# jhqxxx/aha

Hardware: AMD Instinct MI355X
Metric: decode tokens/s (greedy, batch 1) -- Qwen3-VL-8B, 1x1024^2 image + 512-token prompt; prefill tok/s alongside (higher is better)
Workload: dtype bf16; 1 GPU; qwen3vl8b; image=1024, kv_len_mid=2024, replicas=1, loop=device-resident greedy loop

## Files before the change

### aha_amd/_lib.py

```python
from __future__ import annotations

import ctypes as C
import os

_HERE = os.path.dirname(os.path.abspath(__file__))
LIB_PATH = os.path.join(_HERE, "csrc", "libaha_hip.so")

AHA_BF16, AHA_F16, AHA_F32, AHA_U32, AHA_U8 = 0, 1, 2, 3, 4
AHA_ARCH_QWEN3, AHA_ARCH_QWEN3VL, AHA_ARCH_QWEN3ASR = 0, 1, 2
ACT_NONE, ACT_GELU_TANH, ACT_GELU_ERF, ACT_SILU, ACT_SILU_MUL_PAIRS = 0, 1, 2, 3, 4


AHA_SAMPLE_HAS_TOP_P, AHA_SAMPLE_HAS_TOP_K = 1, 2
AHA_SAMPLE_NEED_LOGITS = 1
AHA_WQ_NONE, AHA_WQ_MXFP8_E4M3, AHA_WQ_MXFP4_E2M1 = 0, 1, 2
AHA_WQ_LM_HEAD = 1


class SamplingParams(C.Structure):
    _fields_ = [
        ("temperature", C.c_float), ("top_p", C.c_float), ("top_k", C.c_int32), ("repeat_penalty", C.c_float),
        ("repeat_last_n", C.c_int32), ("flags", C.c_uint32), ("seed", C.c_uint64),
    ]

# ... 80 lines not shown
                ("audio_samples", C.POINTER(C.c_float)), ("n_samples", C.c_int64),
                ("image_embeds", C.c_void_p), ("n_image_tokens", C.c_int64),
                ("pixel_values_video", C.c_void_p), ("n_patches_video", C.c_int64),
                ("video_grid_thw", C.POINTER(C.c_uint32)), ("n_videos", C.c_int32)]


_P = C.c_void_p
ALLREDUCE_FN = C.CFUNCTYPE(C.c_int, C.c_void_p, C.c_size_t, C.c_void_p)
REDUCE_SCATTER_FN = C.CFUNCTYPE(C.c_int, C.c_void_p, C.c_size_t, C.c_void_p)
ALL_GATHER_FN = C.CFUNCTYPE(C.c_int, C.c_void_p, C.c_size_t, C.c_void_p)

SIGNATURES = {
    "aha_hip_init": (C.c_int, [C.c_int, C.POINTER(_P)]),
    "aha_hip_shutdown": (None, [_P]),
    "aha_hip_last_error": (C.c_char_p, []),
    "aha_hip_version": (C.c_char_p, []),
    "aha_hip_get_dtype": (C.c_int, [C.c_int32, C.c_char_p, C.POINTER(C.c_int32)]),
    "aha_hip_check_dtype": (C.c_int, [C.c_int32]),
    "aha_hip_model_create": (C.c_int, [_P, C.POINTER(ModelDesc), C.POINTER(TensorView), C.c_size_t, C.POINTER(_P)]),
    "aha_hip_model_destroy": (None, [_P]),
    "aha_hip_forward_initial": (C.c_int, [_P, C.POINTER(C.c_uint32), C.c_size_t, C.c_size_t, C.POINTER(MmInput),
                                          C.POINTER(C.c_float), C.POINTER(C.c_uint32)]),
    "aha_hip_forward_step": (C.c_int, [_P, C.c_uint32, C.c_size_t, C.POINTER(C.c_float), C.POINTER(C.c_uint32)]),
    "aha_hip_clear_cache": (C.c_int, [_P]),
    "aha_hip_stop_token_ids": (C.c_int, [_P, C.POINTER(C.c_uint32), C.c_size_t]),
    "aha_hip_decode_greedy": (C.c_int, [_P, C.c_uint32, C.c_size_t, C.c_size_t, C.POINTER(C.c_uint32)]),
    "aha_hip_sample_candidates": (C.c_int, [_P, C.POINTER(C.c_uint32), C.c_size_t, C.c_float, C.c_float, C.c_int32,
                                            C.POINTER(C.c_float), C.POINTER(C.c_uint32), C.POINTER(C.c_float),
                                            C.POINTER(C.c_float)]),
    "aha_hip_last_logits": (C.c_int, [_P, C.POINTER(C.c_float)]),
    "aha_hip_rng_create": (C.c_int, [C.c_uint64, C.POINTER(_P)]),
    "aha_hip_rng_destroy": (None, [_P]),
    "aha_hip_rng_next_u32": (C.c_uint32, [_P]),
    "aha_hip_rng_weighted_index": (C.c_int, [_P, C.POINTER(C.c_float), C.c_size_t, C.POINTER(C.c_uint32)]),
    "aha_hip_debug_chacha_block": (C.c_int, [C.POINTER(C.c_uint32), C.c_int, C.POINTER(C.c_uint32)]),
    "aha_hip_img_smart_resize": (C.c_int, [C.c_uint32, C.c_uint32, C.c_uint32, C.c_uint32, C.c_uint32, C.POINTER(C.c_uint32),
                                           C.POINTER(C.c_uint32)]),
    "aha_hip_image_resize": (C.c_int, [_P, C.c_int32, C.c_int32, _P, C.c_int32, C.c_int32, _P]),
    "aha_hip_debug_resize_taps": (C.c_int, [C.c_int32, C.c_int32, C.POINTER(C.c_int32), C.POINTER(C.c_int32), C.POINTER(C.c_float),
                                            C.c_int64]),
    "aha_hip_debug_resample_taps": (C.c_int64, [C.c_int32, C.c_int32, C.POINTER(C.c_float), C.c_int64, C.POINTER(C.c_int32),
                                                C.POINTER(C.c_int32)]),
    "aha_hip_audio_resample": (C.c_int64, [_P, C.POINTER(C.c_float), C.c_int64, C.c_int32, C.c_int32, C.c_int32,
                                           C.POINTER(C.c_float), C.c_int64]),
    "aha_hip_cache_len": (C.c_size_t, [_P]),
    "aha_hip_debug_steps_executed": (C.c_int64, [_P]),
    "aha_hip_debug_graph_step": (C.c_int, [_P, C.c_int32, C.POINTER(C.c_double), C.POINTER(C.c_double)]),
    "aha_hip_kv_export": (C.c_int, [_P, _P, C.c_size_t, C.POINTER(C.c_size_t), C.POINTER(C.c_size_t), C.POINTER(C.c_int64)]),
    "aha_hip_kv_import": (C.c_int, [_P, _P, C.c_size_t, C.c_int32, C.c_int32, C.c_int32, C.c_int32, C.c_size_t, C.c_int64]),
    "aha_hip_set_profiling": (C.c_int, [_P, C.c_int]),
    "aha_hip_get_profile": (C.c_int, [_P, C.c_char_p, C.POINTER(C.c_double), C.POINTER(C.c_int64),
                                      C.POINTER(C.c_double), C.POINTER(C.c_double)]),
    "aha_hip_debug_scramble_pages": (C.c_int, [_P, C.c_int]),
    "aha_hip_debug_attn_decode_form": (C.c_int, [_P]),
    "aha_hip_debug_last_hidden": (C.c_int, [_P, C.POINTER(C.c_float), C.c_size_t]),
    "aha_hip_debug_image_embeds": (C.c_int, [_P, C.c_int, C.POINTER(C.c_float), C.c_size_t]),
    "aha_hip_rmsnorm": (C.c_int, [_P, _P, _P, C.c_int64, C.c_int32, C.c_float, _P]),
    "aha_hip_gemv": (C.c_int, [_P, _P, _P, C.c_int32, C.c_int32, _P, C.c_float, _P, _P]),
    "aha_hip_gemv_gate_up": (C.c_int, [_P, _P, _P, _P, C.c_int32, C.c_int32, _P, C.c_float, _P]),
    "aha_hip_gemm": (C.c_int, [_P, _P, _P, C.c_int32, C.c_int32, C.c_int32, C.c_int32, C.c_int32, C.c_int32, _P, _P,
                               C.c_int32, _P]),
    "aha_hip_qknorm_rope": (C.c_int, [_P, _P, _P, _P, _P, _P, _P, _P, C.c_int32, C.c_int32, C.c_int32, C.c_int32,
                                      C.c_float, C.c_float, _P]),
    "aha_hip_attn_decode": (C.c_int, [_P, _P, _P, _P, C.c_int32, C.c_int32, C.c_int32, C.c_int32, C.c_float, _P]),
    "aha_hip_attn_prefill": (C.c_int, [_P, _P, _P, _P, C.c_int32, C.c_int32, C.c_int32, C.c_int32, C.c_int32,
                                       C.c_int32, C.c_int32, C.c_float, _P]),
    "aha_hip_debug_attn_prefill_segs": (C.c_int, [_P, _P, _P, _P, C.c_int32, C.c_int32, _P, C.c_int32, C.c_int32, C.c_float, _P]),
    "aha_hip_debug_prefill_rope": (C.c_int, [_P, _P, _P, _P, _P, _P, _P, C.c_int32, C.c_int32, C.c_int32, C.c_int32, C.c_int32, C.c_float,
                                             C.c_int32, C.c_int32, C.c_int32, _P, _P, C.c_int32, _P, _P, _P]),
    "aha_hip_debug_prefill_attn_qfuse": (C.c_int, [_P, _P, _P, _P, C.c_int32, C.c_int32, C.c_int32, C.c_int32, C.c_int32, C.c_float, C.c_float,
                                                   C.c_int32, C.c_int32, C.c_int32, C.c_int32, C.c_int32, _P, C.c_int32, C.c_int32, _P, _P]),
    "aha_hip_debug_layernorm_rows": (C.c_int, [_P, _P, _P, _P, C.c_int64, C.c_int32, C.c_float, _P]),
    "aha_hip_debug_gemm_layernorm": (C.c_int, [_P, _P, _P] + [C.c_int32] * 6 + [_P, _P, C.c_int32, _P, _P, _P, C.c_float, _P]),
    "aha_hip_debug_vit_pos_embed": (C.c_int, [_P, C.c_int32, C.c_int32, C.c_int32, _P, _P, C.c_int64, C.c_int32, _P, _P, _P]),
    "aha_hip_debug_vit_rope": (C.c_int, [_P, _P, C.c_int32, C.c_int32, _P, _P, C.c_int32, C.c_int64, C.c_int32, C.c_int32, _P, _P, _P, _P, _P, _P]),
    "aha_hip_debug_scatter_rows": (C.c_int, [_P, _P, _P, C.c_int64, C.c_int64, C.c_int32, C.c_int32, _P]),
    "aha_hip_debug_audio_im2col1": (C.c_int, [_P, C.c_int64, _P, C.c_int32, C.c_int32, C.c_int32, _P, _P]),
    "aha_hip_debug_im2col_nhwc": (C.c_int, [_P, _P, C.c_int32, C.c_int32, C.c_int32, C.c_int32, _P]),
    "aha_hip_debug_audio_tokens_gather": (C.c_int, [_P, _P, C.c_int32, C.c_int32, C.c_int32, C.c_int32, _P]),
    "aha_hip_debug_sinus_pe_add": (C.c_int, [_P, C.c_int64, C.c_int32, C.c_int32, _P]),
    "aha_hip_debug_kv_pack_generic": (C.c_int, [_P, C.c_int64, C.c_int32, C.c_int32, _P, C.c_int32, C.c_int32, C.c_int32, C.c_int32, _P, _P]),
    "aha_hip_argmax": (C.c_int, [_P, C.c_int64, _P, _P]),
    "aha_hip_logmel": (C.c_int, [_P, C.c_int64, _P, _P]),
    "aha_hip_logmel_batch": (C.c_int, [_P, _P, C.c_size_t, _P, _P]),
    "aha_hip_debug_poison_lds": (C.c_int, [C.c_uint32, _P]),
    "aha_hip_debug_gemm_plan": (C.c_int, [C.c_int32, C.c_int32]),
    "aha_hip_debug_attn_variant": (C.c_int, [C.c_int32]),
    "aha_hip_debug_attn_form": (C.c_int, [C.c_int32]),
    "aha_hip_debug_gemm_grouped": (C.c_int, [_P, _P, _P] + [C.c_int32] * 10 + [_P]),
    "aha_hip_debug_streamk_plan": (C.c_int, [C.c_int32, C.c_int32, C.c_int32, C.c_int32, C.c_int32, C.c_size_t, _P, C.c_int32, _P, _P]),
    "aha_hip_set_gemm_reserved_cus": (C.c_int, [C.c_int32]),
    "aha_hip_debug_plan_gemm": (C.c_int, [C.c_int32, C.c_int32, C.c_int32, C.c_int32, C.c_int32, C.c_int32, C.c_size_t, _P]),
    "aha_hip_get_rope_index": (C.c_int, [_P, _P, C.c_size_t, _P, C.c_int32, _P, _P]),
    "aha_hip_get_rope_index_mm": (C.c_int, [_P, _P, C.c_size_t, _P, C.c_int32, _P, C.c_int32, _P, _P]),
    "aha_hip_embed": (C.c_int, [_P, _P, C.c_size_t, _P]),
    "aha_hip_embed_batch": (C.c_int, [_P, _P, _P, C.c_size_t, C.c_size_t, _P]),
    "aha_hip_generate_batch": (C.c_int, [_P, _P, _P, C.c_size_t, C.c_size_t, C.c_size_t, _P, _P, _P]),
    "aha_hip_generate_batch_sampled": (C.c_int, [_P, _P, _P, C.c_size_t, C.POINTER(SamplingParams), C.c_size_t, C.c_size_t, _P, _P, _P]),
    "aha_hip_generate_batch_mm": (C.c_int, [_P, _P, _P, C.c_size_t, _P, C.POINTER(SamplingParams), C.c_size_t, C.c_size_t, _P, _P, _P]),
    "aha_hip_generate_batch_spec": (C.c_int, [_P, _P, _P, C.c_size_t, C.c_size_t, C.c_size_t, C.POINTER(SpecConfig), _P, _P, _P, _P, _P, _P, _P,
                                              C.POINTER(SpecStats)]),
    "aha_hip_spec_propose": (C.c_int, [C.POINTER(SpecConfig), _P, C.c_size_t, C.c_size_t, _P, C.c_size_t, _P, C.POINTER(C.c_size_t)]),
    "aha_hip_engine_create": (C.c_int, [_P, C.POINTER(EngineConfig), _P]),
    "aha_hip_engine_destroy": (None, [_P]),
    "aha_hip_engine_submit": (C.c_int, [_P, _P, C.c_size_t, _P, C.POINTER(SamplingParams), C.c_size_t, C.POINTER(C.c_uint64)]),
    "aha_hip_engine_cancel": (C.c_int, [_P, C.c_uint64]),
    "aha_hip_engine_step": (C.c_int, [_P, C.POINTER(EngineEvent), C.c_size_t, C.POINTER(C.c_size_t), _P]),
    "aha_hip_engine_stats": (C.c_int, [_P, C.POINTER(EngineStats)]),
    "aha_hip_engine_debug_ctr_base": (C.c_int, [_P, C.c_uint32]),
    "aha_hip_engine_submit_spec": (C.c_int, [_P, _P, C.c_size_t, _P, C.c_size_t, C.POINTER(SpecConfig), _P, C.c_size_t, C.POINTER(C.c_uint64)]),
    "aha_hip_engine_max_events": (C.c_size_t, [_P]),
    "aha_hip_engine_spec_stats": (C.c_int, [_P, C.POINTER(SpecStats)]),
    "aha_hip_engine_request_spec": (C.c_int, [_P, C.c_uint64, C.POINTER(C.c_size_t), C.POINTER(C.c_size_t)]),
    "aha_hip_generate_batch_logprobs": (C.c_int, [_P, _P, _P, C.c_size_t, _P, C.POINTER(SamplingParams), _P, C.c_size_t, C.c_size_t, _P, _P, _P,
                                                  C.POINTER(TokenLogprobs)]),
    "aha_hip_engine_submit_logprobs": (C.c_int, [_P, _P, C.c_size_t, _P, C.POINTER(SamplingParams), C.c_size_t, C.c_int32,
                                                 C.POINTER(C.c_uint64)]),
    "aha_hip_engine_step_logprobs": (C.c_int, [_P, C.POINTER(EngineEvent), C.c_size_t, C.POINTER(C.c_size_t), _P, C.POINTER(TokenLogprobs)]),
    "aha_hip_generate_batch_adjusted": (C.c_int, [_P, _P, _P, C.c_size_t, _P, C.POINTER(SamplingParams), C.POINTER(LogitAdjust), _P, C.c_size_t,
                                                  C.c_size_t, _P, _P, _P, C.POINTER(TokenLogprobs)]),
    "aha_hip_engine_submit_adjusted": (C.c_int, [_P, _P, C.c_size_t, _P, C.POINTER(SamplingParams), C.POINTER(LogitAdjust), C.c_size_t, C.c_int32,
                                                 C.POINTER(C.c_uint64)]),
    "aha_hip_sample_rows_adjusted": (C.c_int, [_P, C.c_int64, C.c_int32, C.c_int32, _P, _P, _P, _P, _P, _P, _P, _P, _P, _P, _P, _P]),
    "aha_hip_sampler_set_adjust": (C.c_int, [_P, C.POINTER(LogitAdjust)]),
    "aha_hip_sampler_adjust_list": (C.c_int, [_P, C.c_size_t, _P, C.c_size_t, _P, _P, C.c_size_t, C.POINTER(C.c_size_t)]),
    "aha_hip_generate_batch_masked": (C.c_int, [_P, _P, _P, C.c_size_t, _P, C.POINTER(SamplingParams), C.POINTER(LogitAdjust), _P, C.c_size_t,
                                                C.c_size_t, _P, _P, _P, _P, _P, C.POINTER(TokenLogprobs)]),
    "aha_hip_engine_submit_masked": (C.c_int, [_P, _P, C.c_size_t, _P, C.POINTER(SamplingParams), C.POINTER(LogitAdjust), _P, C.c_size_t,
                                               C.c_size_t, C.c_int32, C.POINTER(C.c_uint64)]),
    "aha_hip_engine_set_mask": (C.c_int, [_P, C.c_uint64, _P, C.c_size_t]),
    "aha_hip_sample_rows_masked": (C.c_int, [_P, C.c_int64, C.c_int32, C.c_int32, _P, _P, _P, _P, _P, _P, _P, _P, _P, _P, _P, _P, _P, _P]),
    "aha_hip_sampler_set_mask": (C.c_int, [_P, _P, C.c_size_t]),
    "aha_hip_logprob_rows": (C.c_int, [_P, C.c_int64, C.c_int32, C.c_int32, _P, _P, _P, _P]),
    "aha_hip_sample_rows": (C.c_int, [_P, C.c_int64, C.c_int32, C.c_int32, _P, _P, _P, _P, _P, _P, _P, _P, _P]),
    "aha_hip_sampler_create": (C.c_int, [C.POINTER(SamplingParams), _P]),
    "aha_hip_sampler_destroy": (None, [_P]),
    "aha_hip_sampler_plan": (C.c_int, [_P, C.c_size_t, C.c_size_t, C.POINTER(C.c_int32), C.POINTER(C.c_float), C.POINTER(C.c_float),
                                       C.POINTER(C.c_size_t)]),
    "aha_hip_sampler_pick": (C.c_int, [_P, _P, _P, C.c_int32, C.c_float, C.c_float, _P, C.c_size_t, _P, C.c_size_t, C.POINTER(C.c_uint32)]),
    "aha_hip_sampler_rng_words": (C.c_uint64, [_P]),
    "aha_hip_gemv_rows": (C.c_int, [_P, _P, _P, C.c_int32, C.c_int32, C.c_int32, C.c_int32, _P, _P, _P, _P]),
    "aha_hip_quantize_mxfp8": (C.c_int, [_P, C.c_int32, C.c_int32, _P, _P, _P, _P]),
    "aha_hip_gemv_rows_mxfp8": (C.c_int, [_P, _P, _P, _P, C.c_int32, C.c_int32, C.c_int32, C.c_int32, _P, _P, _P, _P]),
    "aha_hip_quantize_mxfp4": (C.c_int, [_P, C.c_int32, C.c_int32, _P, _P, _P, _P]),
    "aha_hip_gemv_rows_mxfp4": (C.c_int, [_P, _P, _P, _P, C.c_int32, C.c_int32, C.c_int32, C.c_int32, _P, _P, _P, _P]),
    "aha_hip_model_quantize_weights": (C.c_int, [_P, C.c_int32, C.c_uint32]),
    "aha_hip_model_weight_format": (C.c_int, [_P, C.POINTER(C.c_int32), C.POINTER(C.c_uint32)]),
    "aha_hip_debug_fp8_rows": (C.c_int, [_P, C.c_int]),
    "aha_hip_debug_fp8_single": (C.c_int, [_P, C.c_int]),
    "aha_hip_debug_pk13_single": (C.c_int, [_P, C.c_int]),
    "aha_hip_pk13_status": (C.c_int, [_P, C.c_char_p, C.c_size_t]),
    "aha_hip_pack_pk13": (C.c_int, [_P, C.c_int32, C.c_int32, _P, C.POINTER(C.c_int32), C.POINTER(C.c_int64), _P]),
    "aha_hip_gemv_pk13": (C.c_int, [_P, C.c_int32, _P, _P, C.c_int32, C.c_int32, C.c_int32, _P, C.c_float, _P, _P, _P, _P]),
    "aha_hip_debug_plan_gemv_pk13": (C.c_int, [C.c_int32, C.c_int32, C.c_int32, C.c_int32, C.POINTER(C.c_int32), C.POINTER(C.c_int32),
                                              C.POINTER(C.c_int32), C.POINTER(C.c_int32), C.POINTER(C.c_int32)]),
    "aha_hip_gemv_epi": (C.c_int, [_P, _P, _P, C.c_int32, C.c_int32, C.c_int32, _P, C.c_float, _P, _P, _P, _P]),
    "aha_hip_gemv_mxfp8": (C.c_int, [_P, _P, _P, _P, C.c_int32, C.c_int32, C.c_int32, _P, C.c_float, _P, _P, _P, _P]),
    "aha_hip_debug_plan_gemv_mxfp8": (C.c_int, [C.c_int32, C.c_int32, C.c_int32, C.c_int32, C.POINTER(C.c_int32), C.POINTER(C.c_int32),
                                                C.POINTER(C.c_int32), C.POINTER(C.c_int32), C.POINTER(C.c_int32)]),
    "aha_hip_debug_fp4_single": (C.c_int, [_P, C.c_int]),
    "aha_hip_gemv_mxfp4": (C.c_int, [_P, _P, _P, _P, C.c_int32, C.c_int32, C.c_int32, _P, C.c_float, _P, _P, _P, _P]),
    "aha_hip_debug_plan_gemv_mxfp4": (C.c_int, [C.c_int32, C.c_int32, C.c_int32, C.c_int32, C.POINTER(C.c_int32), C.POINTER(C.c_int32),
                                                C.POINTER(C.c_int32), C.POINTER(C.c_int32), C.POINTER(C.c_int32)]),
    "aha_hip_debug_plan_gemv": (C.c_int, [C.c_int32, C.c_int32, C.c_int32, C.c_int32, C.POINTER(C.c_int32), C.POINTER(C.c_int32),
                                          C.POINTER(C.c_int32), C.POINTER(C.c_int32)]),
    "aha_hip_debug_gemv_partial_f32": (C.c_int, [_P, _P, _P, C.c_int32, C.c_int32, _P, C.c_float, _P]),
    "aha_hip_attn_decode_batch": (C.c_int, [_P, _P, _P, _P, _P, _P, _P, C.c_int32, C.c_int32, C.c_int32, C.c_float, C.c_float, _P, _P]),
    "aha_hip_debug_attn_decode_fused": (C.c_int, [_P, _P, _P, _P, _P, C.c_int32, C.c_int32, C.c_int32, C.c_float, C.c_float, _P, _P]),
    "aha_hip_config_parse": (C.c_int, [C.c_char_p, _P]),
    "aha_hip_config_torch_dtype": (C.c_int, [C.c_char_p, C.c_char_p, C.c_size_t]),
    "aha_hip_weights_open": (C.c_int, [C.c_char_p, _P]),
    "aha_hip_weights_count": (C.c_size_t, [_P]),
    "aha_hip_weights_get": (C.c_int, [_P, C.c_size_t, _P]),
    "aha_hip_weights_close": (None, [_P]),
    "aha_hip_model_load": (C.c_int, [_P, C.c_char_p, C.c_size_t, _P]),
    "aha_hip_set_allreduce": (C.c_int, [_P, _P, _P]),
    "aha_hip_set_seq_parallel": (C.c_int, [_P, _P, _P, _P]),
    "aha_hip_tp_unique_id": (C.c_int, [_P]),
    "aha_hip_tp_init_rccl": (C.c_int, [_P, _P]),
    "aha_hip_set_context_parallel": (C.c_int, [_P, C.c_int32, C.c_int32, _P, _P]),
    "aha_hip_cp_init_rccl": (C.c_int, [_P, _P]),
    "aha_hip_debug_cp_plan": (C.c_int, [C.c_int32, C.c_int32, C.c_int32, C.POINTER(C.c_int32)]),
    "aha_hip_debug_allreduce": (C.c_int, [_P, _P, C.c_size_t]),
    "aha_hip_vision_encode": (C.c_int, [_P, C.POINTER(MmInput), _P, C.POINTER(C.c_int64)]),
    "aha_hip_debug_audio_embeds": (C.c_int, [_P, C.POINTER(C.c_float), C.c_size_t]),
    "aha_hip_image_to_patches": (C.c_int, [_P, _P, C.c_int32, C.c_int32, C.c_int32, C.c_int32, C.POINTER(C.c_float),
                                           C.POINTER(C.c_float), _P]),
    "aha_hip_video_smart_resize": (C.c_int, [C.c_uint32] * 8 + [_P, _P]),
    "aha_hip_video_sample_frames": (C.c_int, [C.c_uint32, C.c_float, C.c_uint32, C.c_uint32, C.c_uint32, _P, _P]),
    "aha_hip_video_timestamps": (C.c_int64, [_P, C.c_size_t, C.c_float, C.c_uint32, _P, C.c_size_t]),
    "aha_hip_video_to_patches": (C.c_int, [_P, _P, C.c_int32, C.c_int32, C.c_int32, C.c_int32, C.c_int32, C.POINTER(C.c_float),
                                           C.POINTER(C.c_float), _P]),
}

TOKEN_MASK_FN = C.CFUNCTYPE(C.c_int, C.c_void_p, C.c_size_t, C.POINTER(C.c_uint32), C.c_size_t, C.POINTER(C.c_uint32), C.c_size_t)

_lib = None


class AhaHipError(RuntimeError):
    def __init__(self, code: int, msg: str):
        super().__init__(f"aha_hip error {code}: {msg}")
        self.code = code


def lib() -> C.CDLL:
    global _lib
    if _lib is None:
        if not os.path.exists(LIB_PATH):
            raise ImportError(f"{LIB_PATH} is missing: run `python -m aha_amd.build` (or __graft_entry__.build()) first; "
                              "there is no CPU fallback for the HIP path")
        try:
            import torch
        except ImportError:
            pass
        l = C.CDLL(LIB_PATH)
        for name, (res, args) in SIGNATURES.items():
            fn = getattr(l, name)
            fn.restype = res
            fn.argtypes = args
        _lib = l
    return _lib


def check(rc: int) -> int:
    if rc < 0:
        raise AhaHipError(rc, lib().aha_hip_last_error().decode(errors="replace"))
    return rc
```

### aha_amd/csrc/capi.hip

```cpp
#include <math.h>
#include <string.h>

#include <algorithm>
#include <map>
#include <memory>
#include <mutex>
#include <numeric>
#include <vector>

#include "common.h"
#include "model.h"
#include "sampler.h"
#include "audio.h"
#include "vision.h"

namespace aha {
const char* last_error_cstr();
}
using namespace aha;

#define API_GUARD_BEGIN try {
#define API_GUARD_END                                   \
  }                                                     \
  catch (const std::exception& e) {                     \
// ... 1023 lines not shown
  m->fp8_rows = on != 0;
  return AHA_OK;
}

int aha_hip_debug_fp8_single(aha_model* m, int on) {
  if (!m) {
    set_error("debug_fp8_single: null model");
    return AHA_ERR_INVALID;
  }
  if (on < 0 || on > 2) {
    set_error("debug_fp8_single: on must be 0 (bf16), 1 (by plan) or 2 (every matrix with a copy)");
    return AHA_ERR_INVALID;
  }
  m->fp8_single = on;
  return AHA_OK;
}

int aha_hip_debug_pk13_single(aha_model* m, int on) {
  if (!m) {
    set_error("debug_pk13_single: null model");
    return AHA_ERR_INVALID;
  }
  if (on < 0 || on > 2) {
    set_error("debug_pk13_single: on must be 0 (bf16), 1 (by plan) or 2 (every matrix with a copy)");
    return AHA_ERR_INVALID;
  }
  m->pk13_single = on;
  return AHA_OK;
}

int aha_hip_pk13_status(const aha_model* m, char* buf, size_t cap) {
  if (!m || (!buf && cap)) {
    set_error("pk13_status: null model or buffer");
    return AHA_ERR_INVALID;
  }
  std::string s;
  int n = 0;
  for (const Pk13Entry& e : m->pk13) {
    s += e.name + "\t" + e.status + "\n";
    n += e.slot->p != nullptr;
  }
  if (cap) {
    const size_t k = std::min(s.size(), cap - 1);
    memcpy(buf, s.data(), k);
    buf[k] = 0;
  }
  return n;
}

int aha_hip_debug_fp4_single(aha_model* m, int on) {
  if (!m) {
    set_error("debug_fp4_single: null model");
    return AHA_ERR_INVALID;
  }
  if (on < 0 || on > 2) {
    set_error("debug_fp4_single: on must be 0 (bf16), 1 (by plan) or 2 (every matrix with a copy)");
    return AHA_ERR_INVALID;
  }
  m->fp4_single = on;
  return AHA_OK;
}

static int debug_plan_gemv_mx(int mx, int32_t N, int32_t K, int32_t epi, int32_t has_norm, int32_t* R, int32_t* U, int32_t* grid, int32_t* form,
                              int32_t* by_plan) {
  if (!R || !U || !grid || N < 1 || K < 32 || K % 32 || epi < 0 || epi > 3 || (epi == 2 && N % 32)) {
    set_error(std::string("debug_plan_gemv_mxfp") + (mx == 8 ? "8" : "4") +
              ": bad argument (N >= 1, K a positive multiple of 32, epi 0..3, epi 2 needs N % 32 == 0)");
    return AHA_ERR_INVALID;
  }
  int o[5];
  (mx == 8 ? debug_plan_gemv_mxfp8 : debug_plan_gemv_mxfp4)(epi == 2 ? N / 2 : N, K, (GemvEpi)epi, has_norm != 0, o);
  *R = o[0]; *U = o[1]; *grid = o[2];
  if (form) *form = o[3] ? 1 + o[4] : 0;
  if (by_plan) *by_plan = (mx == 8 ? gemv_mxfp8_by_plan : gemv_mxfp4_by_plan)(N, K, (GemvEpi)epi) ? 1 : 0;
  return AHA_OK;
}

int aha_hip_debug_plan_gemv_mxfp8(int32_t N, int32_t K, int32_t epi, int32_t has_norm, int32_t* R, int32_t* U, int32_t* grid, int32_t* form,
                                  int32_t* by_plan) {
  return debug_plan_gemv_mx(8, N, K, epi, has_norm, R, U, grid, form, by_plan);
}

int aha_hip_debug_plan_gemv_pk13(int32_t N, int32_t K, int32_t epi, int32_t has_norm, int32_t* R, int32_t* U, int32_t* grid, int32_t* form,
                                 int32_t* by_plan) {
  if (!R || !U || !grid || epi < 0 || epi > 3 || (epi == 2 && N % 32) || !gemv_pk13_shape_ok(N, K)) {
    set_error("debug_plan_gemv_pk13: bad argument (N >= 1, K a multiple of 4096 and at most 32768, epi 0..3, epi 2 needs N % 32 == 0)");
    return AHA_ERR_INVALID;
  }
  int o[5];
  debug_plan_gemv_pk13(epi == 2 ? N / 2 : N, K, (GemvEpi)epi, has_norm != 0, o);
  *R = o[0]; *U = o[1]; *grid = o[2];
  if (form) *form = 1 + o[4];
  if (by_plan) *by_plan = gemv_pk13_by_plan(N, K, (GemvEpi)epi) ? 1 : 0;
  return AHA_OK;
}

int aha_hip_debug_plan_gemv_mxfp4(int32_t N, int32_t K, int32_t epi, int32_t has_norm, int32_t* R, int32_t* U, int32_t* grid, int32_t* form,
                                  int32_t* by_plan) {
  return debug_plan_gemv_mx(4, N, K, epi, has_norm, R, U, grid, form, by_plan);
}

int aha_hip_debug_plan_gemv(int32_t N, int32_t K, int32_t epi, int32_t has_norm, int32_t* R, int32_t* U, int32_t* grid, int32_t* form) {
  if (!R || !U || !grid || N < 1 || K < 8 || K % 8 || K > 32768 || epi < 0 || epi > 4 || (epi == 2 && N % 2)) {
    set_error("debug_plan_gemv: bad argument (N >= 1, K a positive multiple of 8 and at most 32768, epi 0..4, epi 2 needs an even N)");
    return AHA_ERR_INVALID;
  }
  int o[5];
  debug_plan_gemv(epi == 2 ? N / 2 : N, K, (GemvEpi)epi, has_norm != 0, o);
  *R = o[0]; *U = o[1]; *grid = o[2];
  if (form) *form = o[3] ? 1 + o[4] : 0;
  return AHA_OK;
}

int aha_hip_debug_gemv_partial_f32(const void* W, const void* x, float* y_f32, int32_t N, int32_t K, const void* norm_w, float eps,
                                   void* stream) {
  API_GUARD_BEGIN
  if (!W || !x || !y_f32 || N < 1 || K < 8 || K % 8 || K > 32768) {
    set_error("debug_gemv_partial_f32: bad argument (W, x, y_f32 not null, N >= 1, K a positive multiple of 8 and at most 32768)");
    return AHA_ERR_INVALID;
  }
  GemvArgs g{};
  g.W = W; g.x = x; g.y_f32 = y_f32; g.N = N; g.K = K; g.norm_w = norm_w; g.eps = eps;
  launch_gemv(g, GEMV_PARTIAL_F32, (hipStream_t)stream);
  AHA_HIP_CHECK(hipGetLastError());
  return AHA_OK;
  API_GUARD_END
}

namespace {
struct GemvPartials {
  void* p[2] = {nullptr, nullptr};
  ~GemvPartials() {
    for (void* q : p)
      if (q) hipFree(q);
  }
};
const char* gemv_epi_args_bad(const void* w, const void* x, const void* y, int N, int K, int kmul, int epi, const void* residual,
                              const float* logits, const uint32_t* argmax_out) {
  if (!w || !x) return "null matrix or x";
  if (N < 1) return "N must be at least 1";
  if (K < kmul || K % kmul) return kmul == 32 ? "K must be a positive multiple of 32 (the MX block)" : "K must be a positive multiple of 8";
  if (K > 32768) return "K must be at most 32768";
  if (epi < 0 || epi > 3) return "epi must be 0..3";
  if (epi != 3 && !y) return "null y";
  if (epi == 1 && !residual) return "epi 1 needs a residual";
  if (epi == 2 && N % 32) return "epi 2 needs N % 32 == 0";
  if (epi == 3 && (!logits || !argmax_out)) return "epi 3 needs logits and argmax_out";
  return nullptr;
}
}

static int gemv_epi_run(const void* W, int mx, const void* q, const uint32_t* scales, const void* x, void* y, int32_t N, int32_t K,
                        int32_t epi, const void* norm_w, float eps, const void* residual, float* logits, uint32_t* argmax_out, void* stream,
                        int pk13_bh = 0) {
  hipStream_t st = (hipStream_t)stream;
  GemvArgs g{};
  g.W = W; g.x = x; g.y = y; g.N = epi == 2 ? N / 2 : N; g.K = K; g.norm_w = norm_w; g.eps = eps; g.residual = epi == 1 ? residual : nullptr;
  g.y_f32 = logits;
  const GemvEpi e = epi == 0 ? GEMV_STORE : epi == 1 ? GEMV_RESIDUAL : epi == 2 ? GEMV_SILU_MUL : GEMV_LOGITS;
  GemvPartials part;
  int tiles = 0;
  if (epi == 3) {
    tiles = !q ? gemv_num_tiles(N, K) : mx == 8 ? gemv_mxfp8_num_tiles(N, K) : mx == 13 ? gemv_pk13_num_tiles(N, K) : gemv_mxfp4_num_tiles(N, K);
    AHA_HIP_CHECK(hipMalloc(&part.p[0], (size_t)tiles * 4));
    AHA_HIP_CHECK(hipMalloc(&part.p[1], (size_t)tiles * 4));
    g.blk_max = (float*)part.p[0];
    g.blk_idx = (uint32_t*)part.p[1];
  }
  if (!q) launch_gemv(g, e, st);
  else if (mx == 8) launch_gemv_mxfp8(g, q, scales, e, st);
  else if (mx == 13) launch_gemv_pk13(g, q, pk13_bh, e, st);
  else launch_gemv_mxfp4(g, q, scales, e, st);
  if (epi == 3) launch_argmax_partials(g.blk_max, g.blk_idx, tiles, argmax_out, st);
  hipError_t err = hipGetLastError();
  if (epi == 3) {
    const hipError_t e2 = hipStreamSynchronize(st);
    if (err == hipSuccess) err = e2;
  }
  AHA_HIP_CHECK(err);
  return AHA_OK;
}

int aha_hip_gemv_epi(const void* W, const void* x, void* y, int32_t N, int32_t K, int32_t epi, const void* norm_w, float eps,
                     const void* residual, float* logits, uint32_t* argmax_out, void* stream) {
  API_GUARD_BEGIN
  if (const char* bad = gemv_epi_args_bad(W, x, y, N, K, 8, epi, residual, logits, argmax_out)) {
    set_error(std::string("gemv_epi: ") + bad);
    return AHA_ERR_INVALID;
  }
  return gemv_epi_run(W, 0, nullptr, nullptr, x, y, N, K, epi, norm_w, eps, residual, logits, argmax_out, stream);
  API_GUARD_END
}

int aha_hip_gemv_mxfp8(const void* q, const uint32_t* scales, const void* x, void* y, int32_t N, int32_t K, int32_t epi, const void* norm_w,
                       float eps, const void* residual, float* logits, uint32_t* argmax_out, void* stream) {
  API_GUARD_BEGIN
  if (!scales) {
    set_error("gemv_mxfp8: null scales");
    return AHA_ERR_INVALID;
  }
  if (const char* bad = gemv_epi_args_bad(q, x, y, N, K, 32, epi, residual, logits, argmax_out)) {
    set_error(std::string("gemv_mxfp8: ") + bad);
    return AHA_ERR_INVALID;
  }
  return gemv_epi_run(nullptr, 8, q, scales, x, y, N, K, epi, norm_w, eps, residual, logits, argmax_out, stream);
  API_GUARD_END
}

int aha_hip_gemv_pk13(const void* packed, int32_t bh, const void* x, void* y, int32_t N, int32_t K, int32_t epi, const void* norm_w,
                      float eps, const void* residual, float* logits, uint32_t* argmax_out, void* stream) {
  API_GUARD_BEGIN
  if (const char* bad = gemv_epi_args_bad(packed, x, y, N, K, 8, epi, residual, logits, argmax_out)) {
    set_error(std::string("gemv_pk13: ") + bad);
    return AHA_ERR_INVALID;
  }
  if (K % 4096) {
    set_error("gemv_pk13: K must be a multiple of 4096 (the unit)");
    return AHA_ERR_INVALID;
  }
  if (bh < 0 || bh > 112) {
    set_error("gemv_pk13: bh must be 0..112");
    return AHA_ERR_INVALID;
  }
  return gemv_epi_run(nullptr, 13, packed, nullptr, x, y, N, K, epi, norm_w, eps, residual, logits, argmax_out, stream, bh);
  API_GUARD_END
}

int aha_hip_pack_pk13(const void* W, int32_t N, int32_t K, void* out, int32_t* bh_out, int64_t* bad_out, void* stream) {
  API_GUARD_BEGIN
  if (!W || !bh_out || !bad_out || N < 1 || K < 4096 || K % 4096) {
    set_error("pack_pk13: bad argument (W, bh_out, bad_out not null, N >= 1, K a positive multiple of 4096)");
    return AHA_ERR_INVALID;
  }
  hipStream_t st = (hipStream_t)stream;
  GemvPartials d;
  AHA_HIP_CHECK(hipMalloc(&d.p[0], sizeof(Pk13Stats)));
  AHA_HIP_CHECK(hipMemsetAsync(d.p[0], 0, sizeof(Pk13Stats), st));
  launch_pk13_stats(W, (int64_t)N * K, (Pk13Stats*)d.p[0], st);
  AHA_HIP_CHECK(hipGetLastError());
  Pk13Stats h{};
  AHA_HIP_CHECK(hipMemcpyAsync(&h, d.p[0], sizeof(h), hipMemcpyDeviceToHost, st));
  AHA_HIP_CHECK(hipStreamSynchronize(st));
  *bh_out = pk13_base(h.max_e2);
  *bad_out = (int64_t)h.bad;
  if (out && !h.bad) {
    launch_pk13_pack(W, N, K, *bh_out, out, st);
    AHA_HIP_CHECK(hipGetLastError());
    AHA_HIP_CHECK(hipStreamSynchronize(st));
  }
  return AHA_OK;
  API_GUARD_END
}

int aha_hip_gemv_mxfp4(const void* q, const uint32_t* scales, const void* x, void* y, int32_t N, int32_t K, int32_t epi, const void* norm_w,
                       float eps, const void* residual, float* logits, uint32_t* argmax_out, void* stream) {
  API_GUARD_BEGIN
  if (!scales) {
    set_error("gemv_mxfp4: null scales");
    return AHA_ERR_INVALID;
  }
  if (const char* bad = gemv_epi_args_bad(q, x, y, N, K, 32, epi, residual, logits, argmax_out)) {
    set_error(std::string("gemv_mxfp4: ") + bad);
    return AHA_ERR_INVALID;
  }
  return gemv_epi_run(nullptr, 4, q, scales, x, y, N, K, epi, norm_w, eps, residual, logits, argmax_out, stream);
  API_GUARD_END
}

namespace {
struct DevFree {
  void* p[2] = {nullptr, nullptr};
  ~DevFree() {
    for (void* q : p)
      if (q) hipFree(q);
  }
};
}

static int sample_rows_impl(const float* logits, int64_t ld, int32_t R, int32_t V, const int32_t* k, const float* temperature,
                            const float* repeat_penalty, const uint32_t* context, const size_t* context_offsets, const uint32_t* adj_ids,
                            const float* adj_vals, const size_t* adj_offsets, float* vals_out, uint32_t* idx_out, float* ms_out, void* stream,
                            const uint32_t* masks, const int32_t* mask_rows) {
  if (!logits || R < 1 || V < 1 || ld < V || !k || !temperature || !repeat_penalty || !context_offsets || !vals_out || !idx_out || !ms_out) {
    set_error("sample_rows: bad arguments (R >= 1, ld >= V >= 1, per-row k / temperature / repeat_penalty / context_offsets, outputs)");
    return AHA_ERR_INVALID;
  }
  for (int r = 0; r < R; ++r)
    if (!sample_shape_ok(V, k[r]) || !(repeat_penalty[r] > 0.f) || context_offsets[r + 1] < context_offsets[r] ||
        (context_offsets[r + 1] > context_offsets[r] && !context)) {
      set_error("sample_rows: row " + std::to_string(r) + " needs 1 <= k <= 64, repeat_penalty > 0 and ordered context offsets");
      return AHA_ERR_INVALID;
    }
  hipStream_t st = (hipStream_t)stream;
  std::vector<int32_t> tab((size_t)R * SAMPLE_ROW_WORDS, 0);
  std::vector<uint32_t> ctx;
  for (int r = 0; r < R; ++r) {
    int32_t* t = tab.data() + (size_t)r * SAMPLE_ROW_WORDS;
    const size_t c0 = ctx.size();
    if (repeat_penalty[r] != 1.0f) {
      for (size_t i = context_offsets[r]; i < context_offsets[r + 1]; ++i)
        if (context[i] < (uint32_t)V) ctx.push_back(context[i]);
      std::sort(ctx.begin() + c0, ctx.end());
      ctx.erase(std::unique(ctx.begin() + c0, ctx.end()), ctx.end());
    }
    const float inv_t = temperature[r] > 0.f ? (float)(1.0 / (double)temperature[r]) : 1.0f;
    t[SAMPLE_ROW_LROW] = r;
    t[SAMPLE_ROW_K] = k[r];
    memcpy(&t[SAMPLE_ROW_INVT], &inv_t, 4);
    memcpy(&t[SAMPLE_ROW_PEN], &repeat_penalty[r], 4);
    t[SAMPLE_ROW_CTX0] = (int32_t)c0;
    t[SAMPLE_ROW_NCTX] = (int32_t)(ctx.size() - c0);
    t[SAMPLE_ROW_MASK] = mask_rows && mask_rows[r] >= 0 ? mask_rows[r] : -1;
    if (t[SAMPLE_ROW_MASK] >= 0 && (!masks || (int64_t)t[SAMPLE_ROW_MASK] * ((V + 31) / 32) > (int64_t)INT32_MAX)) {
      set_error("sample_rows_masked: row " + std::to_string(r) + " names a mask but masks is null, or the mask index is out of range");
      return AHA_ERR_INVALID;
    }
  }
  std::vector<uint32_t> aid;
  std::vector<float> aval;
  for (int r = 0; adj_offsets && r < R; ++r) {
    const size_t a0 = adj_offsets[r], a1 = adj_offsets[r + 1];
    if (a1 < a0 || (a1 > a0 && (!adj_ids || !adj_vals)) || a1 - a0 > (size_t)V) {
      set_error("sample_rows_adjusted: row " + std::to_string(r) + " needs ordered adj_offsets, adj_ids / adj_vals and at most V entries");
      return AHA_ERR_INVALID;
    }
    std::vector<size_t> o(a1 - a0);
    std::iota(o.begin(), o.end(), a0);
    std::sort(o.begin(), o.end(), [&](size_t x, size_t y) { return adj_ids[x] < adj_ids[y]; });
    int32_t* t = tab.data() + (size_t)r * SAMPLE_ROW_WORDS;
    t[SAMPLE_ROW_ADJ0] = (int32_t)aid.size();
    t[SAMPLE_ROW_NADJ] = (int32_t)o.size();
    for (size_t i = 0; i < o.size(); ++i) {
      const uint32_t id = adj_ids[o[i]];
      const float a = adj_vals[o[i]];
      if (id >= (uint32_t)V || (i && id == aid.back()) || isnan(a) || a == INFINITY) {
        set_error("sample_rows_adjusted: row " + std::to_string(r) + " needs distinct ids < V and addends that are finite or -inf");
        return AHA_ERR_INVALID;
      }
      aid.push_back(id);
      aval.push_back(a);
    }
  }
  if (aid.size() > (size_t)INT32_MAX) {
    set_error("sample_rows_adjusted: too many addends");
    return AHA_ERR_INVALID;
  }
  const int nw = sample_stage1_waves(V);
  const size_t cand = (size_t)R * (nw + 16) * 64;
  DevFree adj_free;
  uint32_t* d_aid = nullptr;
  float* d_aval = nullptr;
  if (!aid.empty()) {
    AHA_HIP_CHECK(hipMalloc((void**)&d_aid, aid.size() * 4));
    adj_free.p[0] = d_aid;
    AHA_HIP_CHECK(hipMalloc((void**)&d_aval, aid.size() * 4));
    adj_free.p[1] = d_aval;
    AHA_HIP_CHECK(hipMemcpyAsync(d_aid, aid.data(), aid.size() * 4, hipMemcpyHostToDevice, st));
    AHA_HIP_CHECK(hipMemcpyAsync(d_aval, aval.data(), aid.size() * 4, hipMemcpyHostToDevice, st));
  }
  int32_t* d_tab = nullptr;
  uint32_t *d_ctx = nullptr, *d_cidx = nullptr;
  float *d_cval = nullptr, *d_part = nullptr, *d_out = nullptr;
  AHA_HIP_CHECK(hipMalloc((void**)&d_tab, tab.size() * 4));
  AHA_HIP_CHECK(hipMalloc((void**)&d_ctx, std::max<size_t>(ctx.size(), 1) * 4));
  AHA_HIP_CHECK(hipMalloc((void**)&d_cval, cand * 4));
  AHA_HIP_CHECK(hipMalloc((void**)&d_cidx, cand * 4));
  AHA_HIP_CHECK(hipMalloc((void**)&d_part, 2 * (size_t)R * nw * 4));
  AHA_HIP_CHECK(hipMalloc((void**)&d_out, (size_t)R * SAMPLE_OUT_WORDS * 4));
  AHA_HIP_CHECK(hipMemcpyAsync(d_tab, tab.data(), tab.size() * 4, hipMemcpyHostToDevice, st));
  if (!ctx.empty()) AHA_HIP_CHECK(hipMemcpyAsync(d_ctx, ctx.data(), ctx.size() * 4, hipMemcpyHostToDevice, st));
  for (int stage = 0; stage < 3; ++stage)
    launch_topk_rows(logits, ld, V, R, d_tab, d_ctx, d_cval, d_cidx, d_part, d_part + (size_t)R * nw, d_out, stage, st, d_aid, d_aval, masks);
  hipError_t err = hipGetLastError();
  if (err == hipSuccess) err = hipMemcpy2DAsync(vals_out, 64 * 4, d_out, SAMPLE_OUT_WORDS * 4, 64 * 4, R, hipMemcpyDeviceToDevice, st);
  if (err == hipSuccess) err = hipMemcpy2DAsync(ms_out, 2 * 4, d_out + 64, SAMPLE_OUT_WORDS * 4, 2 * 4, R, hipMemcpyDeviceToDevice, st);
  if (err == hipSuccess) err = hipMemcpy2DAsync(idx_out, 64 * 4, d_out + 66, SAMPLE_OUT_WORDS * 4, 64 * 4, R, hipMemcpyDeviceToDevice, st);
  hipStreamSynchronize(st);
  hipFree(d_tab);
  hipFree(d_ctx);
  hipFree(d_cval);
  hipFree(d_cidx);
  hipFree(d_part);
  hipFree(d_out);
  AHA_HIP_CHECK(err);
  return AHA_OK;
}

int aha_hip_sample_rows(const float* logits, int64_t ld, int32_t R, int32_t V, const int32_t* k, const float* temperature,
                        const float* repeat_penalty, const uint32_t* context, const size_t* context_offsets, float* vals_out,
                        uint32_t* idx_out, float* ms_out, void* stream) {
  API_GUARD_BEGIN
  return sample_rows_impl(logits, ld, R, V, k, temperature, repeat_penalty, context, context_offsets, nullptr, nullptr, nullptr, vals_out, idx_out,
                          ms_out, stream, nullptr, nullptr);
  API_GUARD_END
}

int aha_hip_sample_rows_adjusted(const float* logits, int64_t ld, int32_t R, int32_t V, const int32_t* k, const float* temperature,
                                 const float* repeat_penalty, const uint32_t* context, const size_t* context_offsets,
                                 const uint32_t* adj_ids, const float* adj_vals, const size_t* adj_offsets, float* vals_out,
                                 uint32_t* idx_out, float* ms_out, void* stream) {
  API_GUARD_BEGIN
  if (!adj_offsets) {
    set_error("sample_rows_adjusted: null adj_offsets");
// ... 868 lines not shown
```

### aha_amd/csrc/gemv_pk13_body.h

```cpp
#pragma once
#include "gemv_body.h"

namespace aha {

typedef __attribute__((ext_vector_type(2))) uint32_t pk13_u32x2_t;
typedef __attribute__((ext_vector_type(2))) uint16_t pk13_u16x2_t;

constexpr int PK13_UNIT_K = 4096;
constexpr int PK13_UNIT_BYTES = 6656;
constexpr int PK13_OFF_H = 4096, PK13_OFF_S = 6144;

__device__ __forceinline__ pk13_u32x2_t pk13_ld_nt8(const void* p) { return __builtin_nontemporal_load(reinterpret_cast<const pk13_u32x2_t*>(p)); }

struct Pk13Unit {
  u32x4_t a[4];
  u32x4_t h[2];
  pk13_u32x2_t s;
};

__device__ __forceinline__ uint32_t pk13_high4(uint32_t x, uint32_t sd, pk13_u16x2_t bh2, int g) {
  const uint32_t nz = ((x + 0x0f0f0f0fu) >> 4) & 0x01010101u;
  const pk13_u16x2_t r = __builtin_bit_cast(pk13_u16x2_t, nz) * bh2 + __builtin_bit_cast(pk13_u16x2_t, x);
  return __builtin_bit_cast(uint32_t, r) | ((sd << (7 - g)) & 0x80808080u);
}

template <int E>
__device__ __forceinline__ float pk13_f32(uint32_t hb, uint32_t lo) {
  return __uint_as_float(__builtin_amdgcn_perm(hb, lo, 0x04000c0cu + 0x01010000u * E));
}

struct GemvPk13Args {
  const void* p;
  const void* x;
  const void* norm_w;
  const void* residual;
  void* y;
  float* y_f32;
  float* blk_max;
  uint32_t* blk_idx;
  void* h_out;
  int N, K;
  int bh;
  float eps;
};

template <int R, int EPI, int PRO>
__device__ __forceinline__ void gemv_pk13_body(const GemvPk13Args& a, float* xs, const int bid, const int nblk) {
  const int tid = threadIdx.x, lane = tid & 63;
  const int wave = __builtin_amdgcn_readfirstlane(tid >> 6);
  const int K = a.K, N = a.N;
  const int nchunks = K >> 9;
  float* red = xs + (nchunks << 9);

  constexpr int ROWS_PER_TILE = GEMV_WAVES * R;
  constexpr int NW = (EPI == GEMV_SILU_MUL) ? 2 : 1;
  const int n_out = N;
  const int ntiles = (n_out + ROWS_PER_TILE - 1) / ROWS_PER_TILE;
  const int gpt = K >> 12;
  const int my_tiles = (ntiles - bid + nblk - 1) / nblk;
  const int ngroups = my_tiles * gpt;
  const uint8_t* P = (const uint8_t*)a.p;
  const size_t prow = (size_t)gpt * PK13_UNIT_BYTES;
  const pk13_u16x2_t bh2 = {(uint16_t)a.bh, (uint16_t)a.bh};

  auto issue = [&](int gi, Pk13Unit (&buf)[NW][R], bf16_t (&resv)[R]) {
    const int tile = bid + (gi / gpt) * nblk;
    const int unit = gi % gpt;
    const int row0 = tile * ROWS_PER_TILE + wave * R;
    if (EPI == GEMV_RESIDUAL) {
#pragma unroll
      for (int r = 0; r < R; ++r) resv[r] = ((const bf16_t*)a.residual)[min(row0 + r, n_out - 1)];
    }
#pragma unroll
    for (int r = 0; r < R; ++r) {
      const int row = min(row0 + r, n_out - 1);
      const size_t fr = NW == 2 ? (size_t)(row >> 4) * 32 + (row & 15) : (size_t)row;
#pragma unroll
      for (int m = 0; m < NW; ++m) {
        const uint8_t* up = P + (fr + 16 * m) * prow + (size_t)unit * PK13_UNIT_BYTES;
        Pk13Unit& b = buf[m][r];
        b.s = pk13_ld_nt8(up + PK13_OFF_S + lane * 8);
        b.h[0] = ld_nt16(up + PK13_OFF_H + lane * 16);
        b.a[0] = ld_nt16(up + lane * 16);
        b.a[1] = ld_nt16(up + 1024 + lane * 16);
        b.h[1] = ld_nt16(up + PK13_OFF_H + 1024 + lane * 16);
        b.a[2] = ld_nt16(up + 2048 + lane * 16);
        b.a[3] = ld_nt16(up + 3072 + lane * 16);
      }
    }
  };

  constexpr int XPRE = 8;
  constexpr bool SL = PRO != 0, SL_NORM = PRO == 2;
  constexpr int XSL = SL_NORM ? 4 : XPRE;
  const bool pre = SL || (nchunks << 6) <= XPRE * GEMV_THREADS;
  u32x4_t xpre[XPRE], npre[XPRE];
  Pk13Unit bufA[NW][R], bufB[NW][R];
  bf16_t resA[R], resB[R];
  if (SL) {
    const int vlast = (K >> 3) - 1;
#pragma unroll
    for (int j = 0; j < XSL; ++j) {
      const int v = min(tid + j * GEMV_THREADS, vlast);
      xpre[j] = ld16((const bf16_t*)a.x + v * 8);
      if (SL_NORM) npre[j] = ld16((const bf16_t*)a.norm_w + v * 8);
    }
    __builtin_amdgcn_sched_barrier(0);
    issue(0, bufA, resA);
    __builtin_amdgcn_sched_barrier(0);
  } else {
    if (pre) {
#pragma unroll
      for (int j = 0; j < XPRE; ++j) {
        const int v = tid + j * GEMV_THREADS;
        xpre[j] = u32x4_t{0u, 0u, 0u, 0u};
        npre[j] = u32x4_t{0u, 0u, 0u, 0u};
        if (v * 8 < K) {
          xpre[j] = ld16((const bf16_t*)a.x + v * 8);
          if (a.norm_w != nullptr) npre[j] = ld16((const bf16_t*)a.norm_w + v * 8);
        }
      }
    }
    issue(0, bufA, resA);
  }

  {
    const bf16_t* x = (const bf16_t*)a.x;
    const bf16_t* nw = (const bf16_t*)a.norm_w;
    float ss = 0.f;
    auto stage = [&](int v, u32x4_t xv) {
      float f[8];
#pragma unroll
      for (int j = 0; j < 4; ++j) { f[2 * j] = lo_bf(xv[j]); f[2 * j + 1] = hi_bf(xv[j]); }
#pragma unroll
      for (int j = 0; j < 8; ++j) ss += f[j] * f[j];
      const int base = xs_index(v * 8);
      *reinterpret_cast<float4*>(xs + base) = make_float4(f[0], f[1], f[2], f[3]);
      *reinterpret_cast<float4*>(xs + base + 256) = make_float4(f[4], f[5], f[6], f[7]);
    };
    if (pre) {
#pragma unroll
      for (int it = 0; it < (SL ? XSL : XPRE); ++it) {
        const int v = tid + it * GEMV_THREADS;
        if (v < (nchunks << 6)) stage(v, xpre[it]);
      }
    } else {
      for (int v = tid; v < (nchunks << 6); v += GEMV_THREADS) stage(v, ld16(x + v * 8));
    }
    if (SL ? SL_NORM : nw != nullptr) {
      ss = wave_sum(ss);
      if (lane == 0) red[wave] = ss;
      __syncthreads();
      const float tot = red[0] + red[1] + red[2] + red[3];
      const float rinv = 1.0f / sqrtf(tot / (float)K + a.eps);
      auto norm = [&](int v, u32x4_t wv) {
        const int base = xs_index(v * 8);
        float4 lo = *reinterpret_cast<float4*>(xs + base), hi = *reinterpret_cast<float4*>(xs + base + 256);
        lo.x = rbf(lo.x * rinv * lo_bf(wv[0])); lo.y = rbf(lo.y * rinv * hi_bf(wv[0]));
        lo.z = rbf(lo.z * rinv * lo_bf(wv[1])); lo.w = rbf(lo.w * rinv * hi_bf(wv[1]));
        hi.x = rbf(hi.x * rinv * lo_bf(wv[2])); hi.y = rbf(hi.y * rinv * hi_bf(wv[2]));
        hi.z = rbf(hi.z * rinv * lo_bf(wv[3])); hi.w = rbf(hi.w * rinv * hi_bf(wv[3]));
        *reinterpret_cast<float4*>(xs + base) = lo;
        *reinterpret_cast<float4*>(xs + base + 256) = hi;
        if (a.h_out != nullptr && bid == 0) {
          u32x4_t o;
          o[0] = pack_bf(lo.x, lo.y); o[1] = pack_bf(lo.z, lo.w); o[2] = pack_bf(hi.x, hi.y); o[3] = pack_bf(hi.z, hi.w);
          *reinterpret_cast<u32x4_t*>((bf16_t*)a.h_out + v * 8) = o;
        }
      };
      if (pre) {
#pragma unroll
        for (int it = 0; it < (SL ? XSL : XPRE); ++it) {
          const int v = tid + it * GEMV_THREADS;
          if (v < (K >> 3)) norm(v, npre[it]);
        }
      } else {
        for (int v = tid; v < (K >> 3); v += GEMV_THREADS) norm(v, ld16(nw + v * 8));
      }
    }
    __syncthreads();
  }
  __builtin_amdgcn_sched_barrier(0);

  float tile_best = -INFINITY;
  uint32_t tile_best_i = 0xffffffffu;
  float acc[NW][R];
#pragma unroll
  for (int m = 0; m < NW; ++m)
#pragma unroll
    for (int r = 0; r < R; ++r) acc[m][r] = 0.f;

  auto consume = [&](int gi, Pk13Unit (&buf)[NW][R], bf16_t (&resv)[R]) {
    const int c0 = (gi % gpt) * 8;
#pragma unroll
    for (int c = 0; c < 8; ++c) {
      const float4 xlo = *reinterpret_cast<const float4*>(xs + ((c0 + c) << 9) + (lane << 2));
      const float4 xhi = *reinterpret_cast<const float4*>(xs + ((c0 + c) << 9) + 256 + (lane << 2));
#pragma unroll
      for (int m = 0; m < NW; ++m)
#pragma unroll
        for (int r = 0; r < R; ++r) {
          const Pk13Unit& b = buf[m][r];
          const uint32_t hd = b.h[c >> 2][c & 3], sd = b.s[c >> 2];
          const uint32_t lo0 = b.a[c >> 1][(c & 1) * 2], lo1 = b.a[c >> 1][(c & 1) * 2 + 1];
          const uint32_t h0 = pk13_high4(hd & 0x0f0f0f0fu, sd, bh2, (c & 3) * 2);
          const uint32_t h1 = pk13_high4((hd >> 4) & 0x0f0f0f0fu, sd, bh2, (c & 3) * 2 + 1);
          float s = acc[m][r];
          s = fmaf(xlo.x, pk13_f32<0>(h0, lo0), s); s = fmaf(xlo.y, pk13_f32<1>(h0, lo0), s);
          s = fmaf(xlo.z, pk13_f32<2>(h0, lo0), s); s = fmaf(xlo.w, pk13_f32<3>(h0, lo0), s);
          s = fmaf(xhi.x, pk13_f32<0>(h1, lo1), s); s = fmaf(xhi.y, pk13_f32<1>(h1, lo1), s);
          s = fmaf(xhi.z, pk13_f32<2>(h1, lo1), s); s = fmaf(xhi.w, pk13_f32<3>(h1, lo1), s);
          acc[m][r] = s;
        }
    }
    if (gi % gpt != gpt - 1) return;
    const int tile = bid + (gi / gpt) * nblk;
    const int row0 = tile * ROWS_PER_TILE + wave * R;
#pragma unroll
    for (int m = 0; m < NW; ++m)
#pragma unroll
      for (int r = 0; r < R; ++r) acc[m][r] = wave_sum(acc[m][r]);
    if (lane == 0) {
#pragma unroll
      for (int r = 0; r < R; ++r) {
        const int row = row0 + r;
        if (row < n_out) {
          const float lin = rbf(acc[0][r]);
          if (EPI == GEMV_STORE) {
            ((bf16_t*)a.y)[row] = f2bf(lin);
          } else if (EPI == GEMV_RESIDUAL) {
            ((bf16_t*)a.y)[row] = f2bf(bf2f(resv[r]) + lin);
          } else if (EPI == GEMV_SILU_MUL) {
            const float g = rbf(silu_f(lin));
            const float up = rbf(acc[NW - 1][r]);
            ((bf16_t*)a.y)[row] = f2bf(g * up);
          } else {
            a.y_f32[row] = lin;
            if (lin > tile_best || (lin == tile_best && (uint32_t)row < tile_best_i)) { tile_best = lin; tile_best_i = row; }
          }
        }
      }
    }
#pragma unroll
    for (int m = 0; m < NW; ++m)
#pragma unroll
      for (int r = 0; r < R; ++r) acc[m][r] = 0.f;
  };

  int g = 0;
  for (; g + 2 < ngroups; g += 2) {
    __builtin_amdgcn_sched_barrier(0);
    issue(g + 1, bufB, resB);
    __builtin_amdgcn_sched_barrier(0);
    consume(g, bufA, resA);
    __builtin_amdgcn_sched_barrier(0);
    issue(g + 2, bufA, resA);
    __builtin_amdgcn_sched_barrier(0);
    consume(g + 1, bufB, resB);
  }
  if (g + 1 < ngroups) {
    __builtin_amdgcn_sched_barrier(0);
    issue(g + 1, bufB, resB);
    __builtin_amdgcn_sched_barrier(0);
    consume(g, bufA, resA);
    consume(g + 1, bufB, resB);
  } else if (g < ngroups) {
    consume(g, bufA, resA);
  }
  if (EPI == GEMV_LOGITS) {
    __syncthreads();
    if (lane == 0) { red[wave] = tile_best; reinterpret_cast<uint32_t*>(red)[4 + wave] = tile_best_i; }
    __syncthreads();
    if (tid == 0) {
      float bv = red[0];
      uint32_t bi = reinterpret_cast<uint32_t*>(red)[4];
      for (int w = 1; w < 4; ++w) {
        const float v = red[w];
        const uint32_t i = reinterpret_cast<uint32_t*>(red)[4 + w];
        if (v > bv || (v == bv && i < bi)) { bv = v; bi = i; }
      }
      a.blk_max[bid] = bv;
      a.blk_idx[bid] = bi;
    }
  }
}

}
```

### aha_amd/csrc/kernels.h

```cpp
#pragma once
#include <hip/hip_runtime.h>
#include <stdint.h>

#include <algorithm>
#include <utility>
#include <vector>

namespace aha {

struct KvLayer {
  const uint64_t* page_ptrs;
  uint64_t layer_off;
  int kvh, d;
};

enum GemvEpi { GEMV_STORE = 0, GEMV_RESIDUAL = 1, GEMV_SILU_MUL = 2, GEMV_LOGITS = 3, GEMV_PARTIAL_F32 = 4 };

struct GemvArgs {
  const void* W;
  const void* W2;
  const void* x;
  const void* norm_w;
  const void* residual;
  void* y;
// ... 91 lines not shown
  const float* rope;
  KvLayer kv;
  uint64_t lin_page0 = 0;
  int64_t lin_step = 0;
  int kv_start_v;
  int kv_len_v;
  float* part_o;
  float* part_ml;
  void* o;
  unsigned* head_ctr;
  unsigned ctr_target;
  unsigned long long* trace;
  int nh, kvh, nsplit;
  float eps, scale;
};
void launch_attn_decode_fused(const AttnDecodeFusedArgs& a, hipStream_t st);

struct AttnPrefillArgs {
  const void* q;
  KvLayer kv;
  void* o;
  int S, nh, kvh, d;
  int kv_offset;
  int kv_total;
  int causal;
  float scale;
  int64_t q_ld;
  int nqb;
  int S2 = 0, kv_offset2 = 0, kv_total2 = 0;
  int epi_rows = 0;
  int v_ones_row = 0;
  int rows_hint = 0;
  const void* q_norm_w = nullptr;
  const void* q_rope_tab = nullptr;
  float q_eps = 0.f;
  const int32_t* seg_tab = nullptr;
  const int32_t* seg_items = nullptr;
  int n_items = 0;
  const int32_t* seg_kv0 = nullptr;
};
inline std::vector<int32_t> seg_items_of(const std::vector<int32_t>& seg_tab, bool causal, const std::vector<int32_t>* kv0 = nullptr) {
  constexpr int QB = 64;
  std::vector<std::pair<int32_t, int32_t>> items;
  for (size_t j = 0; 3 * j < seg_tab.size(); ++j)
    for (int32_t b = 0; b * QB < seg_tab[3 * j + 1]; ++b) items.emplace_back((int32_t)j, b);
  auto cost = [&](const std::pair<int32_t, int32_t>& it) {
    const int32_t len = seg_tab[3 * (size_t)it.first + 1];
    return causal ? (kv0 ? (*kv0)[(size_t)it.first] : 0) + std::min(len, (it.second + 1) * QB) : len;
  };
  std::stable_sort(items.begin(), items.end(), [&](const auto& x, const auto& y) { return cost(x) > cost(y); });
  std::vector<int32_t> out;
  out.reserve(2 * items.size());
  for (const auto& it : items) out.push_back(it.first), out.push_back(it.second);
  return out;
}
void launch_attn_prefill(const AttnPrefillArgs& a, hipStream_t st);
bool attn_prefill_takes_qfuse(const AttnPrefillArgs& a);
int attn_prefill_form_of(const AttnPrefillArgs& a);
bool launch_attn_prefill64(const AttnPrefillArgs& a, hipStream_t st, int pipe);
void set_attn_form_override(int form);
void set_attn_variant_override(int smx);

enum GemmAct { ACT_NONE = 0, ACT_GELU_TANH = 1, ACT_GELU_ERF = 2, ACT_SILU = 3, ACT_SILU_MUL_PAIRS = 4, ACT_PARTIAL_F32 = 5 };
struct GemmArgs {
  const void* A;
  const void* W;
  void* C;
  const void* bias;
  const void* residual;
  int M, N, K;
  int64_t lda, ldw, ldc;
  int act;
  const void* norm_w = nullptr;
  void* norm_out = nullptr;
  float norm_eps = 0.f;
  const void* norm_b = nullptr;
  void* workspace = nullptr;
  size_t workspace_bytes = 0;
  void* sk_counters = nullptr;
  int tile_group = 8;
  int partial_rows = 1;
  int groups = 1, a_gstride = 0, c_gstride = 0, c_row0 = 0, m_total = 0;
};
void launch_gemm(const GemmArgs& a, hipStream_t st);
void launch_gemm_grouped(const GemmArgs& a, hipStream_t st);
void set_gemm_workspace(void* ws, size_t bytes, void* sk_counters = nullptr);
constexpr int SK_MAX_COUNTERS = 4096;
bool streamk_has_kernel(int act, bool has_bias, bool has_res, bool n192);
double streamk_estimate(const GemmArgs& a, int tile_n, int* n_chunks, int* n_split);
bool launch_gemm_streamk(const GemmArgs& a, int tile_n, hipStream_t st);
void set_streamk_forced_cut(int code);
int gemm_streamk_workers();
int gemm_streamk_cus();
int get_gemm_reserved_cus();
void set_gemm_reserved_cus(int n);
bool acquire_gemm_cu_reservation(int cus);
void release_gemm_cu_reservation();
int debug_streamk_plan(int M, int N, int K, int tile_n, int workers, int group, size_t ws_bytes, int* out, int cap, int* off_out, int* info);
void debug_plan_gemm(int M, int N, int K, int act, bool has_bias, bool has_res, size_t ws_bytes, int* out, bool has_norm = false);
void set_gemm_plan_override(int tile, int splitk);
void get_gemm_workspace(void** ws, size_t* bytes, void** sk_counters);
struct GemmWorkspaceScope {
  GemmWorkspaceScope(void* ws, size_t bytes, void* sk_counters = nullptr) {
    get_gemm_workspace(&prev_ws, &prev_bytes, &prev_ctrs);
    set_gemm_workspace(ws, bytes, sk_counters);
  }
  ~GemmWorkspaceScope() { set_gemm_workspace(prev_ws, prev_bytes, prev_ctrs); }
  GemmWorkspaceScope(const GemmWorkspaceScope&) = delete;
  GemmWorkspaceScope& operator=(const GemmWorkspaceScope&) = delete;
  void* prev_ws = nullptr;
  size_t prev_bytes = 0;
  void* prev_ctrs = nullptr;
};
void launch_residual_add_f32(void* x, const float* sum, int64_t n, hipStream_t st);
void launch_poison_lds(uint32_t seed, hipStream_t st);
void launch_residual_add_f32_cols(void* x, int64_t ldx, const float* sum, int64_t lds, int64_t rows, int cols, hipStream_t st);
void launch_row_to_f32(const void* x_bf16_or_null, float* out, int n, hipStream_t st);
void launch_f32_to_row(const float* x, void* out_bf16, int n, hipStream_t st);

struct GemvRowsArgs {
  const void* W;
  const void* x;
  const void* residual;
  void* y;
  float* y_f32;
  float* blk_max;
  uint32_t* blk_idx;
  float* ws;
  int R, N, K;
  int64_t ldx, ldy, ldf;
  int64_t ldws = 0;
};
void launch_gemv_rows(const GemvRowsArgs& a, GemvEpi epi, hipStream_t st);
void launch_gemv_rows_merge(const GemvRowsArgs& a, GemvEpi epi, int nks, hipStream_t st);
struct WQuant {
  void* q = nullptr;
  uint32_t* scales = nullptr;
};
size_t mxfp8_scale_words(int N, int K);
void launch_gemv_rows_mxfp8(const GemvRowsArgs& a, const void* q, const uint32_t* scales, GemvEpi epi, hipStream_t st);
void launch_mxfp8_quantize(const void* w, int N, int K, void* q_out, uint32_t* scales_out, void* w_roundtrip_out, hipStream_t st);
void launch_mxfp8_check(const void* w, int64_t n_elems, int* flag, hipStream_t st);
void launch_gemv_mxfp8(const GemvArgs& g, const void* q, const uint32_t* scales, GemvEpi epi, hipStream_t st);
int gemv_mxfp8_num_tiles(int N, int K);
bool gemv_mxfp8_by_plan(int N, int K, GemvEpi epi);
void debug_plan_gemv_mxfp8(int N, int K, GemvEpi epi, bool has_norm, int* out5);
void launch_gemv_rows_mxfp4(const GemvRowsArgs& a, const void* q, const uint32_t* scales, GemvEpi epi, hipStream_t st);
void launch_mxfp4_quantize(const void* w, int N, int K, void* q_out, uint32_t* scales_out, void* w_roundtrip_out, hipStream_t st);
void launch_mxfp4_check(const void* w, int64_t n_elems, int* flag, hipStream_t st);
void launch_gemv_mxfp4(const GemvArgs& g, const void* q, const uint32_t* scales, GemvEpi epi, hipStream_t st);
int gemv_mxfp4_num_tiles(int N, int K);
bool gemv_mxfp4_by_plan(int N, int K, GemvEpi epi);
void debug_plan_gemv_mxfp4(int N, int K, GemvEpi epi, bool has_norm, int* out5);
struct Pk13Stats {
  int max_e2;
  int pad;
  unsigned long long bad;
};
__host__ __device__ inline int pk13_base(int max_e2) { return max_e2 > 15 ? max_e2 - 15 : 0; }
size_t pk13_bytes(int N, int K);
void launch_pk13_stats(const void* w, int64_t n_elems, Pk13Stats* stats, hipStream_t st);
void launch_pk13_pack(const void* w, int N, int K, int bh, void* out, hipStream_t st);
bool gemv_pk13_shape_ok(int N, int K);
void launch_gemv_pk13(const GemvArgs& g, const void* packed, int bh, GemvEpi epi, hipStream_t st);
int gemv_pk13_num_tiles(int N, int K);
bool gemv_pk13_by_plan(int N, int K, GemvEpi epi);
void debug_plan_gemv_pk13(int N, int K, GemvEpi epi, bool has_norm, int* out5);
void gemv_rows_plan(int N, int K, int* chunks_per_wave, int* k_splits);
int gemv_rows_num_tiles(int N);
size_t gemv_rows_ws_floats(int R, int N, int K);
void launch_argmax_rows(const float* blk_max, const uint32_t* blk_idx, int ntiles, int rows, uint32_t* out, hipStream_t st);

constexpr int GEN_ROW_WORDS = 8;
constexpr int GEN_ROW_PAGE0 = 0;
constexpr int GEN_ROW_KVLEN = 1;
constexpr int GEN_ROW_NSPLIT = 2;
constexpr int GEN_ROW_CTR = 3;
constexpr int GEN_ROW_POS = 4;
constexpr int GEN_ROW_SRC = 5;
constexpr int GEN_ROW_CTRROW = 6;
constexpr int GEN_ROW_TOK = 7;
void launch_gen_embed(const void* table, const uint32_t* tok_in, const int32_t* row_tab, int rows, void* x, int H, const float* inv_freq,
                      const int32_t* axis_map, float* rope, hipStream_t st);

struct AttnDecodeBatchArgs {
  const void* qkv;
  const void* q_norm_w;
  const void* k_norm_w;
  const float* rope;
  const uint64_t* page_ptrs;
  uint64_t layer_off;
  const int32_t* row_tab;
  float* part_o;
  float* part_ml;
  void* o;
  unsigned* head_ctr;
  int ctr_step;
  int nh, kvh, max_nsplit;
  float eps, scale;
};
void launch_attn_decode_batch(const AttnDecodeBatchArgs& a, int rows, int max_nsplit_rows, hipStream_t st, bool append = true);
void launch_kv_append_rows(const AttnDecodeBatchArgs& a, int rows, hipStream_t st);
constexpr int SPEC_MAX_DRAFT = 15;
constexpr int SPEC_SEQ_WORDS = 2, SPEC_SEQ_ROW0 = 0, SPEC_SEQ_NDRAFT = 1;
constexpr int SPEC_OUT_WORDS = 2 + SPEC_MAX_DRAFT + 1, SPEC_OUT_COUNT = 0, SPEC_OUT_LAST_ROW = 1, SPEC_OUT_TOKENS = 2;
void launch_spec_accept_rows(const uint32_t* argmax, const int32_t* row_tab, const int32_t* seq_tab, int n_seqs, uint32_t* out, hipStream_t st);
constexpr int ENG_SEQ_WORDS = 3, ENG_SEQ_ROW = 0, ENG_SEQ_DRAFT0 = 1, ENG_SEQ_NDRAFT = 2;
void launch_spec_accept_split(const uint32_t* argmax, const int32_t* row_tab, const int32_t* seq_tab, int n_seqs, uint32_t* out, hipStream_t st);
int attn_decode_nsplit(int kv_len_after, int g, int max_nsplit);

struct StepState;
constexpr size_t DECODE_SYNC_BYTES = 32768;
constexpr int DECODE_HEAD_CTR_WORD = 6144;

}

namespace aha {
constexpr int VIT_DQK = 96;
constexpr int VIT_DV = 80;
void launch_layernorm_rows(const void* x, const void* w, const void* b, void* y, int64_t rows, int dim, float eps,
                           hipStream_t st);
void launch_pos_embed_add(void* x, const void* table, const int32_t* idx, const float* wt, int64_t N, int D,
                          hipStream_t st);
struct VitRopeArgs {
  const void* qkv;
  const int32_t* rowcol;
  const float* inv_freq;
  const int32_t* page_of;
  const int32_t* slot_of;
  void* q_out;
  KvLayer kv;
  int N, nh, hd;
  const float* cs_tab = nullptr;
  const int32_t* page_first = nullptr;
  const int32_t* page_cnt = nullptr;
  int n_pages = 0;
};
void launch_vit_rope_pack(const VitRopeArgs& a, hipStream_t st);
void launch_vit_rope_table(const int32_t* rowcol, const float* inv_freq, int N, int hd, float* tab, hipStream_t st);
void launch_scatter_rows(void* dst, const void* src, const int32_t* rows, int64_t n, int D, int add, hipStream_t st);
int img_smart_resize(uint32_t h, uint32_t w, uint32_t factor, uint32_t min_pixels, uint32_t max_pixels, uint32_t* h_out, uint32_t* w_out);
int video_smart_resize(uint32_t num_frames, uint32_t h, uint32_t w, uint32_t temporal_factor, uint32_t factor, uint32_t min_pixels,
                       uint32_t max_pixels, uint32_t video_ratio, uint32_t* h_out, uint32_t* w_out);
int video_sample_frames(uint32_t total_frames, float rate, uint32_t fps, uint32_t min_frames, uint32_t max_frames, uint32_t* nframes,
                        uint32_t* interval);
int64_t video_timestamps(const uint32_t* frame_indices, size_t n, float fps, uint32_t t_merge, float* out, size_t cap);
int image_resize(const uint8_t* src, int H, int W, uint8_t* dst, int new_h, int new_w, hipStream_t st);
int debug_resize_taps(int n_in, int n_out, int32_t* left, int32_t* count, float* weights, int64_t weights_cap);
void launch_video_to_patches(const uint8_t* frames, void* out, int T, int H, int W, int patch, int merge, const float* mean,
                             const float* stdv, hipStream_t st);
void launch_image_to_patches(const uint8_t* img, void* out, int H, int W, int patch, int merge, const float* mean,
                             const float* stdv, hipStream_t st);
}

namespace aha {
constexpr int LOGMEL_CLIP_WORDS = 5;
void launch_logmel(const float* x, const int64_t* d_clips, int n_clips, int64_t n_groups, int64_t ld, const float* window, const float* twid,
                   const float* melfb, float* out, float* frame_max, hipStream_t st);
void launch_audio_im2col1(const float* feat, const int32_t* d_chunks, void* out, int64_t ld, int C, int Hin, int Win, hipStream_t st);
void launch_im2col_nhwc(const void* in, void* out, int B, int Hin, int Win, int Cin, hipStream_t st);
void launch_audio_tokens_gather(const void* in, void* out, int B, int Fq, int T, int Cc, hipStream_t st);
void launch_sinus_pe_add(void* x, int64_t rows, int d, int T, hipStream_t st);
void launch_kv_pack_generic(const void* src, int64_t ld, int k_off, int v_off, KvLayer kv, int N, int nh, int hd, hipStream_t st,
                            const int32_t* slot_of = nullptr);
}
```

### aha_amd/csrc/kernels_gemv_pk13.hip

```cpp
#include <algorithm>

#include "gemv_pk13_body.h"
#include "kernels.h"

namespace aha {

namespace {

struct GemvPk13TailArgs {
  float* y_f32;
  float* blk_max;
  uint32_t* blk_idx;
  void* h_out;
  float eps;
  int nblk;
};

template <int R, int EPI, int PRO>
__global__ __launch_bounds__(GEMV_THREADS) void gemv_kernel_pk13(const void* p, const void* x, const void* norm_w, void* y, const void* residual,
                                                                 int N, int K, int bh, GemvPk13TailArgs t) {
  extern __shared__ __attribute__((aligned(16))) float xs[];
  GemvPk13Args a;
  a.p = p; a.x = x; a.norm_w = norm_w; a.residual = residual; a.y = y;
  a.y_f32 = t.y_f32; a.blk_max = t.blk_max; a.blk_idx = t.blk_idx; a.h_out = t.h_out; a.N = N; a.K = K; a.bh = bh; a.eps = t.eps;
  gemv_pk13_body<R, EPI, PRO>(a, xs, (int)blockIdx.x, t.nblk);
}

struct GemvPk13Plan { int R, grid; };

GemvPk13Plan plan_gemv_pk13(int N, GemvEpi epi) {
  const int R = epi == GEMV_LOGITS ? 2 : 1;
  const int gmax = 768;
  const int ntiles = (N + 4 * R - 1) / (4 * R);
  int grid = std::min(ntiles, gmax);
  if (ntiles > gmax) {
    for (int g = gmax; g >= gmax / 2; g -= 8)
      if (ntiles % g == 0) {
        grid = g;
        break;
      }
  }
  return {R, std::max(grid, 1)};
}

int pro_of(int K, bool has_norm) { return K <= (has_norm ? 4 : 8) * 8 * GEMV_THREADS ? (has_norm ? 2 : 1) : 0; }

template <int R, int EPI>
void launch_pk13_epi(const GemvPk13Args& a, const GemvPk13Plan& p, hipStream_t st) {
  const size_t lds = (size_t)a.K * 4 + 64;
  dim3 grid(p.grid), block(GEMV_THREADS);
  const GemvPk13TailArgs t{a.y_f32, a.blk_max, a.blk_idx, a.h_out, a.eps, p.grid};
  const int pro = pro_of(a.K, a.norm_w != nullptr);
#define GV_(PP) hipLaunchKernelGGL((gemv_kernel_pk13<R, EPI, PP>), grid, block, lds, st, a.p, a.x, a.norm_w, a.y, a.residual, a.N, a.K, a.bh, t)
  if (pro == 2) GV_(2); else if (pro == 1) GV_(1); else GV_(0);
#undef GV_
}

__device__ __forceinline__ int pk13_e2(uint32_t bits16) { return (bits16 >> 8) & 0x7f; }

__global__ __launch_bounds__(256) void pk13_max_kernel(const u32x4_t* w, int64_t nvec, Pk13Stats* out) {
  int mx = 0;
  unsigned long long bad = 0;
  for (int64_t i = (int64_t)blockIdx.x * 256 + threadIdx.x; i < nvec; i += (int64_t)gridDim.x * 256) {
    const u32x4_t v = ld_nt16(w + i);
#pragma unroll
    for (int j = 0; j < 8; ++j) {
      const uint32_t b = (v[j >> 1] >> ((j & 1) * 16)) & 0xffffu;
      if ((b & 0x7f80u) == 0x7f80u) ++bad;
      else mx = max(mx, pk13_e2(b));
    }
  }
  for (int o = 32; o > 0; o >>= 1) {
    mx = max(mx, __shfl_xor(mx, o));
    bad += __shfl_xor(bad, o);
  }
  if ((threadIdx.x & 63) == 0) {
    atomicMax(&out->max_e2, mx);
    if (bad) atomicAdd(&out->bad, bad);
  }
}

__global__ __launch_bounds__(256) void pk13_window_kernel(const u32x4_t* w, int64_t nvec, Pk13Stats* out) {
  const int bh = pk13_base(out->max_e2);
  unsigned long long bad = 0;
  for (int64_t i = (int64_t)blockIdx.x * 256 + threadIdx.x; i < nvec; i += (int64_t)gridDim.x * 256) {
    const u32x4_t v = ld_nt16(w + i);
#pragma unroll
    for (int j = 0; j < 8; ++j) {
      const uint32_t b = (v[j >> 1] >> ((j & 1) * 16)) & 0xffffu;
      const int e2 = pk13_e2(b);
      if ((b & 0x7f80u) != 0x7f80u && e2 != 0 && e2 <= bh) ++bad;
    }
  }
  for (int o = 32; o > 0; o >>= 1) bad += __shfl_xor(bad, o);
  if ((threadIdx.x & 63) == 0 && bad) atomicAdd(&out->bad, bad);
}

__global__ __launch_bounds__(256) void pk13_pack_kernel(const bf16_t* w, int64_t nunits, int bh, uint8_t* out) {
  const int lane = threadIdx.x & 63;
  const int64_t unit = (int64_t)blockIdx.x * 4 + (threadIdx.x >> 6);
  if (unit >= nunits) return;
  const bf16_t* src = w + unit * PK13_UNIT_K + lane * 8;
  uint8_t* dst = out + unit * PK13_UNIT_BYTES;
  u32x4_t a[4], h[2];
  uint32_t s[2] = {0u, 0u};
#pragma unroll
  for (int c = 0; c < 8; ++c) {
    const u32x4_t v = ld16(src + c * 512);
    uint32_t lo[2] = {0u, 0u}, hd = 0u;
#pragma unroll
    for (int e = 0; e < 8; ++e) {
      const uint32_t b = (v[e >> 1] >> ((e & 1) * 16)) & 0xffffu;
      const int e2 = pk13_e2(b);
      const uint32_t code = e2 == 0 ? 0u : (uint32_t)(e2 - bh) & 15u;
      lo[e >> 2] |= (b & 0xffu) << (8 * (e & 3));
      hd |= code << (8 * (e & 3) + 4 * (e >> 2));
      s[c >> 2] |= (b >> 15) << ((c & 3) * 2 + (e >> 2) + 8 * (e & 3));
    }
    a[c >> 1][(c & 1) * 2] = lo[0];
    a[c >> 1][(c & 1) * 2 + 1] = lo[1];
    h[c >> 2][c & 3] = hd;
  }
#pragma unroll
  for (int p = 0; p < 4; ++p) *reinterpret_cast<u32x4_t*>(dst + p * 1024 + lane * 16) = a[p];
#pragma unroll
  for (int q = 0; q < 2; ++q) *reinterpret_cast<u32x4_t*>(dst + PK13_OFF_H + q * 1024 + lane * 16) = h[q];
  *reinterpret_cast<pk13_u32x2_t*>(dst + PK13_OFF_S + lane * 8) = pk13_u32x2_t{s[0], s[1]};
}

}

size_t pk13_bytes(int N, int K) { return (size_t)N * (K / PK13_UNIT_K) * PK13_UNIT_BYTES; }

void launch_pk13_stats(const void* w, int64_t n_elems, Pk13Stats* stats, hipStream_t st) {
  const int64_t nvec = n_elems / 8;
  const int grid = (int)std::min<int64_t>((nvec + 255) / 256, 4096);
  hipLaunchKernelGGL(pk13_max_kernel, dim3(grid), dim3(256), 0, st, (const u32x4_t*)w, nvec, stats);
  hipLaunchKernelGGL(pk13_window_kernel, dim3(grid), dim3(256), 0, st, (const u32x4_t*)w, nvec, stats);
}

void launch_pk13_pack(const void* w, int N, int K, int bh, void* out, hipStream_t st) {
  const int64_t nunits = (int64_t)N * (K / PK13_UNIT_K);
  hipLaunchKernelGGL(pk13_pack_kernel, dim3((unsigned)((nunits + 3) / 4)), dim3(256), 0, st, (const bf16_t*)w, nunits, bh, (uint8_t*)out);
}

bool gemv_pk13_shape_ok(int N, int K) { return N >= 1 && K >= PK13_UNIT_K && K % PK13_UNIT_K == 0 && K <= 32768; }

bool gemv_pk13_by_plan(int N, int K, GemvEpi epi) {
  (void)epi;
  return gemv_pk13_shape_ok(N, K) && (int64_t)N * K >= ((int64_t)1 << 25);
}

int gemv_pk13_num_tiles(int N, int K) { (void)K; return plan_gemv_pk13(N, GEMV_LOGITS).grid; }

void debug_plan_gemv_pk13(int N, int K, GemvEpi epi, bool has_norm, int* out5) {
  const GemvPk13Plan p = plan_gemv_pk13(N, epi);
  out5[0] = p.R; out5[1] = 8; out5[2] = p.grid; out5[3] = 1; out5[4] = pro_of(K, has_norm);
}

void launch_gemv_pk13(const GemvArgs& g, const void* packed, int bh, GemvEpi epi, hipStream_t st) {
  if (!gemv_pk13_shape_ok(g.N, g.K)) abort();
  GemvPk13Args a{};
  a.p = packed; a.x = g.x; a.norm_w = g.norm_w; a.residual = g.residual; a.y = g.y; a.y_f32 = g.y_f32;
  a.blk_max = g.blk_max; a.blk_idx = g.blk_idx; a.h_out = g.h_out; a.N = g.N; a.K = g.K; a.bh = bh; a.eps = g.eps;
  const GemvPk13Plan p = plan_gemv_pk13(g.N, epi);
  switch (epi) {
    case GEMV_STORE: launch_pk13_epi<1, GEMV_STORE>(a, p, st); break;
    case GEMV_RESIDUAL: launch_pk13_epi<1, GEMV_RESIDUAL>(a, p, st); break;
    case GEMV_SILU_MUL: launch_pk13_epi<1, GEMV_SILU_MUL>(a, p, st); break;
    case GEMV_LOGITS: launch_pk13_epi<2, GEMV_LOGITS>(a, p, st); break;
    default: abort();
  }
}

}
```

### aha_amd/csrc/model.h

```cpp
#pragma once
#include <hip/hip_runtime.h>

#include <map>
#include <string>
#include <vector>

#include "../../include/aha_hip.h"
#include "kernels.h"

struct aha_ctx {
  int device = 0;
  hipStream_t stream = nullptr;
};

namespace aha {

void set_error(const std::string& msg);
#define AHA_HIP_CHECK(expr)                                                                          \
  do {                                                                                               \
    hipError_t _e = (expr);                                                                          \
    if (_e != hipSuccess) {                                                                          \
      ::aha::set_error(std::string(#expr) + " failed: " + hipGetErrorString(_e));                    \
      return AHA_ERR_HIP;                                                                            \
    }                                                                                                \
  } while (0)

struct Pk13Copy {
  void* p = nullptr;
  int bh = 0;
};
struct Pk13Entry { std::string name; Pk13Copy* slot; std::string status; };

struct LayerWeights {
  void* wqkv = nullptr;
  void* wo = nullptr;
  void* wgu = nullptr;
  void* wdown = nullptr;
  void* in_norm = nullptr;
  void* post_norm = nullptr;
  void* q_norm = nullptr;
  void* k_norm = nullptr;
  WQuant q_wqkv, q_wo, q_wgu, q_wdown;
  Pk13Copy p_wqkv, p_wo, p_wgu, p_wdown;
};

constexpr uint32_t RING_CAP = 256;

struct StepState {
  uint32_t token;
  int32_t pos[3];
  int32_t kv_start;
  int32_t kv_len;
  uint32_t next_token;
  int32_t step;
};

struct ProfRec { int cls; hipEvent_t e0, e1; double bytes, flops; };

struct VisionModel;
struct AudioModel;

}

struct aha_weights {
  struct Mapping { void* base; size_t len; };
  std::vector<Mapping> maps;
  std::vector<std::string> names;
  std::vector<aha_tensor_view> views;
  ~aha_weights();
};

struct aha_model {
  aha_ctx* ctx = nullptr;
  aha_model_desc desc{};
  hipStream_t stream = nullptr;
  void* embed = nullptr;
  void* lm_head = nullptr;
  void* final_norm = nullptr;
  std::vector<aha::LayerWeights> layers;
  std::vector<void*> owned;
  int32_t wq_format = 0;
  uint32_t wq_flags = 0;
  aha::WQuant q_lm_head;
  bool fp8_rows = true;
  int fp8_single = 1;
  aha::Pk13Copy p_lm_head;
  std::vector<aha::Pk13Entry> pk13;
  int pk13_single = 1;
  int fp4_single = 1;
  float* d_inv_freq = nullptr;
  int32_t* d_axis_map = nullptr;
  float* d_rope = nullptr;
  float attn_scale = 0.f;
  std::vector<void*> slabs;
  std::vector<uint64_t> h_page_ptrs;
  uint64_t* d_page_ptrs = nullptr;
  size_t page_table_cap = 0;
  size_t pages_per_slab = 0;
  uint64_t page_bytes = 0;
  uint64_t layer_stride = 0;
  size_t n_pages = 0;
  size_t lin_pages = 0;
  uint64_t lin_p0 = 0;
  int64_t lin_step = 0;
  int last_attn_form = -1;
  size_t cache_len = 0;
  bool scramble_pages = false;
  std::vector<uint64_t> free_pages;
  aha::StepState* d_state = nullptr;
  aha::StepState* h_state = nullptr;
  uint32_t* d_token_log = nullptr;
  size_t token_log_cap = 0;
  uint32_t* h_ring = nullptr;
  uint32_t* h_ring_dev = nullptr;
  uint32_t* h_done = nullptr;
  uint32_t* h_done_dev = nullptr;
  int64_t steps_executed = 0;
  bool rope_delta_valid = false;
  int64_t rope_delta = 0;
  void *d_x = nullptr, *d_qkv = nullptr, *d_q = nullptr, *d_attn = nullptr, *d_act = nullptr, *d_hlast = nullptr;
  float* d_logits = nullptr;
  float* d_blk_max = nullptr;
  uint32_t* d_blk_idx = nullptr;
  float* d_part_o = nullptr;
  float* d_part_ml = nullptr;
  int max_nsplit = 64;
  int tp_rank = 0, tp_size = 1;
  aha_allreduce_fn allreduce_cb = nullptr;
  void* allreduce_user = nullptr;
  aha_reduce_scatter_fn reduce_scatter_cb = nullptr;
  aha_all_gather_fn all_gather_cb = nullptr;
  void* sp_user = nullptr;
  void* rccl_comm = nullptr;
  void* rccl_comm_side = nullptr;
  hipStream_t comm_stream = nullptr;
  bool reserved_cus_set = false;
  hipEvent_t ev_gemm[8] = {};
  hipEvent_t ev_ag[8] = {};
  hipEvent_t ev_comm = nullptr;
  int async_rc = 0;
  int lm_rows = 0, lm_row0 = 0;
  float* d_partial = nullptr;
  float* p_partial = nullptr;
  int cp_rank = 0, cp_size = 1;
  int comm_rank = 0;
  aha_all_gather_fn cp_all_gather_cb = nullptr;
  void* cp_user = nullptr;
  void* p_cp_stage = nullptr;
  std::vector<int32_t> cp_row_map;
  size_t cp_stage_bytes = 0;
  void* p_hstage = nullptr;
  unsigned head_ctr_base = 0;
  unsigned* d_bar = nullptr;
  unsigned long long* d_gemv_trace = nullptr;
  unsigned long long* d_attn_trace = nullptr;
  bool decode_fused = true;
  float* h_logits = nullptr;
  bool have_logits = false;
  bool logits_assembled = false;
  float* d_samp_work = nullptr;
  float* d_samp_f = nullptr;
  unsigned* d_samp_u = nullptr;
  uint32_t* d_samp_ctx = nullptr;
  uint32_t* h_samp = nullptr;
  size_t samp_ctx_cap = 0;
  size_t pf_cap = 0;
  uint32_t* p_ids = nullptr;
  int32_t* p_pos = nullptr;
  void *p_x = nullptr, *p_h = nullptr, *p_qkv = nullptr, *p_q = nullptr, *p_attn = nullptr, *p_act = nullptr;
  void* p_rope = nullptr;
  void* p_gemm_ws = nullptr;
  size_t gemm_ws_bytes = 0;
  void* d_sk_ctrs = nullptr;
  std::vector<void*> pf_owned;
  int32_t* p_pass_tab = nullptr;
  size_t p_pass_tab_cap = 0;
  int32_t* h_pass_stage = nullptr;
  size_t h_pass_stage_cap = 0;
  float* p_pool = nullptr;
  size_t p_pool_cap = 0;
  aha_engine* engine = nullptr;
  aha::VisionModel* vision = nullptr;
// ... 103 lines not shown
```

### aha_amd/csrc/model.hip

```cpp
#include "model.h"
#include "mxfp8.h"

#include <math.h>
#include <stdlib.h>
#include <string.h>

#include <algorithm>
#include <chrono>
#include <deque>

#include "common.h"
#include "audio.h"
#include "sampler.h"
#include "vision.h"

namespace aha {

static thread_local std::string g_last_error;
void set_error(const std::string& msg) { g_last_error = msg; }
const char* last_error_cstr() { return g_last_error.c_str(); }

ProfScope::ProfScope(aha_model* m_, const char* cls, double bytes, double flops) : m(m_) {
  if (!m->profiling) return;
  auto it = m->prof_cls.find(cls);
// ... 372 lines not shown
    set_error("kv_import: the destination model is tensor-parallel (tp_size " + std::to_string(m->tp_size) + "); import into an un-sharded model");
    return AHA_ERR_UNSUPPORTED;
  }
  if (!in_dev || n_heads <= 0 || src_head0 < 0 || dst_head0 < 0 || src_head0 + n_heads > src_heads || dst_head0 + n_heads > c.num_key_value_heads) {
    set_error("kv_import: head ranges out of bounds (buffer holds " + std::to_string(src_heads) + " heads, the model " +
              std::to_string(c.num_key_value_heads) + ")");
    return AHA_ERR_INVALID;
  }
  if (n_tokens == 0) return AHA_OK;
  const size_t pages = (n_tokens + KV_PAGE_TOKENS - 1) / KV_PAGE_TOKENS;
  const size_t need_bytes = (size_t)c.num_hidden_layers * pages * (size_t)src_heads * 2 * KV_BLOCK_BYTES;
  if (in_bytes < need_bytes) {
    set_error("kv_import: the buffer holds " + std::to_string(in_bytes) + " bytes, " + std::to_string(need_bytes) + " are needed for " +
              std::to_string(n_tokens) + " tokens of " + std::to_string(src_heads) + " heads");
    return AHA_ERR_INVALID;
  }
  AHA_HIP_CHECK(hipSetDevice(m->ctx->device));
  int rc = model_ensure_pages(m, n_tokens);
  if (rc) return rc;
  hipLaunchKernelGGL(kv_pack_kernel, dim3((unsigned)pages, (unsigned)c.num_hidden_layers, (unsigned)n_heads * 2), dim3(256), 0, m->stream,
                     m->d_page_ptrs, m->layer_stride, c.num_key_value_heads, (char*)in_dev, src_heads, src_head0, dst_head0, (int)pages, 1);
  AHA_HIP_CHECK(hipGetLastError());
  AHA_HIP_CHECK(hipStreamSynchronize(m->stream));
  m->cache_len = n_tokens;
  m->rope_delta = rope_delta;
  m->rope_delta_valid = true;
  m->have_logits = false;
  m->logits_assembled = false;
  return AHA_OK;
}

static int assemble_logits(aha_model* m);

int model_sample_candidates(aha_model* m, const uint32_t* ctx, size_t n_ctx, float repeat_penalty, float temperature, int k,
                            float* vals_out, uint32_t* idx_out, float* max_out, float* sumexp_out) {
  const int V = m->desc.vocab_size;
  if (!m->have_logits) {
    set_error("sample_candidates: no forward call has produced logits yet");
    return AHA_ERR_STATE;
  }
  if (!sample_shape_ok(V, k)) {
    set_error("sample_candidates: k must be in [1, 64] (and vocab * k within the stage-2 capacity)");
    return AHA_ERR_UNSUPPORTED;
  }
  if (!(repeat_penalty > 0.f) || (n_ctx && !ctx) || !vals_out || !idx_out) {
    set_error("sample_candidates: bad argument");
    return AHA_ERR_INVALID;
  }
  const int nw = sample_stage1_waves(V);
  constexpr size_t OUT_WORDS = 64 + 2 + 64;
  if (!m->d_samp_f) {
    const size_t nc = ((size_t)nw + 16) * 64;
    const size_t nf = nc + 2 * (size_t)nw + OUT_WORDS, nu = nc;
    void *pw = nullptr, *pf = nullptr, *pu = nullptr;
    if (int rc = dev_alloc(m, (size_t)V * 4, &pw, false)) return rc;
    if (int rc = dev_alloc(m, nf * 4, &pf, false)) return rc;
    if (int rc = dev_alloc(m, nu * 4, &pu, false)) return rc;
    m->d_samp_work = (float*)pw;
    m->d_samp_f = (float*)pf;
    m->d_samp_u = (unsigned*)pu;
  }
  if (!m->h_samp || n_ctx > m->samp_ctx_cap) {
    const size_t cap = std::max<size_t>(1024, n_ctx * 2);
    void* pd = nullptr;
    if (int rc = dev_alloc(m, cap * 4, &pd, false)) return rc;
    uint32_t* ph = nullptr;
    AHA_HIP_CHECK(hipHostMalloc((void**)&ph, (cap + OUT_WORDS) * 4));
    if (m->h_samp) hipHostFree(m->h_samp);
    m->h_samp = ph;
    m->d_samp_ctx = (uint32_t*)pd;
    m->samp_ctx_cap = cap;
  }
  if (int rc = assemble_logits(m)) return rc;
  const float* src = m->d_logits;
  if (repeat_penalty != 1.0f && n_ctx > 0) {
    memcpy(m->h_samp, ctx, n_ctx * 4);
    AHA_HIP_CHECK(hipMemcpyAsync(m->d_samp_ctx, m->h_samp, n_ctx * 4, hipMemcpyHostToDevice, m->stream));
    AHA_HIP_CHECK(hipMemcpyAsync(m->d_samp_work, m->d_logits, (size_t)V * 4, hipMemcpyDeviceToDevice, m->stream));
    launch_repeat_penalty(m->d_logits, m->d_samp_work, m->d_samp_ctx, (int)n_ctx, repeat_penalty, V, m->stream);
    src = m->d_samp_work;
  }
  const float inv_temp = temperature > 0.f ? (float)(1.0 / (double)temperature) : 1.0f;
  float* cand_val = m->d_samp_f;
  float* part_m = cand_val + ((size_t)nw + 16) * 64;
  float* part_s = part_m + nw;
  float* out_val = part_s + nw;
  float* out_ms = out_val + 64;
  unsigned* out_idx = reinterpret_cast<unsigned*>(out_ms + 2);
  unsigned* cand_idx = m->d_samp_u;
  launch_topk_candidates(src, V, k, inv_temp, cand_val, cand_idx, part_m, part_s, out_val, out_idx, out_ms, m->stream);
  AHA_HIP_CHECK(hipGetLastError());
  uint32_t* h_out = m->h_samp + m->samp_ctx_cap;
  AHA_HIP_CHECK(hipMemcpyAsync(h_out, out_val, OUT_WORDS * 4, hipMemcpyDeviceToHost, m->stream));
  AHA_HIP_CHECK(hipStreamSynchronize(m->stream));
  memcpy(vals_out, h_out, (size_t)k * 4);
  memcpy(idx_out, h_out + 66, (size_t)k * 4);
  if (max_out) memcpy(max_out, h_out + 64, 4);
  if (sumexp_out) memcpy(sumexp_out, h_out + 65, 4);
  return AHA_OK;
}

int model_last_logits(aha_model* m, float* logits_out) {
  if (!m->have_logits) {
    set_error("last_logits: no forward call has produced logits yet");
    return AHA_ERR_STATE;
  }
  if (int rc = assemble_logits(m)) return rc;
  AHA_HIP_CHECK(hipMemcpyAsync(m->h_logits, m->d_logits, (size_t)m->desc.vocab_size * 4, hipMemcpyDeviceToHost, m->stream));
  AHA_HIP_CHECK(hipStreamSynchronize(m->stream));
  memcpy(logits_out, m->h_logits, (size_t)m->desc.vocab_size * 4);
  return AHA_OK;
}

int model_clear_cache(aha_model* m) {
  for (size_t i = m->n_pages; i > 0; --i) m->free_pages.push_back(m->h_page_ptrs[i - 1]);
  m->n_pages = 0;
  m->lin_pages = 0;
  m->cache_len = 0;
  m->rope_delta = 0;
  m->rope_delta_valid = false;
  return AHA_OK;
}

static void model_free_packed(aha_model* m, const char* why) {
  for (Pk13Entry& e : m->pk13) {
    if (e.slot->p) {
      hipFree(e.slot->p);
      e.status = why;
    }
    *e.slot = Pk13Copy{};
  }
}

static int model_pack_weights(aha_model* m) {
  const aha_model_desc& c = m->desc;
  struct Mat { const void* w; int N, K; };
  std::vector<Mat> mats;
  const int H = c.hidden_size, I = c.intermediate_size, nq = c.num_attention_heads * c.head_dim, nkv = c.num_key_value_heads * c.head_dim;
  for (int li = 0; li < c.num_hidden_layers; ++li) {
    LayerWeights& L = m->layers[li];
    const std::string p = "layers." + std::to_string(li) + ".";
    m->pk13.push_back({p + "self_attn.q_proj/k_proj/v_proj.weight", &L.p_wqkv, ""});
    mats.push_back({L.wqkv, nq + 2 * nkv, H});
    m->pk13.push_back({p + "self_attn.o_proj.weight", &L.p_wo, ""});
    mats.push_back({L.wo, H, nq});
    m->pk13.push_back({p + "mlp.gate_proj/up_proj.weight", &L.p_wgu, ""});
    mats.push_back({L.wgu, 2 * I, H});
    m->pk13.push_back({p + "mlp.down_proj.weight", &L.p_wdown, ""});
    mats.push_back({L.wdown, H, I});
  }
  m->pk13.push_back({c.tie_word_embeddings ? "embed_tokens.weight (tied lm_head)" : "lm_head.weight", &m->p_lm_head, ""});
  mats.push_back({m->lm_head, m->lm_rows, H});
  auto all = [&](const char* why) {
    for (Pk13Entry& e : m->pk13)
      if (e.status.empty()) e.status = why;
    return AHA_OK;
  };
  const char* env = getenv("AHA_WPACK");
  if (env && atoi(env) == 0) return all("off (AHA_WPACK=0)");
  if (m->tp_size > 1 || m->cp_size > 1) return all("sharded model");
  std::vector<size_t> cand;
  for (size_t i = 0; i < mats.size(); ++i) {
    if (!gemv_pk13_shape_ok(mats[i].N, mats[i].K)) m->pk13[i].status = "K is not a multiple of 4096 (or above 32768)";
    else if ((int64_t)mats[i].N * mats[i].K < ((int64_t)1 << 24)) m->pk13[i].status = "fewer than 2^24 elements";
    else cand.push_back(i);
  }
  if (cand.empty()) return AHA_OK;
  hipStream_t st = m->stream;
  std::vector<Pk13Stats> h(cand.size());
  {
    Pk13Stats* d = nullptr;
    if (hipMalloc((void**)&d, cand.size() * sizeof(Pk13Stats)) != hipSuccess) {
      (void)hipGetLastError();
      return all("not enough device memory");
    }
    hipError_t e = hipMemsetAsync(d, 0, cand.size() * sizeof(Pk13Stats), st);
    for (size_t k = 0; k < cand.size() && e == hipSuccess; ++k) launch_pk13_stats(mats[cand[k]].w, (int64_t)mats[cand[k]].N * mats[cand[k]].K, d + k, st);
    if (e == hipSuccess) e = hipGetLastError();
    if (e == hipSuccess) e = hipMemcpyAsync(h.data(), d, cand.size() * sizeof(Pk13Stats), hipMemcpyDeviceToHost, st);
    if (e == hipSuccess) e = hipStreamSynchronize(st);
    hipFree(d);
    AHA_HIP_CHECK(e);
  }
  std::vector<size_t> take;
  size_t bytes = 0;
  for (size_t k = 0; k < cand.size(); ++k) {
    if (h[k].bad) {
      m->pk13[cand[k]].status = std::to_string(h[k].bad) + " weights outside the window (Inf, NaN, or more than 30 binades below the matrix maximum)";
      continue;
    }
    m->pk13[cand[k]].slot->bh = pk13_base(h[k].max_e2);
    take.push_back(cand[k]);
    bytes += pk13_bytes(mats[cand[k]].N, mats[cand[k]].K);
  }
  size_t free_b = 0, total_b = 0;
  if (hipMemGetInfo(&free_b, &total_b) != hipSuccess) {
    (void)hipGetLastError();
    free_b = 0;
  }
  if (take.empty()) return AHA_OK;
  if ((double)free_b < 1.1 * (double)bytes) return all("not enough device memory");
  for (size_t i : take) {
    if (hipMalloc(&m->pk13[i].slot->p, pk13_bytes(mats[i].N, mats[i].K)) != hipSuccess) {
      (void)hipGetLastError();
      m->pk13[i].slot->p = nullptr;
      model_free_packed(m, "not enough device memory");
      return all("not enough device memory");
    }
    launch_pk13_pack(mats[i].w, mats[i].N, mats[i].K, m->pk13[i].slot->bh, m->pk13[i].slot->p, st);
    m->pk13[i].status = "packed";
  }
  hipError_t e = hipGetLastError();
  if (e == hipSuccess) e = hipStreamSynchronize(st);
  AHA_HIP_CHECK(e);
  return AHA_OK;
}

int model_quantize_weights(aha_model* m, int32_t format, uint32_t flags) {
  const aha_model_desc& c = m->desc;
  if (format != AHA_WQ_MXFP8_E4M3 && format != AHA_WQ_MXFP4_E2M1) {
    set_error("quantize_weights: unknown format " + std::to_string(format) + " (AHA_WQ_MXFP8_E4M3 = 1, AHA_WQ_MXFP4_E2M1 = 2)");
    return AHA_ERR_INVALID;
  }
  if (flags & ~(uint32_t)AHA_WQ_LM_HEAD) {
    set_error("quantize_weights: unknown flag bits " + std::to_string(flags & ~(uint32_t)AHA_WQ_LM_HEAD) + " (AHA_WQ_LM_HEAD = 1)");
    return AHA_ERR_INVALID;
  }
  if (m->engine) {
    set_error("quantize_weights: the model has an engine (aha_hip_engine_destroy first)");
    return AHA_ERR_STATE;
  }
  if (m->wq_format != AHA_WQ_NONE) {
    if (m->wq_format == format && m->wq_flags == flags) return AHA_OK;
    set_error("quantize_weights: the model is already quantised with format " + std::to_string(m->wq_format) + ", flags " +
              std::to_string(m->wq_flags));
    return AHA_ERR_STATE;
  }
  if (m->cache_len != 0) {
    set_error("quantize_weights: the cache holds " + std::to_string(m->cache_len) + " tokens (aha_hip_clear_cache first)");
    return AHA_ERR_STATE;
  }
  if (m->tp_size > 1 || m->cp_size > 1) {
    set_error("quantize_weights: tensor- and context-parallel models are not supported");
    return AHA_ERR_UNSUPPORTED;
  }
  if ((c.arch != AHA_ARCH_QWEN3 && c.arch != AHA_ARCH_QWEN3VL && c.arch != AHA_ARCH_QWEN3ASR) || c.head_dim != 128) {
    set_error("quantize_weights: Qwen3, Qwen3-VL and Qwen3-ASR with head_dim 128 only (the models of generate_batch)");
    return AHA_ERR_UNSUPPORTED;
  }
  struct Mat { std::string name; void* w; int N, K; WQuant* slot; };
  std::vector<Mat> mats;
  const int H = c.hidden_size, I = c.intermediate_size, nq = c.num_attention_heads * 128, nkv = c.num_key_value_heads * 128;
  for (int li = 0; li < c.num_hidden_layers; ++li) {
    LayerWeights& L = m->layers[li];
    const std::string p = "layers." + std::to_string(li) + ".";
    mats.push_back({p + "self_attn.q_proj/k_proj/v_proj.weight", L.wqkv, nq + 2 * nkv, H, &L.q_wqkv});
    mats.push_back({p + "self_attn.o_proj.weight", L.wo, H, nq, &L.q_wo});
    mats.push_back({p + "mlp.gate_proj/up_proj.weight", L.wgu, 2 * I, H, &L.q_wgu});
    mats.push_back({p + "mlp.down_proj.weight", L.wdown, H, I, &L.q_wdown});
  }
  if (flags & AHA_WQ_LM_HEAD)
    mats.push_back({c.tie_word_embeddings ? "embed_tokens.weight (tied lm_head)" : "lm_head.weight", m->lm_head, c.vocab_size, H, &m->q_lm_head});
  for (const Mat& t : mats)
    if (t.K % MX_BLOCK) {
      set_error("quantize_weights: " + t.name + " has K = " + std::to_string(t.K) + ", not a multiple of 32 (the MX block)");
      return AHA_ERR_UNSUPPORTED;
    }
  AHA_HIP_CHECK(hipSetDevice(m->ctx->device));
  hipStream_t st = m->stream;
  const bool fp4 = format == AHA_WQ_MXFP4_E2M1;
  {
    int* d_flag = nullptr;
    std::vector<int> h_flag(mats.size(), 0);
    AHA_HIP_CHECK(hipMalloc((void**)&d_flag, mats.size() * sizeof(int)));
    hipError_t e = hipMemsetAsync(d_flag, 0, mats.size() * sizeof(int), st);
    for (size_t i = 0; i < mats.size() && e == hipSuccess; ++i) {
      if (fp4) launch_mxfp4_check(mats[i].w, (int64_t)mats[i].N * mats[i].K, d_flag + i, st);
      else launch_mxfp8_check(mats[i].w, (int64_t)mats[i].N * mats[i].K, d_flag + i, st);
    }
    if (e == hipSuccess) e = hipGetLastError();
    if (e == hipSuccess) e = hipMemcpyAsync(h_flag.data(), d_flag, mats.size() * sizeof(int), hipMemcpyDeviceToHost, st);
    if (e == hipSuccess) e = hipStreamSynchronize(st);
    hipFree(d_flag);
    AHA_HIP_CHECK(e);
    for (size_t i = 0; i < mats.size(); ++i)
      if (h_flag[i]) {
        set_error("quantize_weights: " + mats[i].name + " holds a weight that is not finite (or is " +
                  (fp4 ? "above 1.5 * 2^127" : "1.9375 * 2^127 or more") + " in magnitude); no matrix was modified");
        return AHA_ERR_INVALID;
      }
  }
  std::vector<void*> got;
  std::vector<WQuant> wq(mats.size());
  for (size_t i = 0; i < mats.size(); ++i) {
    const size_t bytes[2] = {(size_t)mats[i].N * mats[i].K / (fp4 ? 2 : 1), mxfp8_scale_words(mats[i].N, mats[i].K) * 4};
    for (int k = 0; k < 2; ++k) {
      void* p = nullptr;
      const hipError_t e = hipMalloc(&p, bytes[k]);
      if (e != hipSuccess) {
        (void)hipGetLastError();
        for (void* q : got) hipFree(q);
        set_error("quantize_weights: hipMalloc of " + std::to_string(bytes[k]) + " bytes for the copy of " + mats[i].name + " failed: " +
                  hipGetErrorString(e) + "; the model is unchanged");
        return e == hipErrorOutOfMemory ? AHA_ERR_OOM : AHA_ERR_HIP;
      }
      got.push_back(p);
      if (k == 0) wq[i].q = p;
      else wq[i].scales = (uint32_t*)p;
    }
  }
  if (const hipError_t es = hipStreamSynchronize(st); es != hipSuccess) {
    for (void* q : got) hipFree(q);
    AHA_HIP_CHECK(es);
  }
  model_free_packed(m, "freed by quantize_weights");
  for (size_t i = 0; i < mats.size(); ++i) {
    if (fp4) launch_mxfp4_quantize(mats[i].w, mats[i].N, mats[i].K, wq[i].q, wq[i].scales, mats[i].w, st);
    else launch_mxfp8_quantize(mats[i].w, mats[i].N, mats[i].K, wq[i].q, wq[i].scales, mats[i].w, st);
  }
  hipError_t e = hipGetLastError();
  if (e == hipSuccess) e = hipStreamSynchronize(st);
  for (void* p : got) m->owned.push_back(p);
  AHA_HIP_CHECK(e);
  for (size_t i = 0; i < mats.size(); ++i) *mats[i].slot = wq[i];
  m->wq_format = format;
  m->wq_flags = flags;
  m->have_logits = false;
  return AHA_OK;
}

int model_create(aha_ctx* ctx, const aha_model_desc* desc, const aha_tensor_view* w, size_t nw, aha_model** out) {
  if (!ctx || !desc || !out || (!w && nw)) {
    set_error("model_create: null argument");
    return AHA_ERR_INVALID;
  }
  const aha_model_desc& cd = *desc;
  if (cd.head_dim != 128) {
    set_error("only head_dim == 128 is supported by the decoder kernels (Qwen3 family)");
    return AHA_ERR_UNSUPPORTED;
  }
  if (cd.hidden_size <= 0 || cd.intermediate_size <= 0 || cd.num_hidden_layers <= 0 || cd.num_attention_heads <= 0 ||
      cd.num_key_value_heads <= 0 || cd.vocab_size <= 0 || cd.n_stop_tokens < 0 || cd.n_stop_tokens > 8 ||
      (cd.arch == AHA_ARCH_QWEN3VL && (cd.vis_spatial_merge_size <= 0 || cd.vis_patch_size <= 0 || cd.vis_num_heads <= 0))) {
    set_error("model_create: sizes must be positive (and at most 8 stop tokens)");
    return AHA_ERR_INVALID;
  }
  if (cd.num_attention_heads % cd.num_key_value_heads || cd.num_attention_heads / cd.num_key_value_heads > 16) {
    set_error("unsupported GQA group size");
    return AHA_ERR_UNSUPPORTED;
  }
  if (cd.hidden_size % 8 || cd.intermediate_size % 16) {
    set_error("hidden_size must be a multiple of 8 and intermediate_size of 16");
    return AHA_ERR_UNSUPPORTED;
  }
  auto ln_covers = [](int64_t dim) { return dim > 0 && dim % 8 == 0 && dim <= 8192; };
  if (cd.arch == AHA_ARCH_QWEN3VL && find_tensor(w, nw, "model.visual.patch_embed.proj.weight")) {
    const int64_t m4 = (int64_t)cd.vis_hidden_size * cd.vis_spatial_merge_size * cd.vis_spatial_merge_size;
    if (!ln_covers(cd.vis_hidden_size) || !ln_covers(m4)) {
      set_error("vision tower: hidden_size " + std::to_string(cd.vis_hidden_size) + " and hidden_size * spatial_merge_size^2 = " + std::to_string(m4) +
                " must be multiples of 8 and at most 8192 (the LayerNorm kernel's row)");
      return AHA_ERR_UNSUPPORTED;
    }
  }
// ... 131 lines not shown
    set_error("model_create: pinned host allocation failed");
    return fail(AHA_ERR_HIP);
  }
  if (hipHostMalloc((void**)&m->h_ring, (RING_CAP + 16) * 4, hipHostMallocMapped | hipHostMallocCoherent) != hipSuccess ||
      hipHostGetDevicePointer((void**)&m->h_ring_dev, m->h_ring, 0) != hipSuccess) {
    set_error("hipHostMalloc (decode token ring) failed");
    return fail(AHA_ERR_OOM);
  }
  memset(m->h_ring, 0, (RING_CAP + 16) * 4);
  m->h_done = m->h_ring + RING_CAP;
  m->h_done_dev = m->h_ring_dev + RING_CAP;
  m->token_log_cap = 1 << 16;
  if ((rc = dev_alloc(m, m->token_log_cap * 4, &p))) return fail(rc);
  m->d_token_log = (uint32_t*)p;
  if ((rc = dev_alloc(m, (size_t)H * 2, &m->d_x))) return fail(rc);
  if ((rc = dev_alloc(m, (size_t)(nq + 2 * nkv) * 2, &m->d_qkv))) return fail(rc);
  if ((rc = dev_alloc(m, (size_t)nq * 2, &m->d_q))) return fail(rc);
  if ((rc = dev_alloc(m, (size_t)nq * 2, &m->d_attn))) return fail(rc);
  if ((rc = dev_alloc(m, (size_t)I * 2, &m->d_act))) return fail(rc);
  if ((rc = dev_alloc(m, (size_t)H * 2, &m->d_hlast, true))) return fail(rc);
  if ((rc = dev_alloc(m, (size_t)H * 4, &p))) return fail(rc);
  m->d_partial = (float*)p;
  if ((rc = dev_alloc(m, (size_t)c.vocab_size * 4, &p))) return fail(rc);
  m->d_logits = (float*)p;
  const int nt = std::max(std::max(std::max(gemv_num_tiles(c.vocab_size, H), gemv_mxfp8_num_tiles(c.vocab_size, H)), gemv_mxfp4_num_tiles(c.vocab_size, H)), std::max(gemv_pk13_num_tiles(c.vocab_size, H), 512));
  if ((rc = dev_alloc(m, (size_t)nt * 4, &p))) return fail(rc);
  m->d_blk_max = (float*)p;
  if ((rc = dev_alloc(m, (size_t)nt * 4, &p))) return fail(rc);
  m->d_blk_idx = (uint32_t*)p;
  if ((rc = dev_alloc(m, (size_t)m->max_nsplit * 4 * c.num_attention_heads * d * 4, &p))) return fail(rc);
  m->d_part_o = (float*)p;
  if ((rc = dev_alloc(m, (size_t)m->max_nsplit * 4 * c.num_attention_heads * 2 * 4, &p))) return fail(rc);
  m->d_part_ml = (float*)p;
  if ((rc = dev_alloc(m, 128 * 4, &p, true))) return fail(rc);
  m->d_rope = (float*)p;

  if ((rc = dev_alloc(m, DECODE_SYNC_BYTES, &p, true))) return fail(rc);
  m->d_bar = (unsigned*)p;
  if ((rc = dev_alloc(m, SK_MAX_COUNTERS * 4, &m->d_sk_ctrs, true))) return fail(rc);

  if (c.arch == AHA_ARCH_QWEN3VL) {
    if ((rc = vision_create(m, w, nw))) return fail(rc);
  }
  if (c.arch == AHA_ARCH_QWEN3ASR) {
    if ((rc = audio_create(m, w, nw))) return fail(rc);
  }
  if ((rc = model_pack_weights(m))) return fail(rc);
  if (hipStreamSynchronize(m->stream) != hipSuccess) {
    set_error(std::string("model_create: ") + hipGetErrorString(hipGetLastError()));
    return fail(AHA_ERR_HIP);
  }
  *out = m;
  return AHA_OK;
}

void model_destroy(aha_model* m) {
  if (!m) return;
  if (m->engine) engine_destroy(m->engine);
  hipStreamSynchronize(m->stream);
  for (auto& r : m->prof) { hipEventDestroy(r.e0); hipEventDestroy(r.e1); }
  vision_destroy(m);
  audio_destroy(m);
  tp_destroy(m);
  model_free_packed(m, "freed");
  for (void* p : m->owned) hipFree(p);
  for (void* p : m->pf_owned) hipFree(p);
  if (m->p_pass_tab) hipFree(m->p_pass_tab);
  if (m->p_pool) hipFree(m->p_pool);
  if (m->h_pass_stage) hipHostFree(m->h_pass_stage);
  for (void* p : m->slabs) hipFree(p);
  if (m->d_page_ptrs) hipFree(m->d_page_ptrs);
  if (m->h_state) hipHostFree(m->h_state);
  if (m->h_ring) hipHostFree(m->h_ring);
  if (m->h_logits) hipHostFree(m->h_logits);
  if (m->h_samp) hipHostFree(m->h_samp);
  delete m;
}

static int ensure_prefill_scratch(aha_model* m, size_t S) {
  if (S <= m->pf_cap) return AHA_OK;
  AHA_HIP_CHECK(hipStreamSynchronize(m->stream));
  for (void* p : m->pf_owned) hipFree(p);
  m->pf_owned.clear();
  m->pf_cap = 0;
  const aha_model_desc& c = m->desc;
  const size_t cap = (S + 255) / 256 * 256;
  const size_t H = c.hidden_size, I = c.intermediate_size, nq = (size_t)c.num_attention_heads * c.head_dim,
               nkv = (size_t)c.num_key_value_heads * c.head_dim;
  auto al = [&](size_t bytes, void** out) -> int {
    void* p = nullptr;
    hipError_t e = hipMalloc(&p, bytes);
    if (e != hipSuccess) {
      set_error(std::string("prefill scratch hipMalloc failed: ") + hipGetErrorString(e));
      return e == hipErrorOutOfMemory ? AHA_ERR_OOM : AHA_ERR_HIP;
    }
    m->pf_owned.push_back(p);
    *out = p;
    return AHA_OK;
  };
  int rc;
  if ((rc = al(cap * 4, (void**)&m->p_ids))) return rc;
  if ((rc = al(cap * 3 * 4, (void**)&m->p_pos))) return rc;
  if ((rc = al(cap * 128 * 2, &m->p_rope))) return rc;
  if ((rc = al(cap * H * 2, &m->p_x))) return rc;
  if ((rc = al((cap + 64) * H * 2, &m->p_h))) return rc;
  if ((rc = al(cap * (nq + 2 * nkv) * 2, &m->p_qkv))) return rc;
  if ((rc = al(cap * nq * 2, &m->p_q))) return rc;
  if ((rc = al(cap * nq * 2, &m->p_attn))) return rc;
  if ((rc = al(cap * I * 2, &m->p_act))) return rc;
  if (m->tp_size > 1 && (rc = al((cap + 64) * H * 4, (void**)&m->p_partial))) return rc;
  if (m->tp_size > 1 && (rc = al((cap + 64) * H * 2, &m->p_hstage))) return rc;
  if (m->cp_size > 1) {
    const size_t pages = cap / KV_PAGE_TOKENS + 1, pmax = pages / m->cp_size + 4;
    m->cp_stage_bytes = std::max((size_t)m->cp_size * pmax * nkv / 128 * 2 * KV_BLOCK_BYTES, (size_t)m->cp_size * H * 2);
    if ((rc = al(m->cp_stage_bytes, &m->p_cp_stage))) return rc;
  }
  m->gemm_ws_bytes = std::min((size_t)12 * cap * H * 4, (size_t)1 << 30);
  if ((rc = al(m->gemm_ws_bytes, &m->p_gemm_ws))) return rc;
  m->pf_cap = cap;
  return AHA_OK;
}

static int push_state(aha_model* m, uint32_t token, const int64_t pos[3], size_t kv_start, size_t kv_len) {
  StepState* s = m->h_state;
  s->token = token;
  for (int i = 0; i < 3; ++i) s->pos[i] = (int32_t)pos[i];
  s->kv_start = (int32_t)kv_start;
  s->kv_len = (int32_t)kv_len;
  s->next_token = 0;
  s->step = 0;
  AHA_HIP_CHECK(hipMemcpyAsync(m->d_state, s, sizeof(StepState), hipMemcpyHostToDevice, m->stream));
  return AHA_OK;
}

static void gemv_row_parallel(aha_model* m, GemvArgs g);

static bool fp8_single(const aha_model* m, const WQuant& wq, int rows, int K, GemvEpi epi) {
  return wq.q != nullptr && m->wq_format == AHA_WQ_MXFP8_E4M3 && m->tp_size <= 1 && (m->fp8_single == 2 || (m->fp8_single == 1 && gemv_mxfp8_by_plan(rows, K, epi)));
}
static bool fp4_single(const aha_model* m, const WQuant& wq, int rows, int K, GemvEpi epi) {
  return wq.q != nullptr && m->wq_format == AHA_WQ_MXFP4_E2M1 && m->tp_size <= 1 && (m->fp4_single == 2 || (m->fp4_single == 1 && gemv_mxfp4_by_plan(rows, K, epi)));
}
static bool pk13_single(const aha_model* m, const Pk13Copy& pk, int rows, int K, GemvEpi epi) {
  return pk.p != nullptr && m->wq_format == AHA_WQ_NONE && m->tp_size <= 1 && gemv_pk13_shape_ok(rows, K) &&
         (m->pk13_single == 2 || (m->pk13_single == 1 && gemv_pk13_by_plan(rows, K, epi)));
}
static void decode_gemv(aha_model* m, const GemvArgs& g, GemvEpi epi, const WQuant& wq, const Pk13Copy& pk, double act_bytes) {
  const double weights = (epi == GEMV_SILU_MUL ? 2.0 : 1.0) * g.N * g.K;
  const int rows = (epi == GEMV_SILU_MUL ? 2 : 1) * g.N;
  const bool fp8 = fp8_single(m, wq, rows, g.K, epi), fp4 = fp4_single(m, wq, rows, g.K, epi), p13 = pk13_single(m, pk, rows, g.K, epi);
  ProfScope ps(m, fp8 ? "gemv_fp8" : fp4 ? "gemv_fp4" : "gemv", weights * (fp8 ? 1.03125 : fp4 ? 0.53125 : p13 ? 1.625 : 2.0) + act_bytes, 2.0 * weights);
  if (fp8) launch_gemv_mxfp8(g, wq.q, wq.scales, epi, m->stream);
  else if (fp4) launch_gemv_mxfp4(g, wq.q, wq.scales, epi, m->stream);
  else if (p13) launch_gemv_pk13(g, pk.p, pk.bh, epi, m->stream);
  else if (epi == GEMV_RESIDUAL) gemv_row_parallel(m, g);
  else launch_gemv(g, epi, m->stream);
}
static int lm_head_partials(const aha_model* m) {
  const int N = m->lm_rows, K = m->desc.hidden_size;
  if (fp8_single(m, m->q_lm_head, N, K, GEMV_LOGITS)) return gemv_mxfp8_num_tiles(N, K);
  if (fp4_single(m, m->q_lm_head, N, K, GEMV_LOGITS)) return gemv_mxfp4_num_tiles(N, K);
  if (pk13_single(m, m->p_lm_head, N, K, GEMV_LOGITS)) return gemv_pk13_num_tiles(N, K);
  return gemv_num_tiles(N, K);
}

static void enqueue_lm_head(aha_model* m, const void* x_last, bool argmax = true) {
  const aha_model_desc& c = m->desc;
  GemvArgs g{};
  g.W = m->lm_head;
  g.x = x_last;
  g.norm_w = m->final_norm;
  g.eps = c.rms_norm_eps;
  g.N = m->lm_rows;
  g.K = c.hidden_size;
  g.y_f32 = m->d_logits + m->lm_row0;
  g.blk_max = m->d_blk_max;
  g.blk_idx = m->d_blk_idx;
  g.h_out = m->d_hlast;
  decode_gemv(m, g, GEMV_LOGITS, m->q_lm_head, m->p_lm_head, c.hidden_size * 2 + m->lm_rows * 4.0);
  if (!argmax) return;
  ProfScope ps(m, "argmax", 0, 0);
  const int ntiles = lm_head_partials(m);
  if (m->lm_rows == c.vocab_size) {
    launch_argmax_partials(m->d_blk_max, m->d_blk_idx, ntiles, &m->d_state->next_token, m->stream);
    return;
  }
  launch_argmax_pair(m->d_blk_max, m->d_blk_idx, ntiles, m->lm_row0, m->d_partial, m->tp_rank, m->tp_size, m->stream);
  const int rc = model_allreduce(m, m->d_partial, (size_t)2 * m->tp_size);
  if (rc && !m->async_rc) m->async_rc = rc;
  launch_argmax_pick(m->d_partial, m->tp_size, &m->d_state->next_token, m->stream);
}

static void gemv_trace_dump(aha_model* m);

static int assemble_logits(aha_model* m) {
  const aha_model_desc& c = m->desc;
  if (m->lm_rows == c.vocab_size || m->logits_assembled) return AHA_OK;
  if (m->lm_row0 > 0) AHA_HIP_CHECK(hipMemsetAsync(m->d_logits, 0, (size_t)m->lm_row0 * 4, m->stream));
  const int tail0 = m->lm_row0 + m->lm_rows;
  if (tail0 < c.vocab_size) AHA_HIP_CHECK(hipMemsetAsync(m->d_logits + tail0, 0, (size_t)(c.vocab_size - tail0) * 4, m->stream));
  const int rc = model_allreduce(m, m->d_logits, (size_t)c.vocab_size);
  if (rc) return rc;
  m->logits_assembled = true;
  return AHA_OK;
}

static int fetch_outputs(aha_model* m, float* logits_out, uint32_t* argmax_out) {
  const aha_model_desc& c = m->desc;
  m->have_logits = true;
  m->logits_assembled = false;
  if (logits_out) {
    const int rc = assemble_logits(m);
    if (rc) return rc;
  }
  if (logits_out) AHA_HIP_CHECK(hipMemcpyAsync(m->h_logits, m->d_logits, (size_t)c.vocab_size * 4, hipMemcpyDeviceToHost, m->stream));
  AHA_HIP_CHECK(hipMemcpyAsync(&m->h_state->next_token, &m->d_state->next_token, 4, hipMemcpyDeviceToHost, m->stream));
  AHA_HIP_CHECK(hipStreamSynchronize(m->stream));
  if (m->d_gemv_trace) gemv_trace_dump(m);
  if (m->d_attn_trace) {
    const int L = m->desc.num_hidden_layers;
    std::vector<unsigned long long> t((size_t)L * 12);
    if (hipMemcpy(t.data(), m->d_attn_trace, t.size() * 8, hipMemcpyDeviceToHost) == hipSuccess) {
      for (int b = 0; b < 2; ++b) {
        double v[5] = {};
        int n = 0;
        for (int li = 1; li < L; ++li) {
          const unsigned long long* p = t.data() + (size_t)li * 12 + b * 6;
          if (p[0] == 0 || p[4] == 0) continue;
          for (int k = 0; k < 5; ++k) v[k] += (p[k + 1] > p[k] ? (double)(p[k + 1] - p[k]) : 0.0) * 0.01;
          ++n;
        }
        if (n) fprintf(stderr, "[attn trace] block %d: prologue %.2f | pages %.2f | merge+publish %.2f | arrive %.2f | final merge %.2f us\n", b, v[0] / n, v[1] / n, v[2] / n, v[3] / n, v[4] / n);
      }
      double dstart = 0.0, arr[2] = {};
      int n = 0;
      for (int li = 1; li < L; ++li) {
        const unsigned long long* p = t.data() + (size_t)li * 12;
        if (p[0] == 0 || p[4] == 0 || p[6] == 0 || p[10] == 0) continue;
        const unsigned long long t0 = std::min(p[0], p[6]);
        dstart += ((double)p[6] - (double)p[0]) * 0.01;
        arr[0] += (double)(p[4] - t0) * 0.01;
        arr[1] += (double)(p[10] - t0) * 0.01;
        ++n;
      }
      if (n) fprintf(stderr, "[attn trace] start of block 1 - start of block 0 %+.2f | arrival after the earlier start: block 0 %.2f | block 1 %.2f us\n", dstart / n, arr[0] / n, arr[1] / n);
    }
  }
  if (logits_out) memcpy(logits_out, m->h_logits, (size_t)c.vocab_size * 4);
  if (argmax_out) *argmax_out = m->h_state->next_token;
  return AHA_OK;
}


int model_allreduce(aha_model* m, float* buf, size_t count) {
  if (m->tp_size <= 1) return AHA_OK;
  ProfScope ps(m, "allreduce", (double)count * 4, 0);
  if (m->rccl_comm) return rccl_allreduce(m, buf, count);
  if (!m->allreduce_cb) {
    set_error("tp_size > 1 but no all-reduce was installed (aha_hip_set_allreduce / aha_hip_tp_init_rccl)");
    return AHA_ERR_STATE;
  }
  AHA_HIP_CHECK(hipStreamSynchronize(m->stream));
  if (m->allreduce_cb(buf, count, m->allreduce_user) != 0) {
    set_error("all-reduce callback failed");
    return AHA_ERR_STATE;
  }
  return AHA_OK;
}
static bool seq_parallel_on(const aha_model* m) {
  static const bool env_on = [] { const char* e = getenv("AHA_TP_SP"); return e ? atoi(e) != 0 : true; }();
  return env_on && m->tp_size > 1 && (m->rccl_comm || (m->reduce_scatter_cb && m->all_gather_cb));
}
static int model_reduce_scatter(aha_model* m, float* buf, size_t count_per_rank) {
  ProfScope ps(m, "reduce_scatter", (double)count_per_rank * m->tp_size * 4, 0);
  if (m->rccl_comm) return rccl_reduce_scatter(m, buf, count_per_rank);
  AHA_HIP_CHECK(hipStreamSynchronize(m->stream));
  if (m->reduce_scatter_cb(buf, count_per_rank, m->sp_user) != 0) {
    set_error("reduce-scatter callback failed");
    return AHA_ERR_STATE;
  }
  return AHA_OK;
}
static int model_all_gather(aha_model* m, void* buf, size_t bytes_per_rank) {
  ProfScope ps(m, "all_gather", (double)bytes_per_rank * m->tp_size, 0);
  if (m->rccl_comm) return rccl_all_gather(m, buf, bytes_per_rank);
  AHA_HIP_CHECK(hipStreamSynchronize(m->stream));
  if (m->all_gather_cb(buf, bytes_per_rank, m->sp_user) != 0) {
    set_error("all-gather callback failed");
    return AHA_ERR_STATE;
  }
  return AHA_OK;
}
static void gemv_row_parallel(aha_model* m, GemvArgs g) {
  if (m->tp_size <= 1) {
    launch_gemv(g, GEMV_RESIDUAL, m->stream);
    return;
  }
  g.y_f32 = m->d_partial;
  launch_gemv(g, GEMV_PARTIAL_F32, m->stream);
  const int rc = model_allreduce(m, m->d_partial, (size_t)g.N);
  if (rc && !m->async_rc) m->async_rc = rc;
  launch_residual_add_f32(g.y, m->d_partial, g.N, m->stream);
}
static int tp_overlap_chunks(const aha_model* m, const GemmArgs& g) {
  const char* e = getenv("AHA_TP_OVERLAP_CHUNKS");
  const char* er = getenv("AHA_TP_OVERLAP_MIN_ROWS");
  int nch = e ? atoi(e) : 4;
// ... 2609 lines not shown
```

### aha_amd/ops.py

```python
from __future__ import annotations

import ctypes as C
import math
from typing import Optional

import numpy as np
import torch

from . import _lib
from ._lib import check, lib


def _ptr(t: Optional[torch.Tensor]):
    return None if t is None else t.data_ptr()


def _stream():
    return torch.cuda.current_stream().cuda_stream


def _chk(*ts):
    for t in ts:
        if t is None:
            continue
# ... 300 lines not shown
    out = torch.empty(128, samples.numel() // 160, dtype=torch.float32, device=samples.device)
    check(lib().aha_hip_logmel(_ptr(samples), samples.numel(), _ptr(out), _stream()))
    return out


def logmel_batch(clips) -> torch.Tensor:
    assert len(clips) > 0
    for c in clips:
        _chk(c)
        assert c.dtype == torch.float32 and c.dim() == 1
    flat = torch.cat([c.reshape(-1) for c in clips]).contiguous()
    n = np.ascontiguousarray([c.numel() for c in clips], dtype=np.int64)
    out = torch.empty(128, int((n // 160).sum()), dtype=torch.float32, device=flat.device)
    check(lib().aha_hip_logmel_batch(_ptr(flat), n.ctypes.data, len(clips), _ptr(out), _stream()))
    return out


GEMV_ROWS_STORE, GEMV_ROWS_RESIDUAL, GEMV_ROWS_SILU_MUL, GEMV_ROWS_LOGITS = 0, 1, 2, 3


def gemv_rows(W: torch.Tensor, x: torch.Tensor, epi: int = GEMV_ROWS_STORE, residual: Optional[torch.Tensor] = None):
    _chk(W, x, residual)
    N, K = W.shape
    R = x.shape[0]
    y = logits = am = None
    if epi == GEMV_ROWS_LOGITS:
        logits = torch.empty(R, N, dtype=torch.float32, device=x.device)
        am = torch.empty(R, dtype=torch.int32, device=x.device)
    else:
        y = torch.empty(R, N // 2 if epi == GEMV_ROWS_SILU_MUL else N, dtype=torch.bfloat16, device=x.device)
    check(lib().aha_hip_gemv_rows(_ptr(W), _ptr(x), _ptr(y), R, N, K, epi, _ptr(residual), _ptr(logits), _ptr(am), _stream()))
    return (logits, am.long()) if epi == GEMV_ROWS_LOGITS else y


def _quantize_mx(entry, W: torch.Tensor, k_per_byte: int):
    from . import quant
    _chk(W)
    N, K = W.shape
    q = torch.empty(N, K // k_per_byte, dtype=torch.uint8, device=W.device)
    words = torch.empty(N, (K + 127) // 128, dtype=torch.int32, device=W.device)
    wr = torch.empty_like(W)
    check(entry(_ptr(W), N, K, _ptr(q), _ptr(words), _ptr(wr), _stream()))
    return q, quant.scales_from_kernel(words, K).to(W.device), wr


def _gemv_rows_mx(entry, q: torch.Tensor, K: int, scales: torch.Tensor, x: torch.Tensor, epi: int, residual: Optional[torch.Tensor]):
    from . import quant
    _chk(q, x, residual)
    N, R = q.shape[0], x.shape[0]
    words = quant.scales_to_kernel(scales).to(x.device)
    y = logits = am = None
    if epi == GEMV_ROWS_LOGITS:
        logits = torch.empty(R, N, dtype=torch.float32, device=x.device)
        am = torch.empty(R, dtype=torch.int32, device=x.device)
    else:
        y = torch.empty(R, N // 2 if epi == GEMV_ROWS_SILU_MUL else N, dtype=torch.bfloat16, device=x.device)
    check(entry(_ptr(q), _ptr(words), _ptr(x), _ptr(y), R, N, K, epi, _ptr(residual), _ptr(logits), _ptr(am), _stream()))
    return (logits, am.long()) if epi == GEMV_ROWS_LOGITS else y


def quantize_mxfp8(W: torch.Tensor):
    return _quantize_mx(lib().aha_hip_quantize_mxfp8, W, 1)


def gemv_rows_mxfp8(q: torch.Tensor, scales: torch.Tensor, x: torch.Tensor, epi: int = GEMV_ROWS_STORE, residual: Optional[torch.Tensor] = None):
    return _gemv_rows_mx(lib().aha_hip_gemv_rows_mxfp8, q, q.shape[1], scales, x, epi, residual)


def quantize_mxfp4(W: torch.Tensor):
    return _quantize_mx(lib().aha_hip_quantize_mxfp4, W, 2)


def gemv_rows_mxfp4(q: torch.Tensor, scales: torch.Tensor, x: torch.Tensor, epi: int = GEMV_ROWS_STORE, residual: Optional[torch.Tensor] = None):
    _chk(q, x, residual)
    N, K = q.shape[0], q.shape[1] * 2
    if scales.shape != (N, K // 32) or x.shape[1] != K:
        raise ValueError(f"gemv_rows_mxfp4: q {tuple(q.shape)} wants scales ({N}, {K // 32}) and x (R, {K})")
    return _gemv_rows_mx(lib().aha_hip_gemv_rows_mxfp4, q, K, scales, x, epi, residual)


def _gemv_epi_outputs(N: int, epi: int, device, out: Optional[torch.Tensor]):
    y = logits = am = None
    if epi == GEMV_ROWS_LOGITS:
        logits = torch.empty(N, dtype=torch.float32, device=device)
        am = torch.empty(1, dtype=torch.int32, device=device)
    else:
        y = out if out is not None else torch.empty(N // 2 if epi == GEMV_ROWS_SILU_MUL else N, dtype=torch.bfloat16, device=device)
    return y, logits, am


def gemv_epi(W: torch.Tensor, x: torch.Tensor, epi: int = GEMV_ROWS_STORE, norm_w: Optional[torch.Tensor] = None, eps: float = 1e-6,
             residual: Optional[torch.Tensor] = None, out: Optional[torch.Tensor] = None):
    _chk(W, x, norm_w, residual, out)
    N, K = W.shape
    y, logits, am = _gemv_epi_outputs(N, epi, x.device, out)
    check(lib().aha_hip_gemv_epi(_ptr(W), _ptr(x), _ptr(y), N, K, epi, _ptr(norm_w), eps, _ptr(residual), _ptr(logits), _ptr(am), _stream()))
    return (logits, int(am.item())) if epi == GEMV_ROWS_LOGITS else y


def plan_gemv(N: int, K: int, epi: int = GEMV_ROWS_STORE, has_norm: bool = False):
    r, u, g, f = C.c_int32(), C.c_int32(), C.c_int32(), C.c_int32()
    check(lib().aha_hip_debug_plan_gemv(N, K, epi, int(has_norm), C.byref(r), C.byref(u), C.byref(g), C.byref(f)))
    return r.value, u.value, g.value, f.value


def gemv_partial_f32(W: torch.Tensor, x: torch.Tensor, norm_w: Optional[torch.Tensor] = None, eps: float = 1e-6) -> torch.Tensor:
    _chk(W, x, norm_w)
    N, K = W.shape
    y = torch.empty(N, dtype=torch.float32, device=x.device)
    check(lib().aha_hip_debug_gemv_partial_f32(_ptr(W), _ptr(x), _ptr(y), N, K, _ptr(norm_w), eps, _stream()))
    return y


def gemv_mxfp8(q: torch.Tensor, scales: torch.Tensor, x: torch.Tensor, epi: int = GEMV_ROWS_STORE, norm_w: Optional[torch.Tensor] = None,
               eps: float = 1e-6, residual: Optional[torch.Tensor] = None, out: Optional[torch.Tensor] = None):
    from . import quant
    _chk(q, x, norm_w, residual, out)
    N, K = q.shape
    words = quant.scales_to_kernel(scales).to(x.device)
    y, logits, am = _gemv_epi_outputs(N, epi, x.device, out)
    check(lib().aha_hip_gemv_mxfp8(_ptr(q), _ptr(words), _ptr(x), _ptr(y), N, K, epi, _ptr(norm_w), eps, _ptr(residual), _ptr(logits), _ptr(am),
                                   _stream()))
    return (logits, int(am.item())) if epi == GEMV_ROWS_LOGITS else y


def plan_gemv_mxfp8(N: int, K: int, epi: int = GEMV_ROWS_STORE, has_norm: bool = False):
    r, u, g, f = C.c_int32(), C.c_int32(), C.c_int32(), C.c_int32()
    check(lib().aha_hip_debug_plan_gemv_mxfp8(N, K, epi, int(has_norm), C.byref(r), C.byref(u), C.byref(g), C.byref(f), None))
    return r.value, u.value, g.value, f.value


def gemv_mxfp8_by_plan(N: int, K: int, epi: int = GEMV_ROWS_STORE) -> bool:
    r, b = C.c_int32(), C.c_int32()
    check(lib().aha_hip_debug_plan_gemv_mxfp8(N, K, epi, 0, C.byref(r), C.byref(r), C.byref(r), None, C.byref(b)))
    return bool(b.value)


def pack_pk13(W: torch.Tensor, check_only: bool = False):
    _chk(W)
    N, K = W.shape
    bh, bad = C.c_int32(), C.c_int64()
    out = None if check_only else torch.zeros(N, K // 4096, 6656, dtype=torch.uint8, device=W.device)
    check(lib().aha_hip_pack_pk13(_ptr(W), N, K, _ptr(out), C.byref(bh), C.byref(bad), _stream()))
    return (out if bad.value == 0 else None), bh.value, bad.value


def gemv_pk13(packed: torch.Tensor, bh: int, x: torch.Tensor, epi: int = GEMV_ROWS_STORE, norm_w: Optional[torch.Tensor] = None,
              eps: float = 1e-6, residual: Optional[torch.Tensor] = None, out: Optional[torch.Tensor] = None):
    _chk(packed, x, norm_w, residual, out)
    N, K = packed.shape[0], packed.shape[1] * 4096
    y, logits, am = _gemv_epi_outputs(N, epi, x.device, out)
    check(lib().aha_hip_gemv_pk13(_ptr(packed), bh, _ptr(x), _ptr(y), N, K, epi, _ptr(norm_w), eps, _ptr(residual), _ptr(logits), _ptr(am),
                                  _stream()))
    return (logits, int(am.item())) if epi == GEMV_ROWS_LOGITS else y


def plan_gemv_pk13(N: int, K: int, epi: int = GEMV_ROWS_STORE, has_norm: bool = False):
    r, u, g, f = C.c_int32(), C.c_int32(), C.c_int32(), C.c_int32()
    check(lib().aha_hip_debug_plan_gemv_pk13(N, K, epi, int(has_norm), C.byref(r), C.byref(u), C.byref(g), C.byref(f), None))
    return r.value, u.value, g.value, f.value


def gemv_pk13_by_plan(N: int, K: int, epi: int = GEMV_ROWS_STORE) -> bool:
    if N < 1 or K < 4096 or K % 4096 or K > 32768:
        return False
    r, b = C.c_int32(), C.c_int32()
    check(lib().aha_hip_debug_plan_gemv_pk13(N, K, epi, 0, C.byref(r), C.byref(r), C.byref(r), None, C.byref(b)))
    return bool(b.value)


def gemv_mxfp4(q: torch.Tensor, scales: torch.Tensor, x: torch.Tensor, epi: int = GEMV_ROWS_STORE, norm_w: Optional[torch.Tensor] = None,
               eps: float = 1e-6, residual: Optional[torch.Tensor] = None, out: Optional[torch.Tensor] = None):
    from . import quant
    _chk(q, x, norm_w, residual, out)
    N, K = q.shape[0], q.shape[1] * 2
    if scales.shape != (N, K // 32) or x.shape[0] != K:
        raise ValueError(f"gemv_mxfp4: q {tuple(q.shape)} wants scales ({N}, {K // 32}) and x ({K})")
    words = quant.scales_to_kernel(scales).to(x.device)
    y, logits, am = _gemv_epi_outputs(N, epi, x.device, out)
    check(lib().aha_hip_gemv_mxfp4(_ptr(q), _ptr(words), _ptr(x), _ptr(y), N, K, epi, _ptr(norm_w), eps, _ptr(residual), _ptr(logits), _ptr(am),
                                   _stream()))
    return (logits, int(am.item())) if epi == GEMV_ROWS_LOGITS else y


def plan_gemv_mxfp4(N: int, K: int, epi: int = GEMV_ROWS_STORE, has_norm: bool = False):
    r, u, g, f = C.c_int32(), C.c_int32(), C.c_int32(), C.c_int32()
    check(lib().aha_hip_debug_plan_gemv_mxfp4(N, K, epi, int(has_norm), C.byref(r), C.byref(u), C.byref(g), C.byref(f), None))
    return r.value, u.value, g.value, f.value


def gemv_mxfp4_by_plan(N: int, K: int, epi: int = GEMV_ROWS_STORE) -> bool:
    r, b = C.c_int32(), C.c_int32()
    check(lib().aha_hip_debug_plan_gemv_mxfp4(N, K, epi, 0, C.byref(r), C.byref(r), C.byref(r), None, C.byref(b)))
    return bool(b.value)


def attn_decode_batch(qkv: torch.Tensor, q_norm_w: torch.Tensor, k_norm_w: torch.Tensor, rope: torch.Tensor, page_ptrs: torch.Tensor,
                      page0, kv_len, nh: int, kvh: int, eps: float, scale: float) -> torch.Tensor:
    _chk(qkv, q_norm_w, k_norm_w, rope, page_ptrs)
    R = qkv.shape[0]
    p0 = np.ascontiguousarray(np.asarray(page0, dtype=np.int32))
    kl = np.ascontiguousarray(np.asarray(kv_len, dtype=np.int32))
    o = torch.empty(R, nh * 128, dtype=torch.bfloat16, device=qkv.device)
    check(lib().aha_hip_attn_decode_batch(_ptr(qkv), _ptr(q_norm_w), _ptr(k_norm_w), _ptr(rope), _ptr(page_ptrs), p0.ctypes.data,
                                          kl.ctypes.data, R, nh, kvh, eps, scale, _ptr(o), _stream()))
    return o


def debug_attn_decode_fused(qkv_row: torch.Tensor, q_norm_w: torch.Tensor, k_norm_w: torch.Tensor, rope_row: torch.Tensor,
                            page_ptrs: torch.Tensor, kv_len: int, nh: int, kvh: int, eps: float, scale: float) -> torch.Tensor:
    _chk(qkv_row, q_norm_w, k_norm_w, rope_row, page_ptrs)
    o = torch.empty(nh * 128, dtype=torch.bfloat16, device=qkv_row.device)
    check(lib().aha_hip_debug_attn_decode_fused(_ptr(qkv_row), _ptr(q_norm_w), _ptr(k_norm_w), _ptr(rope_row), _ptr(page_ptrs), int(kv_len),
                                                nh, kvh, eps, scale, _ptr(o), _stream()))
    return o


def sample_rows(logits: torch.Tensor, k, temperature, repeat_penalty, contexts):
    _chk(logits)
    assert logits.dtype == torch.float32 and logits.dim() == 2 and logits.stride(1) == 1
    R, V = logits.shape
    kk = np.ascontiguousarray(np.asarray(k, dtype=np.int32).reshape(R))
    tt = np.ascontiguousarray(np.asarray(temperature, dtype=np.float32).reshape(R))
    pp = np.ascontiguousarray(np.asarray(repeat_penalty, dtype=np.float32).reshape(R))
    off = np.ascontiguousarray(np.cumsum([0] + [len(c) for c in contexts]), dtype=np.uint64)
    ctx = np.ascontiguousarray(np.concatenate([np.asarray(c, dtype=np.uint32).reshape(-1) for c in contexts] + [np.zeros(1, np.uint32)]))
    vals = torch.empty(R, 64, dtype=torch.float32, device=logits.device)
    idx = torch.empty(R, 64, dtype=torch.int32, device=logits.device)
    ms = torch.empty(R, 2, dtype=torch.float32, device=logits.device)
    check(lib().aha_hip_sample_rows(_ptr(logits), logits.stride(0), R, V, kk.ctypes.data, tt.ctypes.data, pp.ctypes.data, ctx.ctypes.data,
                                    off.ctypes.data, _ptr(vals), _ptr(idx), _ptr(ms), _stream()))
    return vals, idx, ms


def sample_rows_adjusted(logits: torch.Tensor, k, temperature, repeat_penalty, contexts, adjusts):
    if not logits.is_cuda:
        raise ValueError("op inputs must be GPU tensors")
    assert logits.dtype == torch.float32 and logits.dim() == 2 and logits.stride(1) == 1 and logits.stride(0) >= logits.shape[1]
    R, V = logits.shape
    assert len(adjusts) == R
    kk = np.ascontiguousarray(np.asarray(k, dtype=np.int32).reshape(R))
    tt = np.ascontiguousarray(np.asarray(temperature, dtype=np.float32).reshape(R))
    pp = np.ascontiguousarray(np.asarray(repeat_penalty, dtype=np.float32).reshape(R))
    off = np.ascontiguousarray(np.cumsum([0] + [len(c) for c in contexts]), dtype=np.uint64)
    ctx = np.ascontiguousarray(np.concatenate([np.asarray(c, dtype=np.uint32).reshape(-1) for c in contexts] + [np.zeros(1, np.uint32)]))
    aoff = np.ascontiguousarray(np.cumsum([0] + [len(a[0]) for a in adjusts]), dtype=np.uint64)
    aid = np.ascontiguousarray(np.concatenate([np.asarray(a[0], dtype=np.uint32).reshape(-1) for a in adjusts] + [np.zeros(1, np.uint32)]))
    aval = np.ascontiguousarray(np.concatenate([np.asarray(a[1], dtype=np.float32).reshape(-1) for a in adjusts] + [np.zeros(1, np.float32)]))
    vals = torch.empty(R, 64, dtype=torch.float32, device=logits.device)
    idx = torch.empty(R, 64, dtype=torch.int32, device=logits.device)
    ms = torch.empty(R, 2, dtype=torch.float32, device=logits.device)
    check(lib().aha_hip_sample_rows_adjusted(_ptr(logits), logits.stride(0), R, V, kk.ctypes.data, tt.ctypes.data, pp.ctypes.data,
                                             ctx.ctypes.data, off.ctypes.data, aid.ctypes.data, aval.ctypes.data, aoff.ctypes.data, _ptr(vals),
                                             _ptr(idx), _ptr(ms), _stream()))
    return vals, idx, ms


def logprob_rows(logits: torch.Tensor, tokens, n_top):
    if not logits.is_cuda:
        raise ValueError("op inputs must be GPU tensors")
    assert logits.dtype == torch.float32 and logits.dim() == 2 and logits.stride(1) == 1 and logits.stride(0) >= logits.shape[1]
    R, V = logits.shape
    nn = np.ascontiguousarray(np.broadcast_to(np.asarray(n_top, dtype=np.int32), (R,)))
    tok = torch.as_tensor(np.asarray(tokens, dtype=np.int64).reshape(R), dtype=torch.int64).to(torch.int32).to(logits.device)
    out = torch.empty(R, 42, dtype=torch.int32, device=logits.device)
    check(lib().aha_hip_logprob_rows(_ptr(logits), logits.stride(0), R, V, _ptr(tok), nn.ctypes.data, _ptr(out), _stream()))
    o = out.cpu().numpy()
    return (o[:, 0].copy().view(np.float32), o[:, 1].copy(), o[:, 2:22].copy().view(np.uint32), o[:, 22:42].copy().view(np.float32))


def sample_rows_masked(logits: torch.Tensor, k, temperature, repeat_penalty, contexts, adjusts, masks: torch.Tensor, mask_rows):
    if not logits.is_cuda or not masks.is_cuda:
        raise ValueError("op inputs must be GPU tensors")
    assert logits.dtype == torch.float32 and logits.dim() == 2 and logits.stride(1) == 1 and logits.stride(0) >= logits.shape[1]
    R, V = logits.shape
    W = (V + 31) // 32
    assert masks.dim() == 2 and masks.shape[1] == W and masks.is_contiguous() and masks.element_size() == 4
    mr = np.ascontiguousarray(np.asarray(mask_rows, dtype=np.int32).reshape(R))
    assert ((mr >= -1) & (mr < masks.shape[0])).all(), "mask_rows name masks that do not exist"
    adjusts = [([], [])] * R if adjusts is None else adjusts
    assert len(adjusts) == R
    kk = np.ascontiguousarray(np.asarray(k, dtype=np.int32).reshape(R))
    tt = np.ascontiguousarray(np.asarray(temperature, dtype=np.float32).reshape(R))
    pp = np.ascontiguousarray(np.asarray(repeat_penalty, dtype=np.float32).reshape(R))
    off = np.ascontiguousarray(np.cumsum([0] + [len(c) for c in contexts]), dtype=np.uint64)
    ctx = np.ascontiguousarray(np.concatenate([np.asarray(c, dtype=np.uint32).reshape(-1) for c in contexts] + [np.zeros(1, np.uint32)]))
    aoff = np.ascontiguousarray(np.cumsum([0] + [len(a[0]) for a in adjusts]), dtype=np.uint64)
    aid = np.ascontiguousarray(np.concatenate([np.asarray(a[0], dtype=np.uint32).reshape(-1) for a in adjusts] + [np.zeros(1, np.uint32)]))
    aval = np.ascontiguousarray(np.concatenate([np.asarray(a[1], dtype=np.float32).reshape(-1) for a in adjusts] + [np.zeros(1, np.float32)]))
    vals = torch.empty(R, 64, dtype=torch.float32, device=logits.device)
    idx = torch.empty(R, 64, dtype=torch.int32, device=logits.device)
    ms = torch.empty(R, 2, dtype=torch.float32, device=logits.device)
    check(lib().aha_hip_sample_rows_masked(_ptr(logits), logits.stride(0), R, V, kk.ctypes.data, tt.ctypes.data, pp.ctypes.data, ctx.ctypes.data,
                                           off.ctypes.data, aid.ctypes.data, aval.ctypes.data, aoff.ctypes.data, _ptr(masks), mr.ctypes.data,
                                           _ptr(vals), _ptr(idx), _ptr(ms), _stream()))
    return vals, idx, ms
```

### aha_amd/quant.py

```python
from typing import Tuple

import torch

BLOCK = 32
EXP_MIN, EXP_MAX = -117, 120
E4M3_MAX = 448.0


def _blocks(W: torch.Tensor) -> torch.Tensor:
    if W.dim() != 2 or W.shape[1] % BLOCK:
        raise ValueError(f"quantize_mxfp8 wants a (N, K) matrix with K a multiple of {BLOCK}")
    if W.dtype != torch.bfloat16:
        raise ValueError("quantize_mxfp8 wants bf16 weights")
    return W.detach().cpu().float().reshape(W.shape[0], W.shape[1] // BLOCK, BLOCK)


def block_exponents(W: torch.Tensor) -> torch.Tensor:
    amax = _blocks(W).abs().amax(-1)
    if not bool(torch.isfinite(amax).all()):
        raise ValueError("quantize_mxfp8: non-finite weight")
    f, x = torch.frexp(amax)
    e = x.to(torch.int32) - 9 + (f > 0.875).to(torch.int32)
    e = torch.where(amax == 0, torch.full_like(e, EXP_MIN), e)
    return e.clamp(EXP_MIN, EXP_MAX)


def quantize_mxfp8(W: torch.Tensor) -> Tuple[torch.Tensor, torch.Tensor, torch.Tensor]:
    b = _blocks(W)
    e = block_exponents(W)
    v = b * torch.exp2(-e.float())[..., None]
    q8 = v.to(torch.float8_e4m3fn)
    q = q8.view(torch.uint8).reshape(W.shape)
    wr = (q8.float() * torch.exp2(e.float())[..., None]).reshape(W.shape)
    wb = wr.bfloat16()
    if not bool((wb.float() == wr).all()):
        raise ValueError("quantize_mxfp8: a weight of 1.9375 * 2^127 or more in magnitude does not survive the round trip")
    return q.contiguous(), (e + 127).to(torch.uint8).contiguous(), wb.contiguous()


def dequantize_mxfp8(q: torch.Tensor, scales: torch.Tensor) -> torch.Tensor:
    N, K = q.shape
    v = q.cpu().contiguous().view(torch.float8_e4m3fn).float().reshape(N, K // BLOCK, BLOCK)
    e = scales.cpu().to(torch.int32) - 127
    return (v * torch.exp2(e.float())[..., None]).reshape(N, K).bfloat16()


E2M1_GRID = (0.0, 0.5, 1.0, 1.5, 2.0, 3.0, 4.0, 6.0)
EXP4_MIN, EXP4_MAX = -125, 125
E2M1_MAX = 6.0


def _blocks4(W: torch.Tensor) -> torch.Tensor:
    if W.dim() != 2 or W.shape[1] % BLOCK:
        raise ValueError(f"quantize_mxfp4 wants a (N, K) matrix with K a multiple of {BLOCK}")
    if W.dtype != torch.bfloat16:
        raise ValueError("quantize_mxfp4 wants bf16 weights")
    b = W.detach().cpu().double().reshape(W.shape[0], W.shape[1] // BLOCK, BLOCK)
    if not bool(torch.isfinite(b).all()):
        raise ValueError("quantize_mxfp4: non-finite weight")
    if bool((b.abs() > 1.5 * 2.0 ** 127).any()):
        raise ValueError("quantize_mxfp4: a weight above 1.5 * 2^127 in magnitude would round past 6 * 2^125")
    return b


def block_exponents_mxfp4(W: torch.Tensor) -> torch.Tensor:
    amax = _blocks4(W).abs().amax(-1)
    f, x = torch.frexp(amax)
    e = x.to(torch.int32) - 3 + (f > 0.75).to(torch.int32)
    e = torch.where(amax == 0, torch.full_like(e, EXP4_MIN), e)
    return e.clamp(EXP4_MIN, EXP4_MAX)


def pack_nibbles(codes: torch.Tensor) -> torch.Tensor:
    c = codes.cpu().to(torch.uint8)
    return (c[:, 0::2] | (c[:, 1::2] << 4)).contiguous()


def unpack_nibbles(q: torch.Tensor) -> torch.Tensor:
    q = q.cpu()
    return torch.stack((q & 0xf, q >> 4), dim=-1).reshape(q.shape[0], -1).contiguous()


def quantize_mxfp4(W: torch.Tensor) -> Tuple[torch.Tensor, torch.Tensor, torch.Tensor]:
    b = _blocks4(W)
    e = block_exponents_mxfp4(W)
    s = torch.exp2(e.double())[..., None]
    v = b.abs() / s
    idx = ((v > 0.25).to(torch.uint8) + (v >= 0.75).to(torch.uint8) + (v > 1.25).to(torch.uint8) + (v >= 1.75).to(torch.uint8) +
           (v > 2.5).to(torch.uint8) + (v >= 3.5).to(torch.uint8) + (v > 5.0).to(torch.uint8))
    neg = torch.signbit(b)
    codes = (idx | (neg.to(torch.uint8) << 3)).reshape(W.shape)
    mag = torch.tensor(E2M1_GRID, dtype=torch.float64)[idx.long()] * s
    wr = torch.where(neg, -mag, mag).reshape(W.shape)
    wb = wr.bfloat16()
    assert bool((wb.double() == wr).all())
    return pack_nibbles(codes), (e + 127).to(torch.uint8).contiguous(), wb.contiguous()


def dequantize_mxfp4(q: torch.Tensor, scales: torch.Tensor) -> torch.Tensor:
    codes = unpack_nibbles(q)
    N, K = codes.shape
    mag = torch.tensor(E2M1_GRID, dtype=torch.float64)[(codes & 7).long()].reshape(N, K // BLOCK, BLOCK)
    e = scales.cpu().to(torch.int32) - 127
    w = (mag * torch.exp2(e.double())[..., None]).reshape(N, K)
    return torch.where((codes & 8) != 0, -w, w).bfloat16()


def scales_to_kernel(scales: torch.Tensor) -> torch.Tensor:
    N, nb = scales.shape
    nc = (nb + 3) // 4
    s = torch.full((N, nc * 4), 127, dtype=torch.uint8)
    s[:, :nb] = scales.cpu()
    return s.view(torch.int32).reshape(N, nc).contiguous()


def scales_from_kernel(words: torch.Tensor, K: int) -> torch.Tensor:
    N = words.shape[0]
    return words.cpu().contiguous().view(torch.uint8).reshape(N, -1)[:, :K // BLOCK].contiguous()


PK13_UNIT_K = 4096
PK13_UNIT_BYTES = 6656
PK13_OFF_H, PK13_OFF_S = 4096, 6144


def _bf16_bits(W: torch.Tensor) -> torch.Tensor:
    assert W.dtype == torch.bfloat16 and W.dim() == 2
    return W.contiguous().view(torch.int16).to(torch.int32) & 0xffff


def check_pk13(W: torch.Tensor) -> Tuple[int, int]:
    bits = _bf16_bits(W)
    e2 = (bits >> 8) & 0x7f
    nonfinite = (bits & 0x7f80) == 0x7f80
    finite_e2 = e2[~nonfinite]
    bh = max(int(finite_e2.max()) - 15, 0) if finite_e2.numel() else 0
    bad = int(nonfinite.sum()) + int((~nonfinite & (e2 != 0) & (e2 <= bh)).sum())
    return bh, bad


def pack_pk13(W: torch.Tensor, bh: int) -> torch.Tensor:
    N, K = W.shape
    assert K % PK13_UNIT_K == 0 and 0 <= bh <= 112
    J = K // PK13_UNIT_K
    bits = _bf16_bits(W).reshape(N, J, 8, 64, 8)
    lo, e2, sg = bits & 0xff, (bits >> 8) & 0x7f, bits >> 15
    h = torch.where(e2 == 0, torch.zeros_like(e2), (e2 - bh) & 15)
    a = lo.reshape(N, J, 4, 2, 64, 8).permute(0, 1, 2, 4, 3, 5).reshape(N, J, 4 * 64 * 16)
    nib = h[..., 0:4] | (h[..., 4:8] << 4)
    hp = nib.reshape(N, J, 2, 4, 64, 4).permute(0, 1, 2, 4, 3, 5).reshape(N, J, 2 * 64 * 16)
    s5 = sg.reshape(N, J, 2, 4, 64, 2, 4)
    sb = torch.zeros(N, J, 2, 64, 4, dtype=torch.int32, device=W.device)
    for cc in range(4):
        for half in range(2):
            sb |= s5[:, :, :, cc, :, half, :] << (cc * 2 + half)
    sp = sb.permute(0, 1, 3, 2, 4).reshape(N, J, 64 * 8)
    return torch.cat([a, hp, sp], dim=2).to(torch.uint8)


def unpack_pk13(P: torch.Tensor, bh: int) -> torch.Tensor:
    N, J, B = P.shape
    assert B == PK13_UNIT_BYTES
    P = P.to(torch.int32)
    lo = P[:, :, :PK13_OFF_H].reshape(N, J, 4, 64, 2, 8).permute(0, 1, 2, 4, 3, 5).reshape(N, J, 8, 64, 8)
    nib = P[:, :, PK13_OFF_H:PK13_OFF_S].reshape(N, J, 2, 64, 4, 4).permute(0, 1, 2, 4, 3, 5).reshape(N, J, 8, 64, 4)
    h = torch.cat([nib & 15, nib >> 4], dim=-1)
    sb = P[:, :, PK13_OFF_S:].reshape(N, J, 64, 2, 4).permute(0, 1, 3, 2, 4)
    sg = torch.zeros(N, J, 2, 4, 64, 2, 4, dtype=torch.int32)
    for cc in range(4):
        for half in range(2):
            sg[:, :, :, cc, :, half, :] = (sb >> (cc * 2 + half)) & 1
    sg = sg.reshape(N, J, 8, 64, 8)
    e2 = torch.where(h == 0, torch.zeros_like(h), h + bh)
    bits = (sg << 15) | (e2 << 8) | lo
    return bits.reshape(N, J * PK13_UNIT_K).to(torch.int16).view(torch.bfloat16)
```

### include/aha_hip.h

```cpp
#ifndef AHA_HIP_H
#define AHA_HIP_H

#include <stddef.h>
#include <stdint.h>

#ifdef __cplusplus
extern "C" {
#endif

typedef struct aha_ctx aha_ctx;
typedef struct aha_model aha_model;

enum aha_status {
  AHA_OK = 0,
  AHA_ERR_INVALID = -1,
  AHA_ERR_HIP = -2,
  AHA_ERR_OOM = -3,
  AHA_ERR_SHAPE = -4,
  AHA_ERR_MISSING_WEIGHT = -5,
  AHA_ERR_UNSUPPORTED = -6,
  AHA_ERR_STATE = -7
};

enum aha_dtype { AHA_BF16 = 0, AHA_F16 = 1, AHA_F32 = 2, AHA_U32 = 3, AHA_U8 = 4 };
// ... 177 lines not shown
int aha_hip_sampler_plan(const aha_sampler* s, size_t vocab_size, size_t n_generated, int32_t* k_out, float* temperature_out,
                         float* repeat_penalty_out, size_t* n_context_out);
int aha_hip_sampler_pick(aha_sampler* s, const float* vals, const uint32_t* idx, int32_t k, float max, float sumexp, const float* logits,
                         size_t vocab_size, const uint32_t* generated, size_t n_generated, uint32_t* token_out);
uint64_t aha_hip_sampler_rng_words(const aha_sampler* s);

#define AHA_MAX_LOGIT_BIAS 1024
typedef struct aha_logit_adjust {
  float presence_penalty;
  float frequency_penalty;
  const uint32_t* bias_ids;
  const float* bias_vals;
  size_t n_bias;
} aha_logit_adjust;
int aha_hip_generate_batch_adjusted(aha_model* m, const uint32_t* input_ids, const size_t* seq_lens, size_t n_seqs,
                                    const aha_mm_input* const* mm, const aha_sampling_params* params, const aha_logit_adjust* adjust,
                                    const int32_t* top_logprobs, size_t max_new, size_t max_tokens_per_pass, uint32_t* tokens_out,
                                    size_t* n_out, float* step_logits_out, aha_token_logprobs* logprobs_out);
int aha_hip_engine_submit_adjusted(aha_engine* e, const uint32_t* input_ids, size_t n_ids, const aha_mm_input* mm,
                                   const aha_sampling_params* params, const aha_logit_adjust* adjust, size_t max_new, int32_t top_logprobs,
                                   uint64_t* req_id);
int aha_hip_sampler_set_adjust(aha_sampler* s, const aha_logit_adjust* adjust);
int aha_hip_sampler_adjust_list(aha_sampler* s, size_t vocab_size, const uint32_t* generated, size_t n_generated, uint32_t* ids_out,
                                float* vals_out, size_t cap, size_t* n_out);

typedef int (*aha_token_mask_fn)(void* user, size_t seq, const uint32_t* generated, size_t n_generated, uint32_t* mask_words,
                                 size_t n_words);
int aha_hip_generate_batch_masked(aha_model* m, const uint32_t* input_ids, const size_t* seq_lens, size_t n_seqs,
                                  const aha_mm_input* const* mm, const aha_sampling_params* params, const aha_logit_adjust* adjust,
                                  const int32_t* top_logprobs, size_t max_new, size_t max_tokens_per_pass, aha_token_mask_fn mask_fn,
                                  void* mask_user, uint32_t* tokens_out, size_t* n_out, float* step_logits_out,
                                  aha_token_logprobs* logprobs_out);
int aha_hip_engine_submit_masked(aha_engine* e, const uint32_t* input_ids, size_t n_ids, const aha_mm_input* mm,
                                 const aha_sampling_params* params, const aha_logit_adjust* adjust, const uint32_t* mask_words,
                                 size_t n_mask_words, size_t max_new, int32_t top_logprobs, uint64_t* req_id);
int aha_hip_engine_set_mask(aha_engine* e, uint64_t req_id, const uint32_t* words, size_t n_words);
int aha_hip_sampler_set_mask(aha_sampler* s, const uint32_t* words, size_t n_words);

typedef struct aha_weights aha_weights;
int aha_hip_config_parse(const char* model_dir, aha_model_desc* out);
int aha_hip_config_torch_dtype(const char* model_dir, char* out, size_t cap);
int aha_hip_weights_open(const char* model_dir, aha_weights** out);
size_t aha_hip_weights_count(const aha_weights* w);
int aha_hip_weights_get(const aha_weights* w, size_t index, aha_tensor_view* out);
void aha_hip_weights_close(aha_weights* w);
int aha_hip_model_load(aha_ctx* ctx, const char* model_dir, size_t kv_reserve_tokens, aha_model** out);

int aha_hip_forward_initial(aha_model* m, const uint32_t* input_ids, size_t n_ids, size_t seqlen_offset,
                            const aha_mm_input* mm, float* logits_out, uint32_t* argmax_out);
int aha_hip_forward_step(aha_model* m, uint32_t token, size_t seqlen_offset, float* logits_out, uint32_t* argmax_out);
int aha_hip_clear_cache(aha_model* m);
int aha_hip_stop_token_ids(const aha_model* m, uint32_t* out, size_t cap);

int aha_hip_decode_greedy(aha_model* m, uint32_t first_token, size_t seqlen_offset, size_t max_new, uint32_t* tokens_out);

int aha_hip_sample_candidates(aha_model* m, const uint32_t* context, size_t n_context, float repeat_penalty, float temperature,
                              int32_t k, float* vals_out, uint32_t* idx_out, float* max_out, float* sumexp_out);

int aha_hip_last_logits(aha_model* m, float* logits_out);

typedef struct aha_rng aha_rng;
int aha_hip_rng_create(uint64_t seed, aha_rng** out);
void aha_hip_rng_destroy(aha_rng* rng);
uint32_t aha_hip_rng_next_u32(aha_rng* rng);
int aha_hip_rng_weighted_index(aha_rng* rng, const float* weights, size_t n, uint32_t* index_out);
int aha_hip_debug_chacha_block(const uint32_t* state16, int rounds, uint32_t* out16);

int aha_hip_vision_encode(aha_model* m, const aha_mm_input* mm, void* out_dev, int64_t* n_tokens);

typedef int (*aha_allreduce_fn)(void* buf_f32_dev, size_t count, void* user);
int aha_hip_set_allreduce(aha_model* m, aha_allreduce_fn fn, void* user);
int aha_hip_tp_unique_id(void* out128);
int aha_hip_tp_init_rccl(aha_model* m, const void* unique_id128);
typedef int (*aha_reduce_scatter_fn)(void* buf_f32_dev, size_t count_per_rank, void* user);
typedef int (*aha_all_gather_fn)(void* buf_dev, size_t bytes_per_rank, void* user);
int aha_hip_set_seq_parallel(aha_model* m, aha_reduce_scatter_fn reduce_scatter, aha_all_gather_fn all_gather, void* user);
int aha_hip_set_context_parallel(aha_model* m, int32_t rank, int32_t world, aha_all_gather_fn all_gather, void* user);
int aha_hip_cp_init_rccl(aha_model* m, const void* unique_id128);
int aha_hip_debug_cp_plan(int32_t n_tokens, int32_t world, int32_t rank, int32_t* out5);
int aha_hip_kv_export(aha_model* m, void* out_dev, size_t out_bytes, size_t* bytes_needed, size_t* n_tokens, int64_t* rope_delta);
int aha_hip_kv_import(aha_model* m, const void* in_dev, size_t in_bytes, int32_t src_heads, int32_t src_head0, int32_t dst_head0,
                      int32_t n_heads, size_t n_tokens, int64_t rope_delta);
int aha_hip_debug_allreduce(aha_model* m, void* buf_f32_dev, size_t count);

#define AHA_WQ_NONE 0
#define AHA_WQ_MXFP8_E4M3 1
#define AHA_WQ_MXFP4_E2M1 2
#define AHA_WQ_LM_HEAD 1u
int aha_hip_model_quantize_weights(aha_model* m, int32_t format, uint32_t flags);
int aha_hip_model_weight_format(const aha_model* m, int32_t* format, uint32_t* flags);
int aha_hip_debug_fp8_rows(aha_model* m, int on);
int aha_hip_debug_fp8_single(aha_model* m, int on);
int aha_hip_debug_fp4_single(aha_model* m, int on);
int aha_hip_debug_pk13_single(aha_model* m, int on);
int aha_hip_pk13_status(const aha_model* m, char* buf, size_t cap);

size_t aha_hip_cache_len(const aha_model* m);
int64_t aha_hip_debug_steps_executed(const aha_model* m);
int aha_hip_debug_graph_step(aha_model* m, int32_t replays, double* us_launches, double* us_graph);
int aha_hip_set_profiling(aha_model* m, int enable);
int aha_hip_get_profile(aha_model* m, const char* kernel_class, double* total_ms, int64_t* launches, double* bytes,
                        double* flops);
int aha_hip_debug_scramble_pages(aha_model* m, int enable);
int aha_hip_debug_attn_decode_form(const aha_model* m);
int aha_hip_debug_last_hidden(aha_model* m, float* out, size_t n);
int aha_hip_debug_poison_lds(uint32_t seed, void* stream);
int aha_hip_debug_gemm_grouped(const void* A, const void* W, void* C, int32_t M, int32_t N, int32_t K, int32_t ldc, int32_t act,
                               int32_t groups, int32_t a_gstride, int32_t c_gstride, int32_t c_row0, int32_t m_total, void* stream);
int aha_hip_debug_attn_variant(int32_t smx);
int aha_hip_debug_attn_form(int32_t form);
int aha_hip_debug_gemm_plan(int32_t tile, int32_t splitk);
int aha_hip_debug_plan_gemm(int32_t M, int32_t N, int32_t K, int32_t act, int32_t has_bias, int32_t has_residual, size_t workspace_bytes,
                            int32_t* out3);
int aha_hip_debug_streamk_plan(int32_t M, int32_t N, int32_t K, int32_t tile_n, int32_t workers, size_t workspace_bytes, int32_t* out,
                               int32_t cap, int32_t* off_out, int32_t* info7);
int aha_hip_debug_plan_gemv_mxfp8(int32_t N, int32_t K, int32_t epi, int32_t has_norm, int32_t* R, int32_t* U, int32_t* grid, int32_t* form,
                                  int32_t* by_plan);
int aha_hip_debug_plan_gemv_pk13(int32_t N, int32_t K, int32_t epi, int32_t has_norm, int32_t* R, int32_t* U, int32_t* grid, int32_t* form,
                                 int32_t* by_plan);
int aha_hip_debug_plan_gemv_mxfp4(int32_t N, int32_t K, int32_t epi, int32_t has_norm, int32_t* R, int32_t* U, int32_t* grid, int32_t* form,
                                  int32_t* by_plan);
int aha_hip_debug_plan_gemv(int32_t N, int32_t K, int32_t epi, int32_t has_norm, int32_t* R, int32_t* U, int32_t* grid, int32_t* form);
int aha_hip_debug_gemv_partial_f32(const void* W, const void* x, float* y_f32, int32_t N, int32_t K, const void* norm_w, float eps,
                                   void* stream);
int aha_hip_set_gemm_reserved_cus(int32_t n);
int aha_hip_debug_image_embeds(aha_model* m, int which , float* out, size_t n);

int aha_hip_rmsnorm(const void* x, const void* w, void* y, int64_t rows, int32_t dim, float eps, void* stream);
int aha_hip_gemv(const void* W, const void* x, void* y, int32_t N, int32_t K, const void* norm_w, float eps,
                 const void* residual, void* stream);
int aha_hip_gemv_gate_up(const void* Wg, const void* Wu, const void* x, void* y, int32_t I, int32_t K,
                         const void* norm_w, float eps, void* stream);
int aha_hip_gemm(const void* A, const void* W, void* C, int32_t M, int32_t N, int32_t K, int32_t lda, int32_t ldw,
                 int32_t ldc, const void* bias, const void* residual, int32_t act, void* stream);
int aha_hip_qknorm_rope(const void* qkv, const void* q_norm_w, const void* k_norm_w, const int32_t* pos,
                        const int32_t* axis_map, void* q_out, void* k_out, void* v_out, int32_t S, int32_t nh,
                        int32_t kvh, int32_t d, float eps, float theta, void* stream);
int aha_hip_attn_decode(const void* q, const void* k, const void* v, void* o, int32_t nh, int32_t kvh, int32_t d,
                        int32_t L, float scale, void* stream);
int aha_hip_gemv_rows(const void* W, const void* x, void* y, int32_t R, int32_t N, int32_t K, int32_t epi, const void* residual,
                      float* logits, uint32_t* argmax_out, void* stream);
int aha_hip_quantize_mxfp8(const void* W, int32_t N, int32_t K, void* q_out, uint32_t* scales_out, void* w_roundtrip_out, void* stream);
int aha_hip_gemv_epi(const void* W, const void* x, void* y, int32_t N, int32_t K, int32_t epi, const void* norm_w, float eps,
                     const void* residual, float* logits, uint32_t* argmax_out, void* stream);
int aha_hip_gemv_mxfp8(const void* q, const uint32_t* scales, const void* x, void* y, int32_t N, int32_t K, int32_t epi, const void* norm_w,
                       float eps, const void* residual, float* logits, uint32_t* argmax_out, void* stream);
int aha_hip_gemv_rows_mxfp8(const void* q, const uint32_t* scales, const void* x, void* y, int32_t R, int32_t N, int32_t K, int32_t epi,
                            const void* residual, float* logits, uint32_t* argmax_out, void* stream);
int aha_hip_gemv_mxfp4(const void* q, const uint32_t* scales, const void* x, void* y, int32_t N, int32_t K, int32_t epi, const void* norm_w,
                       float eps, const void* residual, float* logits, uint32_t* argmax_out, void* stream);
int aha_hip_pack_pk13(const void* W, int32_t N, int32_t K, void* out, int32_t* bh_out, int64_t* bad_out, void* stream);
int aha_hip_gemv_pk13(const void* packed, int32_t bh, const void* x, void* y, int32_t N, int32_t K, int32_t epi, const void* norm_w,
                      float eps, const void* residual, float* logits, uint32_t* argmax_out, void* stream);
int aha_hip_quantize_mxfp4(const void* W, int32_t N, int32_t K, void* q_out, uint32_t* scales_out, void* w_roundtrip_out, void* stream);
int aha_hip_gemv_rows_mxfp4(const void* q, const uint32_t* scales, const void* x, void* y, int32_t R, int32_t N, int32_t K, int32_t epi,
                            const void* residual, float* logits, uint32_t* argmax_out, void* stream);
int aha_hip_attn_decode_batch(const void* qkv, const void* q_norm_w, const void* k_norm_w, const float* rope, const uint64_t* page_ptrs,
                              const int32_t* page0, const int32_t* kv_len, int32_t rows, int32_t nh, int32_t kvh, float eps, float scale,
                              void* o, void* stream);
int aha_hip_debug_attn_decode_fused(const void* qkv, const void* q_norm_w, const void* k_norm_w, const float* rope, const uint64_t* page_ptrs,
                                    int32_t kv_len, int32_t nh, int32_t kvh, float eps, float scale, void* o, void* stream);
int aha_hip_sample_rows(const float* logits, int64_t ld, int32_t R, int32_t V, const int32_t* k, const float* temperature,
                        const float* repeat_penalty, const uint32_t* context, const size_t* context_offsets, float* vals_out,
                        uint32_t* idx_out, float* ms_out, void* stream);
int aha_hip_logprob_rows(const float* logits, int64_t ld, int32_t R, int32_t V, const uint32_t* tokens, const int32_t* n_top,
                         aha_token_logprobs* out, void* stream);
int aha_hip_sample_rows_adjusted(const float* logits, int64_t ld, int32_t R, int32_t V, const int32_t* k, const float* temperature,
                                 const float* repeat_penalty, const uint32_t* context, const size_t* context_offsets,
                                 const uint32_t* adj_ids, const float* adj_vals, const size_t* adj_offsets, float* vals_out,
                                 uint32_t* idx_out, float* ms_out, void* stream);
int aha_hip_sample_rows_masked(const float* logits, int64_t ld, int32_t R, int32_t V, const int32_t* k, const float* temperature,
                               const float* repeat_penalty, const uint32_t* context, const size_t* context_offsets, const uint32_t* adj_ids,
                               const float* adj_vals, const size_t* adj_offsets, const uint32_t* masks, const int32_t* mask_rows,
                               float* vals_out, uint32_t* idx_out, float* ms_out, void* stream);
int aha_hip_attn_prefill(const void* q, const void* k, const void* v, void* o, int32_t S, int32_t L, int32_t nh,
                         int32_t kvh, int32_t d, int32_t kv_offset, int32_t causal, float scale, void* stream);
int aha_hip_debug_attn_prefill_segs(const void* q, const void* k, const void* v, void* o, int32_t nh, int32_t kvh, const int32_t* segs,
                                    int32_t n_seg, int32_t with_kv0, float scale, void* stream);
#define AHA_ROPE_FORM_TABLE 0
#define AHA_ROPE_FORM_NO_TABLE 1
#define AHA_ROPE_FORM_DEVICE_START 2
#define AHA_ROPE_FORM_PACKED 3
int aha_hip_debug_prefill_rope(const void* qkv, const void* q_norm_w, const void* k_norm_w, const int32_t* pos, const int32_t* axis_map,
                               const float* inv_freq, const uint64_t* page_ptrs, int32_t n_page_ptrs, int32_t S, int32_t nh, int32_t kvh,
                               int32_t d, float eps, int32_t form, int32_t kv_start, int32_t skip_q, const int32_t* row_slot,
                               const int32_t* page_rows, int32_t n_pages, void* rope_tab, void* q_out, void* stream);
int aha_hip_debug_prefill_attn_qfuse(const void* qkv, const void* q_norm_w, const void* rope_tab, const uint64_t* page_ptrs,
                                     int32_t n_page_ptrs, int32_t S, int32_t nh, int32_t kvh, int32_t d, float eps, float scale,
                                     int32_t kv_offset, int32_t kv_total, int32_t S2, int32_t kv_offset2, int32_t kv_total2,
                                     const int32_t* segs, int32_t n_seg, int32_t with_kv0, void* o, void* stream);
int aha_hip_debug_layernorm_rows(const void* x, const void* w, const void* b, void* y, int64_t rows, int32_t dim, float eps, void* stream);
int aha_hip_debug_gemm_layernorm(const void* A, const void* W, void* C, int32_t M, int32_t N, int32_t K, int32_t lda, int32_t ldw, int32_t ldc,
                                 const void* bias, const void* residual, int32_t act, const void* norm_w, const void* norm_b, void* norm_out,
                                 float eps, void* stream);
int aha_hip_debug_vit_pos_embed(const uint32_t* grid_thw, int32_t n_grids, int32_t G, int32_t merge, const void* table, void* x, int64_t N,
                                int32_t D, int32_t* idx_out, float* wt_out, void* stream);
int aha_hip_debug_vit_rope(const void* qkv, const uint32_t* grid_thw, int32_t n_grids, int32_t merge, const float* inv_freq,
                           const uint64_t* page_ptrs, int32_t n_page_ptrs, int64_t N, int32_t nh, int32_t hd, float* cs_tab, void* q_out,
                           int32_t* rowcol_out, int32_t* page_of_out, int32_t* slot_of_out, void* stream);
int aha_hip_debug_scatter_rows(void* dst, const void* src, const int32_t* rows, int64_t n, int64_t dst_rows, int32_t D, int32_t add, void* stream);
int aha_hip_debug_audio_im2col1(const float* feat, int64_t ld, const int32_t* chunks, int32_t C, int32_t mels, int32_t win, void* out, void* stream);
int aha_hip_debug_im2col_nhwc(const void* in, void* out, int32_t B, int32_t Hin, int32_t Win, int32_t Cin, void* stream);
int aha_hip_debug_audio_tokens_gather(const void* in, void* out, int32_t B, int32_t Fq, int32_t T, int32_t Cc, void* stream);
int aha_hip_debug_sinus_pe_add(void* x, int64_t rows, int32_t d, int32_t T, void* stream);
int aha_hip_debug_kv_pack_generic(const void* src, int64_t ld, int32_t k_off, int32_t v_off, const uint64_t* page_ptrs, int32_t n_page_ptrs,
                                  int32_t N, int32_t nh, int32_t hd, const int32_t* slot_of, void* stream);
int aha_hip_img_smart_resize(uint32_t h, uint32_t w, uint32_t factor, uint32_t min_pixels, uint32_t max_pixels, uint32_t* h_out,
                             uint32_t* w_out);
int aha_hip_video_smart_resize(uint32_t num_frames, uint32_t h, uint32_t w, uint32_t temporal_factor, uint32_t factor, uint32_t min_pixels,
                               uint32_t max_pixels, uint32_t video_ratio, uint32_t* h_out, uint32_t* w_out);
int aha_hip_video_sample_frames(uint32_t total_frames, float rate, uint32_t fps, uint32_t min_frames, uint32_t max_frames,
                                uint32_t* nframes_out, uint32_t* interval_out);
int64_t aha_hip_video_timestamps(const uint32_t* frame_indices, size_t n, float fps, uint32_t t_merge_size, float* out, size_t cap);
int aha_hip_image_resize(const uint8_t* src_hwc, int32_t H, int32_t W, uint8_t* dst_hwc, int32_t new_h, int32_t new_w, void* stream);
int aha_hip_debug_resize_taps(int32_t n_in, int32_t n_out, int32_t* left, int32_t* count, float* weights, int64_t weights_cap);
int64_t aha_hip_debug_resample_taps(int32_t orig, int32_t new_f, float* taps, int64_t cap, int32_t* width, int32_t* klen);
int aha_hip_image_to_patches(const uint8_t* img_hwc, void* out, int32_t H, int32_t W, int32_t patch, int32_t merge,
                             const float mean[3], const float std[3], void* stream);
int aha_hip_video_to_patches(const uint8_t* frames_thwc, void* out, int32_t T, int32_t H, int32_t W, int32_t patch, int32_t merge,
                             const float mean[3], const float std[3], void* stream);
int aha_hip_logmel(const float* samples, int64_t n_samples, float* out, void* stream);
int aha_hip_logmel_batch(const float* samples, const int64_t* n_samples, size_t n_clips, float* out, void* stream);
int64_t aha_hip_audio_resample(aha_ctx* ctx, const float* pcm, int64_t n_frames, int32_t channels, int32_t orig_sr,
                               int32_t target_sr, float* out, int64_t out_cap);
int aha_hip_debug_audio_embeds(aha_model* m, float* out, size_t n);
int aha_hip_argmax(const float* x, int64_t n, uint32_t* out_dev, void* stream);

#ifdef __cplusplus
}
#endif
#endif
```

Baseline: 379.3 tokens/s.

## Allow pk13 packing with a few exception rows read from bf16

```diff
diff --git a/aha_amd/_lib.py b/aha_amd/_lib.py
--- a/aha_amd/_lib.py
+++ b/aha_amd/_lib.py
@@ -256,6 +256,10 @@
     "aha_hip_pk13_status": (C.c_int, [_P, C.c_char_p, C.c_size_t]),
     "aha_hip_pack_pk13": (C.c_int, [_P, C.c_int32, C.c_int32, _P, C.POINTER(C.c_int32), C.POINTER(C.c_int64), _P]),
     "aha_hip_gemv_pk13": (C.c_int, [_P, C.c_int32, _P, _P, C.c_int32, C.c_int32, C.c_int32, _P, C.c_float, _P, _P, _P, _P]),
+    "aha_hip_pack_pk13_rows": (C.c_int, [_P, C.c_int32, C.c_int32, _P, C.POINTER(C.c_int32), C.POINTER(C.c_int32), C.c_int32, C.POINTER(C.c_int32),
+                                         C.POINTER(C.c_int64), C.POINTER(C.c_int64), _P]),
+    "aha_hip_gemv_pk13_rows": (C.c_int, [_P, C.c_int32, _P, C.POINTER(C.c_int32), C.c_int32, _P, _P, C.c_int32, C.c_int32, C.c_int32, _P, C.c_float,
+                                         _P, _P, _P, _P]),
     "aha_hip_debug_plan_gemv_pk13": (C.c_int, [C.c_int32, C.c_int32, C.c_int32, C.c_int32, C.POINTER(C.c_int32), C.POINTER(C.c_int32),
                                               C.POINTER(C.c_int32), C.POINTER(C.c_int32), C.POINTER(C.c_int32)]),
     "aha_hip_gemv_epi": (C.c_int, [_P, _P, _P, C.c_int32, C.c_int32, C.c_int32, _P, C.c_float, _P, _P, _P, _P]),
diff --git a/aha_amd/csrc/capi.hip b/aha_amd/csrc/capi.hip
--- a/aha_amd/csrc/capi.hip
+++ b/aha_amd/csrc/capi.hip
@@ -1199,7 +1199,7 @@
 
 static int gemv_epi_run(const void* W, int mx, const void* q, const uint32_t* scales, const void* x, void* y, int32_t N, int32_t K,
                         int32_t epi, const void* norm_w, float eps, const void* residual, float* logits, uint32_t* argmax_out, void* stream,
-                        int pk13_bh = 0) {
+                        int pk13_bh = 0, const int32_t* pk13_rows = nullptr, int pk13_nrows = 0) {
   hipStream_t st = (hipStream_t)stream;
   GemvArgs g{};
   g.W = W; g.x = x; g.y = y; g.N = epi == 2 ? N / 2 : N; g.K = K; g.norm_w = norm_w; g.eps = eps; g.residual = epi == 1 ? residual : nullptr;
@@ -1216,7 +1216,7 @@
   }
   if (!q) launch_gemv(g, e, st);
   else if (mx == 8) launch_gemv_mxfp8(g, q, scales, e, st);
-  else if (mx == 13) launch_gemv_pk13(g, q, pk13_bh, e, st);
+  else if (mx == 13) launch_gemv_pk13(g, q, pk13_bh, pk13_rows, pk13_nrows, e, st);
   else launch_gemv_mxfp4(g, q, scales, e, st);
   if (epi == 3) launch_argmax_partials(g.blk_max, g.blk_idx, tiles, argmax_out, st);
   hipError_t err = hipGetLastError();
@@ -1283,7 +1283,7 @@
   GemvPartials d;
   AHA_HIP_CHECK(hipMalloc(&d.p[0], sizeof(Pk13Stats)));
   AHA_HIP_CHECK(hipMemsetAsync(d.p[0], 0, sizeof(Pk13Stats), st));
-  launch_pk13_stats(W, (int64_t)N * K, (Pk13Stats*)d.p[0], st);
+  launch_pk13_stats(W, N, K, (Pk13Stats*)d.p[0], st);
   AHA_HIP_CHECK(hipGetLastError());
   Pk13Stats h{};
   AHA_HIP_CHECK(hipMemcpyAsync(&h, d.p[0], sizeof(h), hipMemcpyDeviceToHost, st));
@@ -1296,6 +1296,67 @@
     AHA_HIP_CHECK(hipStreamSynchronize(st));
   }
   return AHA_OK;
+  API_GUARD_END
+}
+
+int aha_hip_pack_pk13_rows(const void* W, int32_t N, int32_t K, void* out, int32_t* bh_out, int32_t* rows_out, int32_t cap, int32_t* nrows_out,
+                           int64_t* below_out, int64_t* nonfinite_out, void* stream) {
+  API_GUARD_BEGIN
+  if (!W || !bh_out || !rows_out || !nrows_out || !below_out || !nonfinite_out || cap < 0 || cap > PK13_MAX_EXC || N < 1 || K < 4096 || K % 4096) {
+    set_error("pack_pk13_rows: bad argument (W and the outputs not null, cap 0..16, N >= 1, K a positive multiple of 4096)");
+    return AHA_ERR_INVALID;
+  }
+  hipStream_t st = (hipStream_t)stream;
+  GemvPartials d;
+  AHA_HIP_CHECK(hipMalloc(&d.p[0], sizeof(Pk13Stats)));
+  AHA_HIP_CHECK(hipMemsetAsync(d.p[0], 0, sizeof(Pk13Stats), st));
+  launch_pk13_stats(W, N, K, (Pk13Stats*)d.p[0], st);
+  AHA_HIP_CHECK(hipGetLastError());
+  Pk13Stats h{};
+  AHA_HIP_CHECK(hipMemcpyAsync(&h, d.p[0], sizeof(h), hipMemcpyDeviceToHost, st));
+  AHA_HIP_CHECK(hipStreamSynchronize(st));
+  int rows[PK13_MAX_EXC];
+  const int n = pk13_exception_rows(h, rows);
+  *bh_out = pk13_base(h.max_e2);
+  *nonfinite_out = (int64_t)h.nonfinite;
+  *below_out = (int64_t)(h.bad - h.nonfinite);
+  *nrows_out = n;
+  for (int i = 0; i < cap && i < n && n <= PK13_MAX_EXC; ++i) rows_out[i] = rows[i];
+  if (out && !h.nonfinite && n <= cap) {
+    launch_pk13_pack(W, N, K, *bh_out, out, st);
+    AHA_HIP_CHECK(hipGetLastError());
+    AHA_HIP_CHECK(hipStreamSynchronize(st));
+  }
+  return AHA_OK;
+  API_GUARD_END
+}
+
+int aha_hip_gemv_pk13_rows(const void* packed, int32_t bh, const void* W, const int32_t* rows, int32_t nrows, const void* x, void* y, int32_t N,
+                           int32_t K, int32_t epi, const void* norm_w, float eps, const void* residual, float* logits, uint32_t* argmax_out,
+                           void* stream) {
+  API_GUARD_BEGIN
+  if (const char* bad = gemv_epi_args_bad(packed, x, y, N, K, 8, epi, residual, logits, argmax_out)) {
+    set_error(std::string("gemv_pk13_rows: ") + bad);
+    return AHA_ERR_INVALID;
+  }
+  if (K % 4096) {
+    set_error("gemv_pk13_rows: K must be a multiple of 4096 (the unit)");
+    return AHA_ERR_INVALID;
+  }
+  if (bh < 0 || bh > 112) {
+    set_error("gemv_pk13_rows: bh must be 0..112");
+    return AHA_ERR_INVALID;
+  }
+  if (nrows < 0 || nrows > PK13_MAX_EXC || (nrows > 0 && (!W || !rows))) {
+    set_error("gemv_pk13_rows: nrows must be 0..16, and rows need W and the list");
+    return AHA_ERR_INVALID;
+  }
+  for (int i = 0; i < nrows; ++i)
+    if (rows[i] < 0 || rows[i] >= N) {
+      set_error("gemv_pk13_rows: row " + std::to_string(rows[i]) + " is not a row of the matrix");
+      return AHA_ERR_INVALID;
+    }
+  return gemv_epi_run(W, 13, packed, nullptr, x, y, N, K, epi, norm_w, eps, residual, logits, argmax_out, stream, bh, rows, nrows);
   API_GUARD_END
 }
 
diff --git a/aha_amd/csrc/gemv_pk13_body.h b/aha_amd/csrc/gemv_pk13_body.h
--- a/aha_amd/csrc/gemv_pk13_body.h
+++ b/aha_amd/csrc/gemv_pk13_body.h
@@ -44,8 +44,14 @@
   float eps;
 };
 
-template <int R, int EPI, int PRO>
-__device__ __forceinline__ void gemv_pk13_body(const GemvPk13Args& a, float* xs, const int bid, const int nblk) {
+struct Pk13ExcRows {
+  const void* W;
+  int n;
+  int row[PK13_MAX_EXC];
+};
+
+template <int R, int EPI, int PRO, bool EXC = false>
+__device__ __forceinline__ void gemv_pk13_body(const GemvPk13Args& a, float* xs, const int bid, const int nblk, const Pk13ExcRows& ex = Pk13ExcRows{}) {
   const int tid = threadIdx.x, lane = tid & 63;
   const int wave = __builtin_amdgcn_readfirstlane(tid >> 6);
   const int K = a.K, N = a.N;
@@ -190,6 +196,41 @@
 #pragma unroll
     for (int r = 0; r < R; ++r) acc[m][r] = 0.f;
 
+  float* exc = red + 16;
+  if (EXC) {
+    for (int i = 0; i < ex.n; ++i) {
+      int wr = -1;
+#pragma unroll
+      for (int j = 0; j < PK13_MAX_EXC; ++j) wr = j == i ? ex.row[j] : wr;
+      const int orow = NW == 2 ? (wr >> 5) * 16 + (wr & 15) : wr;
+      const int otile = orow / ROWS_PER_TILE;
+      if (otile % nblk != bid || (orow % ROWS_PER_TILE) / R != wave) continue;
+      const bf16_t* wp = (const bf16_t*)ex.W + (size_t)wr * K + lane * 8;
+      float s = 0.f;
+#pragma unroll 1
+      for (int u = 0; u < gpt; ++u) {
+        u32x4_t w[8];
+        __builtin_amdgcn_sched_barrier(0);
+#pragma unroll
+        for (int c = 0; c < 8; ++c) w[c] = ld16(wp + ((u * 8 + c) << 9));
+#pragma unroll
+        for (int c = 0; c < 8; ++c) {
+          __builtin_amdgcn_sched_barrier(0);
+          const float4 xlo = *reinterpret_cast<const float4*>(xs + ((u * 8 + c) << 9) + (lane << 2));
+          const float4 xhi = *reinterpret_cast<const float4*>(xs + ((u * 8 + c) << 9) + 256 + (lane << 2));
+          s = fmaf(xlo.x, lo_bf(w[c][0]), s); s = fmaf(xlo.y, hi_bf(w[c][0]), s);
+          s = fmaf(xlo.z, lo_bf(w[c][1]), s); s = fmaf(xlo.w, hi_bf(w[c][1]), s);
+          s = fmaf(xhi.x, lo_bf(w[c][2]), s); s = fmaf(xhi.y, hi_bf(w[c][2]), s);
+          s = fmaf(xhi.z, lo_bf(w[c][3]), s); s = fmaf(xhi.w, hi_bf(w[c][3]), s);
+        }
+        __builtin_amdgcn_sched_barrier(0);
+      }
+      s = wave_sum(s);
+      if (lane == 0) exc[i] = s;
+    }
+    __builtin_amdgcn_sched_barrier(0);
+  }
+
   auto consume = [&](int gi, Pk13Unit (&buf)[NW][R], bf16_t (&resv)[R]) {
     const int c0 = (gi % gpt) * 8;
 #pragma unroll
@@ -220,6 +261,20 @@
     for (int m = 0; m < NW; ++m)
 #pragma unroll
       for (int r = 0; r < R; ++r) acc[m][r] = wave_sum(acc[m][r]);
+    if (EXC) {
+#pragma unroll
+      for (int r = 0; r < R; ++r) {
+        const int row = min(row0 + r, n_out - 1);
+        const int fr = NW == 2 ? (row >> 4) * 32 + (row & 15) : row;
+#pragma unroll
+        for (int m = 0; m < NW; ++m) {
+          int hit = -1;
+#pragma unroll
+          for (int i = 0; i < PK13_MAX_EXC; ++i) hit = ex.row[i] == fr + 16 * m ? i : hit;
+          if (__builtin_expect(hit >= 0, 0)) acc[m][r] = exc[hit];
+        }
+      }
+    }
     if (lane == 0) {
 #pragma unroll
       for (int r = 0; r < R; ++r) {
diff --git a/aha_amd/csrc/kernels.h b/aha_amd/csrc/kernels.h
--- a/aha_amd/csrc/kernels.h
+++ b/aha_amd/csrc/kernels.h
@@ -267,17 +267,22 @@
 int gemv_mxfp4_num_tiles(int N, int K);
 bool gemv_mxfp4_by_plan(int N, int K, GemvEpi epi);
 void debug_plan_gemv_mxfp4(int N, int K, GemvEpi epi, bool has_norm, int* out5);
+constexpr int PK13_MAX_EXC = 16;
 struct Pk13Stats {
   int max_e2;
-  int pad;
+  int over;
   unsigned long long bad;
+  unsigned long long nonfinite;
+  int row1[PK13_MAX_EXC];
 };
 __host__ __device__ inline int pk13_base(int max_e2) { return max_e2 > 15 ? max_e2 - 15 : 0; }
 size_t pk13_bytes(int N, int K);
-void launch_pk13_stats(const void* w, int64_t n_elems, Pk13Stats* stats, hipStream_t st);
+void launch_pk13_stats(const void* w, int N, int K, Pk13Stats* stats, hipStream_t st);
+int pk13_exception_rows(const Pk13Stats& s, int* rows);
 void launch_pk13_pack(const void* w, int N, int K, int bh, void* out, hipStream_t st);
 bool gemv_pk13_shape_ok(int N, int K);
 void launch_gemv_pk13(const GemvArgs& g, const void* packed, int bh, GemvEpi epi, hipStream_t st);
+void launch_gemv_pk13(const GemvArgs& g, const void* packed, int bh, const int* rows, int nrows, GemvEpi epi, hipStream_t st);
 int gemv_pk13_num_tiles(int N, int K);
 bool gemv_pk13_by_plan(int N, int K, GemvEpi epi);
 void debug_plan_gemv_pk13(int N, int K, GemvEpi epi, bool has_norm, int* out5);
diff --git a/aha_amd/csrc/kernels_gemv_pk13.hip b/aha_amd/csrc/kernels_gemv_pk13.hip
--- a/aha_amd/csrc/kernels_gemv_pk13.hip
+++ b/aha_amd/csrc/kernels_gemv_pk13.hip
@@ -24,6 +24,16 @@
   a.p = p; a.x = x; a.norm_w = norm_w; a.residual = residual; a.y = y;
   a.y_f32 = t.y_f32; a.blk_max = t.blk_max; a.blk_idx = t.blk_idx; a.h_out = t.h_out; a.N = N; a.K = K; a.bh = bh; a.eps = t.eps;
   gemv_pk13_body<R, EPI, PRO>(a, xs, (int)blockIdx.x, t.nblk);
+}
+
+template <int R, int EPI, int PRO>
+__global__ __launch_bounds__(GEMV_THREADS) void gemv_kernel_rows_pk13(const void* p, const void* x, const void* norm_w, void* y, const void* residual,
+                                                                      int N, int K, int bh, GemvPk13TailArgs t, Pk13ExcRows ex) {
+  extern __shared__ __attribute__((aligned(16))) float xs[];
+  GemvPk13Args a;
+  a.p = p; a.x = x; a.norm_w = norm_w; a.residual = residual; a.y = y;
+  a.y_f32 = t.y_f32; a.blk_max = t.blk_max; a.blk_idx = t.blk_idx; a.h_out = t.h_out; a.N = N; a.K = K; a.bh = bh; a.eps = t.eps;
+  gemv_pk13_body<R, EPI, PRO, true>(a, xs, (int)blockIdx.x, t.nblk, ex);
 }
 
 struct GemvPk13Plan { int R, grid; };
@@ -46,11 +56,17 @@
 int pro_of(int K, bool has_norm) { return K <= (has_norm ? 4 : 8) * 8 * GEMV_THREADS ? (has_norm ? 2 : 1) : 0; }
 
 template <int R, int EPI>
-void launch_pk13_epi(const GemvPk13Args& a, const GemvPk13Plan& p, hipStream_t st) {
+void launch_pk13_epi(const GemvPk13Args& a, const GemvPk13Plan& p, const Pk13ExcRows& ex, hipStream_t st) {
   const size_t lds = (size_t)a.K * 4 + 64;
   dim3 grid(p.grid), block(GEMV_THREADS);
   const GemvPk13TailArgs t{a.y_f32, a.blk_max, a.blk_idx, a.h_out, a.eps, p.grid};
   const int pro = pro_of(a.K, a.norm_w != nullptr);
+  if (ex.n > 0) {
+#define GV_(PP) hipLaunchKernelGGL((gemv_kernel_rows_pk13<R, EPI, PP>), grid, block, lds + PK13_MAX_EXC * 4, st, a.p, a.x, a.norm_w, a.y, a.residual, a.N, a.K, a.bh, t, ex)
+    if (pro == 2) GV_(2); else if (pro == 1) GV_(1); else GV_(0);
+#undef GV_
+    return;
+  }
 #define GV_(PP) hipLaunchKernelGGL((gemv_kernel_pk13<R, EPI, PP>), grid, block, lds, st, a.p, a.x, a.norm_w, a.y, a.residual, a.N, a.K, a.bh, t)
   if (pro == 2) GV_(2); else if (pro == 1) GV_(1); else GV_(0);
 #undef GV_
@@ -76,20 +92,37 @@
   }
   if ((threadIdx.x & 63) == 0) {
     atomicMax(&out->max_e2, mx);
-    if (bad) atomicAdd(&out->bad, bad);
-  }
-}
-
-__global__ __launch_bounds__(256) void pk13_window_kernel(const u32x4_t* w, int64_t nvec, Pk13Stats* out) {
+    if (bad) {
+      atomicAdd(&out->bad, bad);
+      atomicAdd(&out->nonfinite, bad);
+    }
+  }
+}
+
+__global__ __launch_bounds__(256) void pk13_window_kernel(const u32x4_t* w, int64_t nvec, int K, Pk13Stats* out) {
   const int bh = pk13_base(out->max_e2);
   unsigned long long bad = 0;
   for (int64_t i = (int64_t)blockIdx.x * 256 + threadIdx.x; i < nvec; i += (int64_t)gridDim.x * 256) {
     const u32x4_t v = ld_nt16(w + i);
+    bool below = false;
 #pragma unroll
     for (int j = 0; j < 8; ++j) {
       const uint32_t b = (v[j >> 1] >> ((j & 1) * 16)) & 0xffffu;
       const int e2 = pk13_e2(b);
-      if ((b & 0x7f80u) != 0x7f80u && e2 != 0 && e2 <= bh) ++bad;
+      if ((b & 0x7f80u) != 0x7f80u && e2 != 0 && e2 <= bh) {
+        ++bad;
+        below = true;
+      }
+    }
+    if (below && *(volatile int*)&out->over == 0) {
+      const int key = (int)(i * 8 / K) + 1;
+      int s = 0;
+      for (; s < PK13_MAX_EXC; ++s) {
+        int cur = *(volatile int*)&out->row1[s];
+        if (cur == 0) cur = atomicCAS(&out->row1[s], 0, key);
+        if (cur == 0 || cur == key) break;
+      }
+      if (s == PK13_MAX_EXC) atomicExch(&out->over, 1);
     }
   }
   for (int o = 32; o > 0; o >>= 1) bad += __shfl_xor(bad, o);
@@ -132,11 +165,21 @@
 
 size_t pk13_bytes(int N, int K) { return (size_t)N * (K / PK13_UNIT_K) * PK13_UNIT_BYTES; }
 
-void launch_pk13_stats(const void* w, int64_t n_elems, Pk13Stats* stats, hipStream_t st) {
-  const int64_t nvec = n_elems / 8;
+void launch_pk13_stats(const void* w, int N, int K, Pk13Stats* stats, hipStream_t st) {
+  const int64_t nvec = (int64_t)N * K / 8;
   const int grid = (int)std::min<int64_t>((nvec + 255) / 256, 4096);
   hipLaunchKernelGGL(pk13_max_kernel, dim3(grid), dim3(256), 0, st, (const u32x4_t*)w, nvec, stats);
-  hipLaunchKernelGGL(pk13_window_kernel, dim3(grid), dim3(256), 0, st, (const u32x4_t*)w, nvec, stats);
+  hipLaunchKernelGGL(pk13_window_kernel, dim3(grid), dim3(256), 0, st, (const u32x4_t*)w, nvec, K, stats);
+}
+
+int pk13_exception_rows(const Pk13Stats& s, int* rows) {
+  if (s.over) return PK13_MAX_EXC + 1;
+  int n = 0;
+  for (int i = 0; i < PK13_MAX_EXC; ++i)
+    if (s.row1[i] > 0) rows[n++] = s.row1[i] - 1;
+  std::sort(rows, rows + n);
+  for (int i = n; i < PK13_MAX_EXC; ++i) rows[i] = -1;
+  return n;
 }
 
 void launch_pk13_pack(const void* w, int N, int K, int bh, void* out, hipStream_t st) {
@@ -158,19 +201,32 @@
   out5[0] = p.R; out5[1] = 8; out5[2] = p.grid; out5[3] = 1; out5[4] = pro_of(K, has_norm);
 }
 
-void launch_gemv_pk13(const GemvArgs& g, const void* packed, int bh, GemvEpi epi, hipStream_t st) {
+void launch_gemv_pk13(const GemvArgs& g, const void* packed, int bh, const int* rows, int nrows, GemvEpi epi, hipStream_t st) {
   if (!gemv_pk13_shape_ok(g.N, g.K)) abort();
+  const int mat_rows = (epi == GEMV_SILU_MUL ? 2 : 1) * g.N;
+  if (nrows < 0 || nrows > PK13_MAX_EXC || (nrows > 0 && (g.W == nullptr || rows == nullptr))) abort();
+  Pk13ExcRows ex{};
+  ex.W = g.W;
+  ex.n = nrows;
+  for (int i = 0; i < PK13_MAX_EXC; ++i) {
+    ex.row[i] = i < nrows ? rows[i] : -1;
+    if (i < nrows && (rows[i] < 0 || rows[i] >= mat_rows)) abort();
+  }
   GemvPk13Args a{};
   a.p = packed; a.x = g.x; a.norm_w = g.norm_w; a.residual = g.residual; a.y = g.y; a.y_f32 = g.y_f32;
   a.blk_max = g.blk_max; a.blk_idx = g.blk_idx; a.h_out = g.h_out; a.N = g.N; a.K = g.K; a.bh = bh; a.eps = g.eps;
   const GemvPk13Plan p = plan_gemv_pk13(g.N, epi);
   switch (epi) {
-    case GEMV_STORE: launch_pk13_epi<1, GEMV_STORE>(a, p, st); break;
-    case GEMV_RESIDUAL: launch_pk13_epi<1, GEMV_RESIDUAL>(a, p, st); break;
-    case GEMV_SILU_MUL: launch_pk13_epi<1, GEMV_SILU_MUL>(a, p, st); break;
-    case GEMV_LOGITS: launch_pk13_epi<2, GEMV_LOGITS>(a, p, st); break;
+    case GEMV_STORE: launch_pk13_epi<1, GEMV_STORE>(a, p, ex, st); break;
+    case GEMV_RESIDUAL: launch_pk13_epi<1, GEMV_RESIDUAL>(a, p, ex, st); break;
+    case GEMV_SILU_MUL: launch_pk13_epi<1, GEMV_SILU_MUL>(a, p, ex, st); break;
+    case GEMV_LOGITS: launch_pk13_epi<2, GEMV_LOGITS>(a, p, ex, st); break;
     default: abort();
   }
 }
 
-}
+void launch_gemv_pk13(const GemvArgs& g, const void* packed, int bh, GemvEpi epi, hipStream_t st) {
+  launch_gemv_pk13(g, packed, bh, nullptr, 0, epi, st);
+}
+
+}
diff --git a/aha_amd/csrc/model.h b/aha_amd/csrc/model.h
--- a/aha_amd/csrc/model.h
+++ b/aha_amd/csrc/model.h
@@ -28,6 +28,9 @@
 struct Pk13Copy {
   void* p = nullptr;
   int bh = 0;
+  const void* w = nullptr;
+  int nrows = 0;
+  int rows[PK13_MAX_EXC] = {};
 };
 struct Pk13Entry { std::string name; Pk13Copy* slot; std::string status; };
 
diff --git a/aha_amd/csrc/model.hip b/aha_amd/csrc/model.hip
--- a/aha_amd/csrc/model.hip
+++ b/aha_amd/csrc/model.hip
@@ -548,8 +548,10 @@
   m->pk13.push_back({c.tie_word_embeddings ? "embed_tokens.weight (tied lm_head)" : "lm_head.weight", &m->p_lm_head, ""});
   mats.push_back({m->lm_head, m->lm_rows, H});
   auto all = [&](const char* why) {
-    for (Pk13Entry& e : m->pk13)
+    for (Pk13Entry& e : m->pk13) {
       if (e.status.empty()) e.status = why;
+      if (!e.slot->p) *e.slot = Pk13Copy{};
+    }
     return AHA_OK;
   };
   const char* env = getenv("AHA_WPACK");
@@ -571,7 +573,7 @@
       return all("not enough device memory");
     }
     hipError_t e = hipMemsetAsync(d, 0, cand.size() * sizeof(Pk13Stats), st);
-    for (size_t k = 0; k < cand.size() && e == hipSuccess; ++k) launch_pk13_stats(mats[cand[k]].w, (int64_t)mats[cand[k]].N * mats[cand[k]].K, d + k, st);
+    for (size_t k = 0; k < cand.size() && e == hipSuccess; ++k) launch_pk13_stats(mats[cand[k]].w, mats[cand[k]].N, mats[cand[k]].K, d + k, st);
     if (e == hipSuccess) e = hipGetLastError();
     if (e == hipSuccess) e = hipMemcpyAsync(h.data(), d, cand.size() * sizeof(Pk13Stats), hipMemcpyDeviceToHost, st);
     if (e == hipSuccess) e = hipStreamSynchronize(st);
@@ -579,13 +581,24 @@
     AHA_HIP_CHECK(e);
   }
   std::vector<size_t> take;
+  std::vector<std::string> row_note(mats.size());
   size_t bytes = 0;
   for (size_t k = 0; k < cand.size(); ++k) {
+    Pk13Copy& pk = *m->pk13[cand[k]].slot;
+    pk.nrows = h[k].bad ? pk13_exception_rows(h[k], pk.rows) : 0;
+    if (h[k].nonfinite || pk.nrows > PK13_MAX_EXC) {
+      m->pk13[cand[k]].status = std::to_string(h[k].bad) + " weights outside the window (Inf, NaN, or more than 30 binades below the matrix maximum)";
+      pk = Pk13Copy{};
+      continue;
+    }
     if (h[k].bad) {
-      m->pk13[cand[k]].status = std::to_string(h[k].bad) + " weights outside the window (Inf, NaN, or more than 30 binades below the matrix maximum)";
-      continue;
-    }
-    m->pk13[cand[k]].slot->bh = pk13_base(h[k].max_e2);
+      std::string& why = row_note[cand[k]];
+      why = std::to_string(h[k].bad) + " weights outside the window: packed, rows";
+      for (int i = 0; i < pk.nrows; ++i) why += (i ? ", " : " ") + std::to_string(pk.rows[i]);
+      why += " read from bf16";
+    }
+    pk.w = mats[cand[k]].w;
+    pk.bh = pk13_base(h[k].max_e2);
     take.push_back(cand[k]);
     bytes += pk13_bytes(mats[cand[k]].N, mats[cand[k]].K);
   }
@@ -604,7 +617,7 @@
       return all("not enough device memory");
     }
     launch_pk13_pack(mats[i].w, mats[i].N, mats[i].K, m->pk13[i].slot->bh, m->pk13[i].slot->p, st);
-    m->pk13[i].status = "packed";
+    m->pk13[i].status = row_note[i].empty() ? "packed" : row_note[i];
   }
   hipError_t e = hipGetLastError();
   if (e == hipSuccess) e = hipStreamSynchronize(st);
@@ -1042,7 +1055,11 @@
   ProfScope ps(m, fp8 ? "gemv_fp8" : fp4 ? "gemv_fp4" : "gemv", weights * (fp8 ? 1.03125 : fp4 ? 0.53125 : p13 ? 1.625 : 2.0) + act_bytes, 2.0 * weights);
   if (fp8) launch_gemv_mxfp8(g, wq.q, wq.scales, epi, m->stream);
   else if (fp4) launch_gemv_mxfp4(g, wq.q, wq.scales, epi, m->stream);
-  else if (p13) launch_gemv_pk13(g, pk.p, pk.bh, epi, m->stream);
+  else if (p13) {
+    GemvArgs gw = g;
+    gw.W = pk.w;
+    launch_gemv_pk13(gw, pk.p, pk.bh, pk.rows, pk.nrows, epi, m->stream);
+  }
   else if (epi == GEMV_RESIDUAL) gemv_row_parallel(m, g);
   else launch_gemv(g, epi, m->stream);
 }
diff --git a/aha_amd/ops.py b/aha_amd/ops.py
--- a/aha_amd/ops.py
+++ b/aha_amd/ops.py
@@ -476,6 +476,33 @@
     y, logits, am = _gemv_epi_outputs(N, epi, x.device, out)
     check(lib().aha_hip_gemv_pk13(_ptr(packed), bh, _ptr(x), _ptr(y), N, K, epi, _ptr(norm_w), eps, _ptr(residual), _ptr(logits), _ptr(am),
                                   _stream()))
+    return (logits, int(am.item())) if epi == GEMV_ROWS_LOGITS else y
+
+
+def pack_pk13_rows(W: torch.Tensor, cap: int = 16, check_only: bool = False):
+    _chk(W)
+    N, K = W.shape
+    bh, n, below, nonfinite = C.c_int32(), C.c_int32(), C.c_int64(), C.c_int64()
+    rows = (C.c_int32 * 16)()
+    out = None if check_only else torch.zeros(N, K // 4096, 6656, dtype=torch.uint8, device=W.device)
+    check(lib().aha_hip_pack_pk13_rows(_ptr(W), N, K, _ptr(out), C.byref(bh), rows, cap, C.byref(n), C.byref(below), C.byref(nonfinite), _stream()))
+    got = None if n.value > 16 else [int(rows[i]) for i in range(min(n.value, cap))]
+    ok = nonfinite.value == 0 and n.value <= cap
+    return (out if ok else None), bh.value, got, below.value, nonfinite.value
+
+
+def gemv_pk13_rows(packed: torch.Tensor, bh: int, W: Optional[torch.Tensor], rows, x: torch.Tensor, epi: int = GEMV_ROWS_STORE,
+                   norm_w: Optional[torch.Tensor] = None, eps: float = 1e-6, residual: Optional[torch.Tensor] = None,
+                   out: Optional[torch.Tensor] = None):
+    _chk(packed, x, norm_w, residual, out)
+    if W is not None:
+        _chk(W)
+    N, K = packed.shape[0], packed.shape[1] * 4096
+    rows = [int(r) for r in rows]
+    arr = (C.c_int32 * max(len(rows), 1))(*rows)
+    y, logits, am = _gemv_epi_outputs(N, epi, x.device, out)
+    check(lib().aha_hip_gemv_pk13_rows(_ptr(packed), bh, _ptr(W), arr, len(rows), _ptr(x), _ptr(y), N, K, epi, _ptr(norm_w), eps, _ptr(residual),
+                                       _ptr(logits), _ptr(am), _stream()))
     return (logits, int(am.item())) if epi == GEMV_ROWS_LOGITS else y
 
 
diff --git a/aha_amd/quant.py b/aha_amd/quant.py
--- a/aha_amd/quant.py
+++ b/aha_amd/quant.py
@@ -1,4 +1,4 @@
-from typing import Tuple
+from typing import List, Tuple
 
 import torch
 
@@ -158,6 +158,40 @@
     return torch.cat([a, hp, sp], dim=2).to(torch.uint8)
 
 
+PK13_MAX_ROWS = 16
+
+
+def _below_window(W: torch.Tensor, bh: int) -> torch.Tensor:
+    bits = _bf16_bits(W)
+    e2 = (bits >> 8) & 0x7f
+    return ((bits & 0x7f80) != 0x7f80) & (e2 != 0) & (e2 <= bh)
+
+
+def check_pk13_rows(W: torch.Tensor) -> Tuple[int, int, List[int]]:
+    bh, _ = check_pk13(W)
+    bits = _bf16_bits(W)
+    nonfinite = int(((bits & 0x7f80) == 0x7f80).sum())
+    rows = torch.nonzero(_below_window(W, bh).any(dim=1)).flatten().tolist()
+    return bh, nonfinite, rows
+
+
+def packable_pk13_rows(nonfinite: int, rows) -> bool:
+    return nonfinite == 0 and len(rows) <= PK13_MAX_ROWS
+
+
+def pack_pk13_rows(W: torch.Tensor, bh: int) -> torch.Tensor:
+    Wz = W.clone()
+    Wz[_below_window(W, bh)] = 0.0
+    return pack_pk13(Wz, bh)
+
+
+def unpack_pk13_rows(P: torch.Tensor, bh: int, W: torch.Tensor, rows) -> torch.Tensor:
+    out = unpack_pk13(P, bh).clone()
+    for r in rows:
+        out[r] = W[r]
+    return out
+
+
 def unpack_pk13(P: torch.Tensor, bh: int) -> torch.Tensor:
     N, J, B = P.shape
     assert B == PK13_UNIT_BYTES
diff --git a/include/aha_hip.h b/include/aha_hip.h
--- a/include/aha_hip.h
+++ b/include/aha_hip.h
@@ -353,6 +353,11 @@
 int aha_hip_pack_pk13(const void* W, int32_t N, int32_t K, void* out, int32_t* bh_out, int64_t* bad_out, void* stream);
 int aha_hip_gemv_pk13(const void* packed, int32_t bh, const void* x, void* y, int32_t N, int32_t K, int32_t epi, const void* norm_w,
                       float eps, const void* residual, float* logits, uint32_t* argmax_out, void* stream);
+int aha_hip_pack_pk13_rows(const void* W, int32_t N, int32_t K, void* out, int32_t* bh_out, int32_t* rows_out, int32_t cap, int32_t* nrows_out,
+                           int64_t* below_out, int64_t* nonfinite_out, void* stream);
+int aha_hip_gemv_pk13_rows(const void* packed, int32_t bh, const void* W, const int32_t* rows, int32_t nrows, const void* x, void* y, int32_t N,
+                           int32_t K, int32_t epi, const void* norm_w, float eps, const void* residual, float* logits, uint32_t* argmax_out,
+                           void* stream);
 int aha_hip_quantize_mxfp4(const void* W, int32_t N, int32_t K, void* q_out, uint32_t* scales_out, void* w_roundtrip_out, void* stream);
 int aha_hip_gemv_rows_mxfp4(const void* q, const uint32_t* scales, const void* x, void* y, int32_t R, int32_t N, int32_t K, int32_t epi,
                             const void* residual, float* logits, uint32_t* argmax_out, void* stream);
```

Measured after the change: 386.2 tokens/s, median of 6. +1.8%, better.
